# JiapengWu/TeMP

Hardware: AMD Instinct MI355X
Metric: edges/sec (fwd+bwd) RGCN+GRU seq_len=15 (higher is better)
Workload: dtype f32

## Files before the change

### include/temp_amd.h

```cpp
#ifndef TEMP_AMD_H
#define TEMP_AMD_H

#include <stddef.h>
#include <stdint.h>

#ifdef __cplusplus
extern "C" {
#endif

#define TEMP_ABI_VERSION 2

enum {
  TEMP_OK = 0,
  TEMP_E_BADARG = 1,
  TEMP_E_UNSUPPORTED = 2,
  TEMP_E_WORKSPACE = 3,
  TEMP_E_LAUNCH = 4
};

enum { TEMP_ACT_NONE = 0, TEMP_ACT_RELU = 1 };
enum { TEMP_GRU_TORCH = 0,
       TEMP_GRU_TYPE1 = 1 };

int temp_abi_version(void);
// ... 108 lines not shown
  TempEdgeView by_pair;
} TempPairView;
int temp_expand_chunk_segments(int n_chunks, const int32_t* chunk_seg, const int32_t* chunk_beg, const int32_t* chunk_end, int n_pos,
                               int32_t* seg_of, void* stream);
int temp_rgcn_pair_supported(int d_in, int d_out, int num_bases);
size_t temp_rgcn_pair_fwd_workspace(const TempGraph* g, const TempPairView* pv, int d_out);
int temp_rgcn_pair_fwd(const TempGraph* g, const TempPairView* pv, const float* table, const int32_t* ids, int n_table, int d_in, int d_out,
                       int num_bases, int n_rel_rows, const float* weight, const float* loop_w, const float* bias, int act, float* out,
                       void* workspace, size_t workspace_bytes, const TempDropout* drop, void* stream);
size_t temp_rgcn_pair_bwd_workspace(const TempGraph* g, const TempPairView* pv, int d_in, int d_out, int num_bases);
int temp_rgcn_pair_bwd(const TempGraph* g, const TempPairView* pv, const float* table, const int32_t* ids, const int32_t* inv_ptr,
                       const int32_t* inv_order, int n_table, const float* out, const float* d_out_grad, int d_in, int d_out, int num_bases,
                       int n_rel_rows, const float* weight, const float* loop_w, int has_bias, int act, float* d_table, float* d_weight,
                       float* d_loop_w, float* d_bias, void* workspace, size_t workspace_bytes, const TempDropout* drop, void* stream);

int temp_rgcn_isolated_fwd(int n, int d, const float* e, const float* loop_w, const float* bias ,
                           int act, float* out, const TempDropout* drop, void* stream);
size_t temp_rgcn_isolated_bwd_workspace(int n, int d);
int temp_rgcn_isolated_bwd(int n, int d, const float* e, const float* out, const float* d_out_grad,
                           const float* loop_w, int has_bias, int act,
                           float* d_e, float* d_loop_w, float* d_bias ,
                           void* workspace, size_t workspace_bytes, const TempDropout* drop, void* stream);

int temp_gru_fwd(int n, int d, int variant,
                 const float* x, const float* prev, const int32_t* prev_idx , const float* dt,
                 float lambda, const float* decay_wb ,
                 const float* w_ih, const float* w_hh, const float* b_ih, const float* b_hh,
                 float* h_out, float* saved, void* stream);

size_t temp_gru_bwd_workspace(int n, int d, int variant);
int temp_gru_bwd(int n, int d, int variant,
                 const float* x, const float* prev, const int32_t* prev_idx , const float* dt,
                 float lambda, const float* decay_wb ,
                 const float* w_ih, const float* w_hh,
                 const float* saved, const float* d_h_out,
                 float* d_x, float* d_prev, float* d_w_ih, float* d_w_hh, float* d_b_ih, float* d_b_hh,
                 float* d_decay_wb ,
                 void* workspace, size_t workspace_bytes, void* stream);

int temp_decay_rows(int n, int d, const float* x, const float* dt, float lambda, float* out, void* stream);

int temp_gru_input_gates(int n, int d, int variant, const float* x, const float* w_ih, const float* b_ih, float* gi, void* stream);
int temp_gru_input_gates_multi(int count, const int* ns, int d, int variant, const float* const* xs, const float* const* w_ihs,
                               const float* const* b_ihs, float* const* gis, void* stream);
int temp_gru_input_gates_gather_multi(int count, const int* ns, int d, int variant, const float* const* xs, const int32_t* const* x_idx,
                                      const float* const* w_ihs, const float* const* b_ihs, float* const* gis, void* stream);
int temp_gru_cell_fwd(int n, int d, int variant, const float* gi, const float* prev, const int32_t* prev_idx ,
                      const float* dt, float lambda, const float* w_hh, const float* b_hh,
                      float* h_out, float* saved, size_t saved_plane, void* stream);
int temp_gru_cell_bwd(int n, int d, int variant, const float* saved, size_t saved_plane,
                      const float* dh_up , const float* d_prev_next , const int32_t* next_idx ,
                      const float* dt, float lambda, const float* w_hh,
                      float* dgi, float* dgh, float* decv, float* d_prev, void* stream);
typedef struct TempGruCellFwd {
  int32_t n; const float* gi; const float* prev ;
  const int32_t* prev_idx ; const float* dt;
  const float* w_hh; const float* b_hh; float* h_out; float* saved ;
} TempGruCellFwd;
typedef struct TempGruCellBwd {
  int32_t n; const float* saved; const float* dh_up ; const float* d_prev_next ;
  const int32_t* next_idx ; const float* dt; const float* w_hh;
  float* dgi; float* dgh; float* decv; float* d_prev;
  int32_t no_prev;
} TempGruCellBwd;
int temp_gru_cell_fwd_multi(int count, const TempGruCellFwd* cells, int d, int variant, float lambda, size_t saved_plane, void* stream);
int temp_gru_cell_bwd_multi(int count, const TempGruCellBwd* cells, int d, int variant, float lambda, size_t saved_plane, void* stream);
size_t temp_gru_weight_grads_workspace(int n, int d, int variant);
int temp_gru_weight_grads(int n, int d, int variant, const float* x, const float* hdec, const float* dgi, const float* dgh,
                          const float* w_ih, float* d_x , float* d_w_ih, float* d_w_hh, float* d_b_ih, float* d_b_hh,
                          void* workspace, size_t workspace_bytes, void* stream);
size_t temp_gru_weight_grads_multi_workspace(int count, const int* ns, int d, int variant);
int temp_gru_weight_grads_multi(int count, const int* ns, int d, int variant, const float* const* xs, const float* const* hdecs,
                                const float* const* dgis, const float* const* dghs, const float* const* w_ihs, float* const* d_xs,
                                float* d_w, float* d_b, void* workspace, size_t workspace_bytes, void* stream);

size_t temp_gru_grads_g4_workspace(int count, const int* ns, int d);
int temp_gru_grads_g4(int count, const int* ns, int d, const float* const* xs, const float* const* hdecs, const float* const* g4s,
                      const float* const* w_ihs, float* const* d_xs, float* d_w, float* d_b, void* workspace, size_t workspace_bytes,
                      void* stream);
int temp_gru_grads_g4_keys(int count, const int* ns, int d, const float* const* xs, const float* const* hdecs, const float* const* g4s,
                           const float* const* w_ihs, float* const* d_xs, float* d_w, float* d_b, const uint32_t* const* g4_row_keys,
                           const uint32_t* const* g4_col_keys, const uint32_t* const* x_col_keys ,
                           void* workspace, size_t workspace_bytes, void* stream);

#define TEMP_CHAIN_HAS_PREV (1 << 30)
#define TEMP_CHAIN_TRACKS 32
#define TEMP_CHAIN_MAX_RNN 4
#define TEMP_CHAIN_MAX_UP 8
typedef struct TempGruChain {
  int32_t d, variant, n_panels, n_steps;
  int32_t max_steps;
  const int32_t* panel; const int32_t* rows; const int32_t* sinfo;
  const float* dt;
  float lambda;
  size_t saved_plane;
  int32_t n_rnn;
  const float* packed[TEMP_CHAIN_MAX_RNN];
  const float* b_hh[TEMP_CHAIN_MAX_RNN];
  const int32_t* gi_index;
  int32_t pack_layout;
} TempGruChain;
enum { TEMP_CHAIN_PACK_F32 = 1, TEMP_CHAIN_PACK_BX = 2, TEMP_CHAIN_PACK_HX = 3, TEMP_CHAIN_PACK_HX_X = 4 };
int temp_gru_chain_pack_layout(int d);
int temp_gru_chain_supported(int d);
size_t temp_gru_chain_pack_floats(int d);
int temp_gru_chain_pack(int d, const float* w_hh, float* packed, void* stream);
int temp_gru_chain_pack_multi(int count, int d, const float* const* w_hh, float* const* packed, void* stream);
int temp_gru_chain_fwd(const TempGruChain* c, const float* gi, float* h_out, float* saved, void* stream);
int temp_gru_chain_fwd_x_supported(int d, int variant, int max_steps);
size_t temp_gru_chain_pack_x_floats(int d);
int temp_gru_chain_pack_x_multi(int count, int d, const float* const* w_hh, const float* const* w_ih, float* const* packed, void* stream);
int temp_gru_chain_fwd_x(const TempGruChain* c, const float* x, const int32_t* x_index, const float* const* b_ih, float* h_out, float* saved,
                         void* stream);
long long temp_gru_chain_fwd_x_launches(void);
int temp_gru_chain_bwd(const TempGruChain* c, const float* saved, int n_up, const float* const* up ,
                       float* dgi, float* dgh, void* stream);
int temp_gru_chain_bwd_g4(const TempGruChain* c, const float* saved, int n_up, const float* const* up ,
                          float* g4, void* stream);
int temp_gru_chain_keys_supported(int d);
int temp_gru_chain_bwd_g4_keys(const TempGruChain* c, const float* saved, int n_up, const float* const* up, float* g4,
                               uint32_t* row_keys, uint32_t* col_keys, void* stream);

int temp_gather_rows(int n, int d, const float* table, const int32_t* idx, float* out, void* stream);
size_t temp_keys_cols_size(int d);
int temp_absmax_keys(int n, int d, const float* x, int ldx, uint32_t* row_keys, uint32_t* col_keys, void* stream);
int temp_gather_rows_keys(int n, int d, const float* table, const int32_t* idx, float* out, uint32_t* row_keys, uint32_t* col_keys, void* stream);
int temp_linear_keys(int M, int N, int K, const float* A, int lda, const uint32_t* a_keys, const float* B, int ldb, int trans_b, float* C, int ldc,
                     void* stream);
int temp_gru_input_gates_gather_multi_keys(int count, const int* ns, int d, int variant, const float* const* xs, const int32_t* const* x_idx,
                                           const uint32_t* const* x_keys, const float* const* w_ihs, const float* const* b_ihs, float* const* gis,
                                           void* stream);
int temp_scatter_add_rows(int n, int d, const float* src, const int32_t* idx, float* table, void* stream);
size_t temp_segment_sum_rows_workspace(int n_seg, int n_rows, int d);
int temp_segment_sum_rows(int n_seg, int n_rows, int d, const int32_t* seg_ptr, const int32_t* order, const float* src, float* out,
                          void* workspace, size_t workspace_bytes, void* stream);
int temp_segment_sum_rows_relu(int n_seg, int n_rows, int d, const int32_t* seg_ptr, const int32_t* order, const float* src, const float* relu_of,
                               float* out, void* workspace, size_t workspace_bytes, void* stream);

int temp_linear(int M, int N, int K, const float* A, int lda, const float* B, int ldb, int trans_b, float* C, int ldc, void* stream);
int temp_linear_t(int M, int N, int K, const float* A, int lda, const float* B, int ldb, int trans_b, float* Ct, int ldct, void* stream);
typedef struct TempLinearProblem { int M; const float* A; const float* B; float* C; } TempLinearProblem;
int temp_linear_multi(int count, const TempLinearProblem* probs, int N, int K, int lda, int ldb, int trans_b, int ldc, void* stream);
size_t temp_linear_tn_workspace(int M, int Ka, int Nb);
int temp_linear_tn(int M, int Ka, int Nb, const float* A, int lda, const float* B, int ldb, float* out, int ldo,
                   void* workspace, size_t workspace_bytes, void* stream);
size_t temp_linear_tn_multi_workspace(int count, int max_m, int Ka, int Nb);
int temp_linear_tn_multi(int count, const TempLinearProblem* probs, int Ka, int Nb, int lda, int ldb, int ldc, void* workspace,
                         size_t workspace_bytes, void* stream);

int temp_gather_ce_fwd(int P, int C, int N, const float* scores, const int32_t* cand, float* loss_rows, float* lse_rows, void* stream);
int temp_gather_ce_bwd(int P, int C, int N, const float* scores, const int32_t* cand, const float* lse_rows, const float* scale,
                       float inv_rows, const float* row_scale , float* d_scores, void* stream);

#define TEMP_SCORE_DISTMULT 0
#define TEMP_SCORE_COMPLEX 1
int temp_bilinear_query_fwd(int P, int d, int kind, const float* ent_rows, const int32_t* known_idx, const float* rel, const int32_t* rel_idx,
                            const int32_t* is_tail, float* q, void* stream);
int temp_bilinear_query_bwd(int P, int d, int kind, const float* ent_rows, const int32_t* known_idx, const float* rel, const int32_t* rel_idx,
                            const int32_t* is_tail, const float* d_q, float* d_known_rows, float* d_rel_rows, void* stream);

int temp_gated_query_fwd(int P, int d, int kind, const float* A, const int32_t* ia, const float* B, const int32_t* ib, const float* w,
                         const float* rel, const int32_t* rel_idx, const int32_t* is_tail, float* q, void* stream);
int temp_gated_query_bwd(int P, int d, int kind, const float* A, const int32_t* ia, const float* B, const int32_t* ib, const float* w,
                         const float* rel, const int32_t* rel_idx, const int32_t* is_tail, const float* d_q, float* d_a_rows, float* d_b_rows,
                         float* d_rel_rows, float* d_w, void* stream);
int temp_gather_ce_mix_fwd(int P, int C, int N, const float* s_a, const float* s_b, const float* w, const int32_t* cand, float* loss_rows,
                           float* lse_rows, void* stream);
int temp_gather_ce_mix_bwd(int P, int C, int N, const float* s_a, const float* s_b, const float* w, const int32_t* cand, const float* lse_rows,
                           const float* scale, float inv_rows, const float* row_scale , float* d_s_a, float* d_s_b,
                           float* d_w, void* stream);

#define TEMP_ASSEMBLE_PIECE 4096
typedef struct TempCopyDesc { const int32_t* src; const int32_t* aux; int32_t dst_off; int32_t len; int32_t add; int32_t mode; } TempCopyDesc;
int temp_assemble_views(int n_pieces, const int32_t* piece_desc, const int32_t* piece_start, const TempCopyDesc* descs, const int32_t* table,
                        int32_t* out, void* stream);

typedef struct TempSubsampleJob {
  int32_t n_nodes, n_edges, keep;
  uint64_t seed;
  const int32_t* parent; int32_t* child; const int32_t* eid;
  int32_t off_a[3], off_b[3], off_chunk_beg[3], off_chunk_end[3], off_chunk_seg[3], n_chunks[3];
  int32_t off_in_deg, off_out_deg, off_nnorm;
  uint8_t* keep_mask; void* scratch;
} TempSubsampleJob;
int temp_subsample_views(int n_jobs, const TempSubsampleJob* jobs, void* stream);

int temp_corrupt_sample(int R, int K, int N, uint64_t seed, const int32_t* truth, const int32_t* lo, const int32_t* hi, const int32_t* ids,
                        int32_t* cand, void* stream);

int temp_filtered_rank(int P, int N, int ld, const float* scores, const int32_t* target, const int32_t* filt_ptr,
                       const int32_t* filt_ids, int32_t* ranks, void* stream);

typedef struct TempAttn {
  int32_t n, D, heads, T;
// ... 22 lines not shown
```

### temp_amd/_lib.py

```python
import ctypes
import threading
import os

_HERE = os.path.dirname(os.path.abspath(__file__))
LIB_PATH = os.path.join(_HERE, "libtemp_amd.so")

c_i32p = ctypes.POINTER(ctypes.c_int32)
c_f32p = ctypes.POINTER(ctypes.c_float)
c_vp = ctypes.c_void_p

ACT_NONE, ACT_RELU = 0, 1
GRU_TORCH, GRU_TYPE1 = 0, 1
CHUNK = 64
CHUNK_REL = 128


class TempEdgeView(ctypes.Structure):
    _fields_ = [("n_seg", ctypes.c_int32), ("n_edges", ctypes.c_int32), ("a", c_vp), ("b", c_vp),
                ("n_chunks", ctypes.c_int32), ("chunk_seg", c_vp), ("chunk_beg", c_vp), ("chunk_end", c_vp),
                ("chunk_slot", c_vp), ("n_partial", ctypes.c_int32), ("n_fix", ctypes.c_int32),
                ("fix_seg", c_vp), ("fix_slot", c_vp), ("fix_cnt", c_vp)]


class TempMembers(ctypes.Structure):
    _fields_ = [("n_members", ctypes.c_int32), ("max_nodes", ctypes.c_int32), ("max_edges", ctypes.c_int32),
                ("max_chunks", ctypes.c_int32 * 3), ("node_off", c_vp), ("edge_off", c_vp), ("chunk_off", c_vp), ("fix_off", c_vp)]


class TempGraph(ctypes.Structure):
    _fields_ = [("n_nodes", ctypes.c_int32), ("n_edges", ctypes.c_int32), ("nnorm", c_vp), ("in_deg", c_vp),
                ("out_deg", c_vp), ("by_dst", TempEdgeView), ("by_src", TempEdgeView), ("by_rel", TempEdgeView),
                ("members", TempMembers)]


class TempPairView(ctypes.Structure):
    _fields_ = [("n_table", ctypes.c_int32), ("n_rel_rows", ctypes.c_int32), ("fwd_row", c_vp), ("by_pair", TempEdgeView)]


ABI_VERSION = 2
OPT_MFMA_BF16X3, OPT_TN_SPLIT, OPT_RGCN_SCALAR, OPT_GEMM_STREAM, OPT_GRU_STREAM, OPT_RGCN_TILE, OPT_DEBUG, OPT_OVERLAP, OPT_GEMM_RESIDENT, OPT_MFMA_F16X2, OPT_RGCN_PAIR = range(11)


class TempGruCellFwd(ctypes.Structure):
    _fields_ = [("n", ctypes.c_int32), ("gi", c_vp), ("prev", c_vp), ("prev_idx", c_vp), ("dt", c_vp), ("w_hh", c_vp),
                ("b_hh", c_vp), ("h_out", c_vp), ("saved", c_vp)]


class TempGruCellBwd(ctypes.Structure):
    _fields_ = [("n", ctypes.c_int32), ("saved", c_vp), ("dh_up", c_vp), ("d_prev_next", c_vp), ("next_idx", c_vp), ("dt", c_vp),
                ("w_hh", c_vp), ("dgi", c_vp), ("dgh", c_vp), ("decv", c_vp), ("d_prev", c_vp), ("no_prev", ctypes.c_int32)]


CHAIN_HAS_PREV = 1 << 30
CHAIN_TRACKS = 32
CHAIN_MAX_RNN = 4
CHAIN_MAX_UP = 8
CHAIN_MAX_STEPS = 64
CHAIN_PACK_F32, CHAIN_PACK_BX, CHAIN_PACK_HX, CHAIN_PACK_HX_X = 1, 2, 3, 4


class TempGruChain(ctypes.Structure):
    _fields_ = [("d", ctypes.c_int32), ("variant", ctypes.c_int32), ("n_panels", ctypes.c_int32), ("n_steps", ctypes.c_int32),
                ("max_steps", ctypes.c_int32), ("panel", c_vp), ("rows", c_vp), ("sinfo", c_vp), ("dt", c_vp), ("lambda_", ctypes.c_float),
                ("saved_plane", ctypes.c_size_t), ("n_rnn", ctypes.c_int32), ("packed", c_vp * CHAIN_MAX_RNN), ("b_hh", c_vp * CHAIN_MAX_RNN),
                ("gi_index", c_vp), ("pack_layout", ctypes.c_int32)]


class TempSubsampleJob(ctypes.Structure):
    _fields_ = [("n_nodes", ctypes.c_int32), ("n_edges", ctypes.c_int32), ("keep", ctypes.c_int32), ("seed", ctypes.c_uint64),
                ("parent", c_vp), ("child", c_vp), ("eid", c_vp),
                ("off_a", ctypes.c_int32 * 3), ("off_b", ctypes.c_int32 * 3), ("off_chunk_beg", ctypes.c_int32 * 3),
                ("off_chunk_end", ctypes.c_int32 * 3), ("off_chunk_seg", ctypes.c_int32 * 3), ("n_chunks", ctypes.c_int32 * 3),
                ("off_in_deg", ctypes.c_int32), ("off_out_deg", ctypes.c_int32), ("off_nnorm", ctypes.c_int32),
                ("keep_mask", c_vp), ("scratch", c_vp)]


class TempDropout(ctypes.Structure):
    _fields_ = [("p", ctypes.c_float), ("seed", ctypes.c_uint64)]


class TempAttn(ctypes.Structure):
    _fields_ = [("n", ctypes.c_int32), ("D", ctypes.c_int32), ("heads", ctypes.c_int32), ("T", ctypes.c_int32),
                ("q", c_vp), ("ldq", ctypes.c_int32), ("kh", c_vp), ("vh", c_vp), ("ldh", ctypes.c_int32),
                ("kc", c_vp), ("vc", c_vp), ("ldc", ctypes.c_int32), ("idx", c_vp), ("decay", c_vp)]


class TempLinearProblem(ctypes.Structure):
    _fields_ = [("M", ctypes.c_int32), ("A", c_vp), ("B", c_vp), ("C", c_vp)]


ASSEMBLE_PIECE = 4096
SCORE_KINDS = {"distmult": 0, "complex": 1}

_G = ctypes.POINTER(TempGraph)
_PV = ctypes.POINTER(TempPairView)
_I, _F, _SZ = ctypes.c_int, ctypes.c_float, ctypes.c_size_t
SYMBOLS = {
    "temp_abi_version": (_I, []),
    "temp_error_string": (ctypes.c_char_p, [_I]),
    "temp_set_option": (_I, [_I, _I]),
    "temp_get_option": (_I, [_I]),
    "temp_scratch_refused": (ctypes.c_longlong, []),
    "temp_f16_launches": (ctypes.c_longlong, []),
    "temp_tile_launches": (ctypes.c_longlong, []),
    "temp_set_debug_buffer": (None, [c_vp, _SZ]),
    "temp_rgcn_fwd_workspace": (_SZ, [_G, _I]),
    "temp_rgcn_fwd": (_I, [_G, c_vp, c_vp, _I, _I, _I, _I, c_vp, c_vp, c_vp, _I, c_vp, c_vp, _SZ, c_vp, c_vp]),
    "temp_rgcn_bwd_workspace": (_SZ, [_G, _I, _I, _I, _I]),
    "temp_rgcn_bwd": (_I, [_G, c_vp, c_vp, c_vp, _I, _I, _I, _I, c_vp, c_vp, _I, _I, c_vp, c_vp, c_vp, c_vp, c_vp, _SZ, c_vp, c_vp]),
    "temp_rgcn_bwd_dh": (_I, [_G, c_vp, c_vp, _I, _I, _I, _I, c_vp, c_vp, _I, c_vp, c_vp, c_vp, c_vp, _SZ, c_vp, c_vp]),
    "temp_rgcn_bwd_weights": (_I, [_G, c_vp, c_vp, c_vp, _I, _I, _I, _I, _I, c_vp, c_vp, c_vp, c_vp, _SZ, c_vp]),
    "temp_rgcn_table_fwd_workspace": (_SZ, [_G, _I, _I]),
    "temp_rgcn_table_fwd": (_I, [_G, c_vp, c_vp, _I, _I, _I, _I, _I, c_vp, c_vp, c_vp, _I, c_vp, c_vp, _SZ, c_vp, c_vp]),
    "temp_rgcn_table_bwd_workspace": (_SZ, [_G, _I, _I, _I, _I]),
    "temp_rgcn_table_bwd": (_I, [_G, c_vp, c_vp, c_vp, c_vp, _I, c_vp, c_vp, _I, _I, _I, _I, c_vp, c_vp, _I, _I, c_vp, c_vp, c_vp, c_vp,
                                 c_vp, _SZ, c_vp, c_vp]),
    "temp_pair_launches": (ctypes.c_longlong, []),
    "temp_expand_chunk_segments": (_I, [_I, c_vp, c_vp, c_vp, _I, c_vp, c_vp]),
    "temp_rgcn_pair_supported": (_I, [_I, _I, _I]),
    "temp_rgcn_pair_fwd_workspace": (_SZ, [_G, _PV, _I]),
    "temp_rgcn_pair_fwd": (_I, [_G, _PV, c_vp, c_vp, _I, _I, _I, _I, _I, c_vp, c_vp, c_vp, _I, c_vp, c_vp, _SZ, c_vp, c_vp]),
    "temp_rgcn_pair_bwd_workspace": (_SZ, [_G, _PV, _I, _I, _I]),
    "temp_rgcn_pair_bwd": (_I, [_G, _PV, c_vp, c_vp, c_vp, c_vp, _I, c_vp, c_vp, _I, _I, _I, _I, c_vp, c_vp, _I, _I, c_vp, c_vp, c_vp, c_vp,
                                c_vp, _SZ, c_vp, c_vp]),
    "temp_rgcn_isolated_fwd": (_I, [_I, _I, c_vp, c_vp, c_vp, _I, c_vp, c_vp, c_vp]),
    "temp_rgcn_isolated_bwd_workspace": (_SZ, [_I, _I]),
    "temp_rgcn_isolated_bwd": (_I, [_I, _I, c_vp, c_vp, c_vp, c_vp, _I, _I, c_vp, c_vp, c_vp, c_vp, _SZ, c_vp, c_vp]),
    "temp_gru_fwd": (_I, [_I, _I, _I, c_vp, c_vp, c_vp, c_vp, _F, c_vp, c_vp, c_vp, c_vp, c_vp, c_vp, c_vp, c_vp]),
    "temp_gru_bwd_workspace": (_SZ, [_I, _I, _I]),
    "temp_gru_bwd": (_I, [_I, _I, _I, c_vp, c_vp, c_vp, c_vp, _F, c_vp, c_vp, c_vp, c_vp, c_vp,
                          c_vp, c_vp, c_vp, c_vp, c_vp, c_vp, c_vp, c_vp, _SZ, c_vp]),
    "temp_decay_rows": (_I, [_I, _I, c_vp, c_vp, _F, c_vp, c_vp]),
    "temp_gru_input_gates": (_I, [_I, _I, _I, c_vp, c_vp, c_vp, c_vp, c_vp]),
    "temp_gru_input_gates_multi": (_I, [_I, c_vp, _I, _I, c_vp, c_vp, c_vp, c_vp, c_vp]),
    "temp_gru_input_gates_gather_multi": (_I, [_I, c_vp, _I, _I, c_vp, c_vp, c_vp, c_vp, c_vp, c_vp]),
    "temp_gru_cell_fwd": (_I, [_I, _I, _I, c_vp, c_vp, c_vp, c_vp, _F, c_vp, c_vp, c_vp, c_vp, _SZ, c_vp]),
    "temp_gru_cell_bwd": (_I, [_I, _I, _I, c_vp, _SZ, c_vp, c_vp, c_vp, c_vp, _F, c_vp, c_vp, c_vp, c_vp, c_vp, c_vp]),
    "temp_gru_cell_fwd_multi": (_I, [_I, ctypes.POINTER(TempGruCellFwd), _I, _I, _F, _SZ, c_vp]),
    "temp_gru_cell_bwd_multi": (_I, [_I, ctypes.POINTER(TempGruCellBwd), _I, _I, _F, _SZ, c_vp]),
    "temp_gru_weight_grads_workspace": (_SZ, [_I, _I, _I]),
    "temp_gru_weight_grads": (_I, [_I, _I, _I, c_vp, c_vp, c_vp, c_vp, c_vp, c_vp, c_vp, c_vp, c_vp, c_vp, c_vp, _SZ, c_vp]),
    "temp_gru_weight_grads_multi_workspace": (ctypes.c_size_t, [_I, c_vp, _I, _I]),
    "temp_gru_weight_grads_multi": (_I, [_I, c_vp, _I, _I, c_vp, c_vp, c_vp, c_vp, c_vp, c_vp, c_vp, c_vp, c_vp, ctypes.c_size_t, c_vp]),
    "temp_gru_chain_supported": (_I, [_I]),
    "temp_gru_chain_pack_floats": (_SZ, [_I]),
    "temp_gru_chain_pack": (_I, [_I, c_vp, c_vp, c_vp]),
    "temp_gru_chain_pack_multi": (_I, [_I, _I, ctypes.POINTER(c_vp), ctypes.POINTER(c_vp), c_vp]),
    "temp_gru_chain_fwd": (_I, [ctypes.POINTER(TempGruChain), c_vp, c_vp, c_vp, c_vp]),
    "temp_gru_chain_pack_layout": (_I, [_I]),
    "temp_gru_chain_fwd_x_supported": (_I, [_I, _I, _I]),
    "temp_gru_chain_pack_x_floats": (_SZ, [_I]),
    "temp_gru_chain_pack_x_multi": (_I, [_I, _I, ctypes.POINTER(c_vp), ctypes.POINTER(c_vp), ctypes.POINTER(c_vp), c_vp]),
    "temp_gru_chain_fwd_x": (_I, [ctypes.POINTER(TempGruChain), c_vp, c_vp, ctypes.POINTER(c_vp), c_vp, c_vp, c_vp]),
    "temp_gru_chain_fwd_x_launches": (ctypes.c_longlong, []),
    "temp_gru_chain_bwd": (_I, [ctypes.POINTER(TempGruChain), c_vp, _I, ctypes.POINTER(c_vp), c_vp, c_vp, c_vp]),
    "temp_gru_chain_bwd_g4": (_I, [ctypes.POINTER(TempGruChain), c_vp, _I, ctypes.POINTER(c_vp), c_vp, c_vp]),
    "temp_gru_chain_keys_supported": (_I, [_I]),
    "temp_gru_chain_bwd_g4_keys": (_I, [ctypes.POINTER(TempGruChain), c_vp, _I, ctypes.POINTER(c_vp), c_vp, c_vp, c_vp, c_vp]),
    "temp_gru_grads_g4_keys": (_I, [_I, c_vp, _I, c_vp, c_vp, c_vp, c_vp, c_vp, c_vp, c_vp, c_vp, c_vp, c_vp, c_vp, ctypes.c_size_t, c_vp]),
    "temp_gru_grads_g4_workspace": (ctypes.c_size_t, [_I, c_vp, _I]),
    "temp_gru_grads_g4": (_I, [_I, c_vp, _I, c_vp, c_vp, c_vp, c_vp, c_vp, c_vp, c_vp, c_vp, ctypes.c_size_t, c_vp]),
    "temp_gather_rows": (_I, [_I, _I, c_vp, c_vp, c_vp, c_vp]),
    "temp_keys_cols_size": (_SZ, [_I]),
    "temp_absmax_keys": (_I, [_I, _I, c_vp, _I, c_vp, c_vp, c_vp]),
    "temp_gather_rows_keys": (_I, [_I, _I, c_vp, c_vp, c_vp, c_vp, c_vp, c_vp]),
    "temp_linear_keys": (_I, [_I, _I, _I, c_vp, _I, c_vp, c_vp, _I, _I, c_vp, _I, c_vp]),
    "temp_gru_input_gates_gather_multi_keys": (_I, [_I, c_vp, _I, _I, c_vp, c_vp, c_vp, c_vp, c_vp, c_vp, c_vp]),
    "temp_scatter_add_rows": (_I, [_I, _I, c_vp, c_vp, c_vp, c_vp]),
    "temp_segment_sum_rows_workspace": (_SZ, [_I, _I, _I]),
    "temp_segment_sum_rows": (_I, [_I, _I, _I, c_vp, c_vp, c_vp, c_vp, c_vp, _SZ, c_vp]),
    "temp_segment_sum_rows_relu": (_I, [_I, _I, _I, c_vp, c_vp, c_vp, c_vp, c_vp, c_vp, _SZ, c_vp]),
    "temp_linear": (_I, [_I, _I, _I, c_vp, _I, c_vp, _I, _I, c_vp, _I, c_vp]),
    "temp_linear_t": (_I, [_I, _I, _I, c_vp, _I, c_vp, _I, _I, c_vp, _I, c_vp]),
    "temp_linear_multi": (_I, [_I, ctypes.POINTER(TempLinearProblem), _I, _I, _I, _I, _I, _I, c_vp]),
    "temp_linear_tn_workspace": (_SZ, [_I, _I, _I]),
    "temp_linear_tn_multi_workspace": (_SZ, [_I, _I, _I, _I]),
    "temp_linear_tn_multi": (_I, [_I, ctypes.POINTER(TempLinearProblem), _I, _I, _I, _I, _I, c_vp, _SZ, c_vp]),
    "temp_linear_tn": (_I, [_I, _I, _I, c_vp, _I, c_vp, _I, c_vp, _I, c_vp, _SZ, c_vp]),
    "temp_gather_ce_fwd": (_I, [_I, _I, _I, c_vp, c_vp, c_vp, c_vp, c_vp]),
    "temp_gather_ce_bwd": (_I, [_I, _I, _I, c_vp, c_vp, c_vp, c_vp, _F, c_vp, c_vp, c_vp]),
    "temp_bilinear_query_fwd": (_I, [_I, _I, _I, c_vp, c_vp, c_vp, c_vp, c_vp, c_vp, c_vp]),
    "temp_bilinear_query_bwd": (_I, [_I, _I, _I, c_vp, c_vp, c_vp, c_vp, c_vp, c_vp, c_vp, c_vp, c_vp]),
    "temp_gated_query_fwd": (_I, [_I, _I, _I, c_vp, c_vp, c_vp, c_vp, c_vp, c_vp, c_vp, c_vp, c_vp, c_vp]),
    "temp_gated_query_bwd": (_I, [_I, _I, _I, c_vp, c_vp, c_vp, c_vp, c_vp, c_vp, c_vp, c_vp, c_vp, c_vp, c_vp, c_vp, c_vp, c_vp]),
    "temp_gather_ce_mix_fwd": (_I, [_I, _I, _I, c_vp, c_vp, c_vp, c_vp, c_vp, c_vp, c_vp]),
    "temp_gather_ce_mix_bwd": (_I, [_I, _I, _I, c_vp, c_vp, c_vp, c_vp, c_vp, c_vp, _F, c_vp, c_vp, c_vp, c_vp, c_vp]),
    "temp_assemble_views": (_I, [_I, c_vp, c_vp, c_vp, c_vp, c_vp, c_vp]),
    "temp_subsample_views": (_I, [_I, ctypes.POINTER(TempSubsampleJob), c_vp]),
    "temp_corrupt_sample": (_I, [_I, _I, _I, ctypes.c_uint64, c_vp, c_vp, c_vp, c_vp, c_vp, c_vp]),
    "temp_filtered_rank": (_I, [_I, _I, _I, c_vp, c_vp, c_vp, c_vp, c_vp, c_vp]),
    "temp_sa_attn_fwd": (_I, [ctypes.POINTER(TempAttn), c_vp, c_vp, c_vp, c_vp]),
    "temp_sa_attn_bwd": (_I, [ctypes.POINTER(TempAttn), c_vp, c_vp, c_vp, c_vp, c_vp, _I, c_vp, c_vp, _I, c_vp, c_vp, _I, c_vp, _I, c_vp, c_vp, c_vp, c_vp]),
    "temp_copy_probe": (_I, [c_vp, c_vp, _SZ, c_vp]),
    "temp_trace_begin": (_I, [_I]),
    "temp_trace_end": (_I, [c_i32p, c_f32p, _I, c_i32p]),
    "temp_trace_kernel_name": (ctypes.c_char_p, [_I]),
}

_lib = None


class TempAmdError(RuntimeError):
    pass


def load():
    global _lib
    if _lib is not None:
        return _lib
    if not os.path.exists(LIB_PATH):
        raise TempAmdError("libtemp_amd.so not found at %s -- run `python -m temp_amd.build` "
                           "(hipcc --offload-arch=gfx950); there is no CPU fallback" % LIB_PATH)
    lib = ctypes.CDLL(LIB_PATH) if os.environ.get("TEMP_PYDLL", "1") == "0" else ctypes.PyDLL(LIB_PATH)
    for name, (res, args) in SYMBOLS.items():
        fn = getattr(lib, name)
        fn.restype = res
        fn.argtypes = args
    if lib.temp_abi_version() != ABI_VERSION:
        raise TempAmdError("libtemp_amd.so ABI version %d != %d (stale .so or stale Python package)" % (lib.temp_abi_version(), ABI_VERSION))
    _lib = lib
    return lib


def check(rc, what):
    if rc != 0:
        msg = load().temp_error_string(rc).decode()
        raise TempAmdError("%s failed: %s (code %d)" % (what, msg, rc))


class _CreateLock:

    def __init__(self):
        self._l = threading.RLock()

    def __enter__(self):
        if not self._l.acquire(blocking=False):
            held = getattr(_coop, "held", False)
            if held:
                _py_token.release()
            self._l.acquire()
            if held:
                _py_token.acquire()
# ... 100 lines not shown
```

### temp_amd/backend.py

```python
import ctypes

import torch

from . import _lib

_backend = None


def set_backend(b):
    global _backend
    _backend = b


def get_backend():
    global _backend
    if _backend is None:
        _backend = HipBackend()
    return _backend


def _ptr(t):
    return ctypes.c_void_p(t.data_ptr()) if t is not None else None


# ... 298 lines not shown
            a.dh_up, a.d_prev_next, a.next_idx = opt(c["dh_up"]), opt(c["d_prev_next"]), opt(nidx)
            a.dt, a.w_hh = dt.data_ptr(), w_hh.data_ptr()
            a.dgi, a.dgh, a.decv, a.d_prev = c["dgi"].data_ptr(), c["dgh"].data_ptr(), c["decv"].data_ptr(), c["d_prev"].data_ptr()
            a.no_prev = 1 if c.get("no_prev") else 0
        rc = self.lib.temp_gru_cell_bwd_multi(len(cells), arr, d, variant, float(lam), saved_all.shape[1] * d, _stream())
        _lib.check(rc, "temp_gru_cell_bwd_multi")

    def subsample_views(self, jobs):
        arr = (_lib.TempSubsampleJob * len(jobs))()
        for a, j in zip(arr, jobs):
            a.n_nodes, a.n_edges, a.keep, a.seed = j["n_nodes"], j["n_edges"], j["keep"], int(j["seed"]) & 0xFFFFFFFFFFFFFFFF
            a.parent, a.child = _i32(j["parent"], "parent").data_ptr(), _i32(j["child"], "child").data_ptr()
            a.eid = _i32(j["eid"], "eid").data_ptr() if j["n_edges"] else None
            for fld in ("off_a", "off_b", "off_chunk_beg", "off_chunk_end", "off_chunk_seg", "n_chunks"):
                for v in range(3):
                    getattr(a, fld)[v] = int(j[fld][v])
            a.off_in_deg, a.off_out_deg, a.off_nnorm = int(j["off_in_deg"]), int(j["off_out_deg"]), int(j["off_nnorm"])
            a.keep_mask = j["keep_mask"].data_ptr() if j.get("keep_mask") is not None else None
            a.scratch = j["scratch"].data_ptr()
        _lib.check(self.lib.temp_subsample_views(len(jobs), arr, _stream()), "temp_subsample_views")

    def decay_rows(self, x, dt, lam):
        x, dt = _f32(x, "x"), _f32(dt, "dt")
        out = torch.empty_like(x)
        _lib.check(self.lib.temp_decay_rows(x.shape[0], x.shape[1], _ptr(x), _ptr(dt), float(lam), _ptr(out), _stream()), "temp_decay_rows")
        return out

    def gru_chain_supported(self, d):
        return bool(self.lib.temp_gru_chain_supported(int(d)))

    def gru_chain_pack(self, w_hh):
        w_hh = _f32(w_hh, "w_hh")
        d = w_hh.shape[1]
        out = torch.empty(self.lib.temp_gru_chain_pack_floats(d), dtype=torch.float32, device=w_hh.device)
        layout = self.lib.temp_gru_chain_pack_layout(d)
        _lib.check(self.lib.temp_gru_chain_pack(d, _ptr(w_hh), _ptr(out), _stream()), "temp_gru_chain_pack")
        out.chain_pack_layout = layout
        return out

    def gru_chain_pack_multi(self, w_hhs):
        w_hhs = [_f32(w, "w_hh") for w in w_hhs]
        d = w_hhs[0].shape[1]
        n = self.lib.temp_gru_chain_pack_floats(d)
        buf = torch.empty(len(w_hhs), n, dtype=torch.float32, device=w_hhs[0].device)
        src = (ctypes.c_void_p * len(w_hhs))(*[w.data_ptr() for w in w_hhs])
        dst = (ctypes.c_void_p * len(w_hhs))(*[buf[i].data_ptr() for i in range(len(w_hhs))])
        layout = self.lib.temp_gru_chain_pack_layout(d)
        _lib.check(self.lib.temp_gru_chain_pack_multi(len(w_hhs), d, src, dst, _stream()), "temp_gru_chain_pack_multi")
        return self._tagged([buf[i] for i in range(len(w_hhs))], layout)

    @staticmethod
    def _tagged(packs, layout):
        for pk in packs:
            pk.chain_pack_layout = layout
        return packs

    def _chain_desc(self, tabs, d, variant, lam, plane, packs, b_hhs):
        c = _lib.TempGruChain()
        c.d, c.variant, c.n_panels, c.n_steps, c.max_steps = d, variant, tabs["n_panels"], tabs["n_steps"], tabs["max_steps"]
        c.panel, c.rows, c.sinfo, c.dt = (_i32(tabs[k], k).data_ptr() for k in ("panel", "rows", "sinfo", "dt_bits"))
        c.lambda_, c.saved_plane, c.n_rnn = float(lam), plane, len(packs)
        layouts = {getattr(pk, "chain_pack_layout", None) for pk in packs}
        assert len(layouts) == 1 and None not in layouts, "chain packs without one common layout tag (gru_chain_pack*)"
        c.pack_layout = layouts.pop()
        keep = []
        for i, (pk, b) in enumerate(zip(packs, b_hhs)):
            pk, b = _f32(pk, "packed"), _f32(b, "b_hh")
            keep += [pk, b]
            c.packed[i], c.b_hh[i] = pk.data_ptr(), b.data_ptr()
        return c, keep

    def gru_chain_fwd(self, tabs, gi, lam, variant, packs, b_hhs, h_out, saved_all, gi_index=None):
        d = saved_all.shape[2]
        c, keep = self._chain_desc(tabs, d, variant, lam, saved_all.shape[1] * d, packs, b_hhs)
        if gi_index is not None:
            assert gi_index.shape[0] == saved_all.shape[1]
            c.gi_index = _i32(gi_index, "gi_index").data_ptr()
        rc = self.lib.temp_gru_chain_fwd(ctypes.byref(c), _ptr(_f32(gi, "gi")), _ptr(h_out), _ptr(saved_all), _stream())
        _lib.check(rc, "temp_gru_chain_fwd")

    def gru_chain_fwd_x_supported(self, d, variant, max_steps):
        return bool(self.lib.temp_gru_chain_fwd_x_supported(int(d), int(variant), int(max_steps)))

    def gru_chain_pack_x_multi(self, w_hhs, w_ihs):
        w_hhs, w_ihs = [_f32(w, "w_hh") for w in w_hhs], [_f32(w, "w_ih") for w in w_ihs]
        d = w_hhs[0].shape[1]
        k = len(w_hhs)
        n = self.lib.temp_gru_chain_pack_x_floats(d)
        buf = torch.empty(k, n, dtype=torch.float32, device=w_hhs[0].device)
        arr = lambda ts: (ctypes.c_void_p * k)(*[t.data_ptr() for t in ts])
        _lib.check(self.lib.temp_gru_chain_pack_x_multi(k, d, arr(w_hhs), arr(w_ihs), arr([buf[i] for i in range(k)]), _stream()),
                   "temp_gru_chain_pack_x_multi")
        return self._tagged([buf[i] for i in range(k)], _lib.CHAIN_PACK_HX_X)

    def gru_chain_fwd_x(self, tabs, x, x_index, lam, variant, packs, b_hhs, b_ihs, h_out, saved_all):
        d = saved_all.shape[2]
        c, keep = self._chain_desc(tabs, d, variant, lam, saved_all.shape[1] * d, packs, b_hhs)
        x = _f32(x, "x")
        assert x.shape[1] == d and x_index.shape[0] == saved_all.shape[1]
        b_ihs = [_f32(b, "b_ih") for b in b_ihs]
        barr = (ctypes.c_void_p * len(b_ihs))(*[b.data_ptr() for b in b_ihs])
        rc = self.lib.temp_gru_chain_fwd_x(ctypes.byref(c), _ptr(x), _ptr(_i32(x_index, "x_index")), barr, _ptr(h_out), _ptr(saved_all), _stream())
        _lib.check(rc, "temp_gru_chain_fwd_x")

    def gru_chain_bwd(self, tabs, saved_all, ups, lam, variant, packs, b_hhs, dgi, dgh):
        d = saved_all.shape[2]
        c, keep = self._chain_desc(tabs, d, variant, lam, saved_all.shape[1] * d, packs, b_hhs)
        ups = [_f32(u, "upstream") if u is not None else None for u in ups]
        arr = (ctypes.c_void_p * max(len(ups), 1))(*[u.data_ptr() if u is not None else None for u in ups])
        rc = self.lib.temp_gru_chain_bwd(ctypes.byref(c), _ptr(saved_all), len(ups), arr, _ptr(dgi), _ptr(dgh), _stream())
        _lib.check(rc, "temp_gru_chain_bwd")

    def gru_chain_keys_supported(self, d):
        return bool(self.lib.temp_gru_chain_keys_supported(int(d)))

    def gru_chain_bwd_g4(self, tabs, saved_all, ups, lam, variant, packs, b_hhs, g4, keys=None):
        d = saved_all.shape[2]
        c, keep = self._chain_desc(tabs, d, variant, lam, saved_all.shape[1] * d, packs, b_hhs)
        ups = [_f32(u, "upstream") if u is not None else None for u in ups]
        arr = (ctypes.c_void_p * max(len(ups), 1))(*[u.data_ptr() if u is not None else None for u in ups])
        if keys is not None:
            row_keys, col_keys = keys
            assert row_keys.dtype == torch.int32 and col_keys.dtype == torch.int32 and col_keys.is_contiguous()
            assert row_keys.numel() == saved_all.shape[1] and col_keys.numel() == (len(packs) + tabs["n_panels"]) * 4 * d
            rc = self.lib.temp_gru_chain_bwd_g4_keys(ctypes.byref(c), _ptr(saved_all), len(ups), arr, _ptr(g4), _ptr(row_keys), _ptr(col_keys),
                                                     _stream())
            _lib.check(rc, "temp_gru_chain_bwd_g4_keys")
            return
        rc = self.lib.temp_gru_chain_bwd_g4(ctypes.byref(c), _ptr(saved_all), len(ups), arr, _ptr(g4), _stream())
        _lib.check(rc, "temp_gru_chain_bwd_g4")

    def gru_grads_g4_supported(self, ns, d, variant):
        k = len(ns)
        if k < 1 or k > 4 or variant != _lib.GRU_TORCH:
            return False
        return self.lib.temp_gru_grads_g4_workspace(k, (ctypes.c_int * k)(*[int(n) for n in ns]), int(d)) > 0

    def gru_grads_g4(self, xs, hdecs, g4s, w_ihs, d_xs, row_keys=None, col_keys=None, x_col_keys=None):
        k = len(xs)
        d = xs[0].shape[1]
        dev = xs[0].device
        ns = (ctypes.c_int * k)(*[x.shape[0] for x in xs])
        nb = self.lib.temp_gru_grads_g4_workspace(k, ns, d)
        if nb == 0:
            raise ValueError("temp_gru_grads_g4: unsupported shape (check gru_grads_g4_supported first)")
        keep = [[_f32(t, "operand") for t in ts] for ts in (xs, hdecs, w_ihs)]
        for g in g4s:
            assert g.dtype == torch.float32 and g.is_contiguous() and g.shape[1] == 4 * d
        arr = lambda ts: (ctypes.c_void_p * k)(*[t.data_ptr() for t in ts])
        dx = (ctypes.c_void_p * k)(*[None if t is None else t.data_ptr() for t in d_xs])
        d_w = torch.empty(2 * k, 3 * d, d, dtype=torch.float32, device=dev)
        d_b = torch.empty(2 * k, 3 * d, dtype=torch.float32, device=dev)
        ws = self._ws(nb, dev)
        if row_keys is not None and col_keys is not None:
            for rk, ck, x in zip(row_keys, col_keys, xs):
                assert rk.dtype == torch.int32 and ck.dtype == torch.int32 and rk.is_contiguous() and ck.is_contiguous()
                assert rk.numel() == x.shape[0] and ck.numel() == 4 * d
            xk = None
            if x_col_keys is not None:
                for t in x_col_keys:
                    assert t.dtype == torch.int32 and t.is_contiguous() and t.numel() == d
                xk = arr(x_col_keys)
            rc = self.lib.temp_gru_grads_g4_keys(k, ns, d, arr(keep[0]), arr(keep[1]), arr(g4s), arr(keep[2]), dx, _ptr(d_w), _ptr(d_b),
                                                 arr(row_keys), arr(col_keys), xk, _ptr(ws), ws.numel(), _stream())
            _lib.check(rc, "temp_gru_grads_g4_keys")
            return [(d_w[2 * i], d_w[2 * i + 1], d_b[2 * i], d_b[2 * i + 1]) for i in range(k)]
        rc = self.lib.temp_gru_grads_g4(k, ns, d, arr(keep[0]), arr(keep[1]), arr(g4s), arr(keep[2]), dx, _ptr(d_w), _ptr(d_b), _ptr(ws),
                                        ws.numel(), _stream())
        _lib.check(rc, "temp_gru_grads_g4")
        return [(d_w[2 * i], d_w[2 * i + 1], d_b[2 * i], d_b[2 * i + 1]) for i in range(k)]

    def gru_weight_grads(self, x, hdec, dgi, dgh, w_ih, variant, d_x):
        n, d = x.shape
        w_ih = _f32(w_ih, "w_ih")
        dev = x.device
        d_w_ih = torch.empty_like(w_ih)
        d_w_hh = torch.empty(3 * d, d, dtype=torch.float32, device=dev)
        d_b_ih = torch.empty(w_ih.shape[0], dtype=torch.float32, device=dev)
        d_b_hh = torch.empty(3 * d, dtype=torch.float32, device=dev)
        ws = self._ws(self.lib.temp_gru_weight_grads_workspace(n, d, variant), dev)
        rc = self.lib.temp_gru_weight_grads(n, d, variant, _ptr(x), _ptr(hdec), _ptr(dgi), _ptr(dgh), _ptr(w_ih), _ptr(d_x),
                                            _ptr(d_w_ih), _ptr(d_w_hh), _ptr(d_b_ih), _ptr(d_b_hh), _ptr(ws), ws.numel(), _stream())
        _lib.check(rc, "temp_gru_weight_grads")
        return d_w_ih, d_w_hh, d_b_ih, d_b_hh

    def gru_weight_grads_multi(self, xs, hdecs, dgis, dghs, w_ihs, variant, d_xs):
        k = len(xs)
        if k < 1 or k > 4 or variant != _lib.GRU_TORCH or any(h is None for h in hdecs):
            return None
        d = xs[0].shape[1]
        dev = xs[0].device
        ns = (ctypes.c_int * k)(*[x.shape[0] for x in xs])
        nb = self.lib.temp_gru_weight_grads_multi_workspace(k, ns, d, variant)
        if nb == 0:
            return None
        keep = [[_f32(t, "operand") for t in ts] for ts in (xs, hdecs, dgis, dghs, w_ihs)]
        arr = lambda ts: (ctypes.c_void_p * k)(*[t.data_ptr() for t in ts])
        dx = (ctypes.c_void_p * k)(*[None if t is None else t.data_ptr() for t in d_xs])
        d_w = torch.empty(2 * k, 3 * d, d, dtype=torch.float32, device=dev)
        d_b = torch.empty(2 * k, 3 * d, dtype=torch.float32, device=dev)
        ws = self._ws(nb, dev)
        rc = self.lib.temp_gru_weight_grads_multi(k, ns, d, variant, arr(keep[0]), arr(keep[1]), arr(keep[2]), arr(keep[3]), arr(keep[4]), dx,
                                                  _ptr(d_w), _ptr(d_b), _ptr(ws), ws.numel(), _stream())
        if rc == 2:
            return None
        _lib.check(rc, "temp_gru_weight_grads_multi")
        return [(d_w[2 * i], d_w[2 * i + 1], d_b[2 * i], d_b[2 * i + 1]) for i in range(k)]

    def linear(self, a, b, trans_b, out=None, a_keys=None):
        a, b = _f32(a, "a"), _f32(b, "b")
        M, K = a.shape
        N = b.shape[0] if trans_b else b.shape[1]
        c = out if out is not None else torch.empty(M, N, dtype=torch.float32, device=a.device)
        assert c.shape == (M, N) and c.is_contiguous() and c.dtype == torch.float32
        if a_keys is not None:
            assert a_keys.dtype == torch.int32 and a_keys.is_contiguous() and a_keys.numel() == M
            rc = self.lib.temp_linear_keys(M, N, K, _ptr(a), K, _ptr(a_keys), _ptr(b), b.shape[1], int(trans_b), _ptr(c), N, _stream())
            _lib.check(rc, "temp_linear_keys")
            return c
        rc = self.lib.temp_linear(M, N, K, _ptr(a), K, _ptr(b), b.shape[1], int(trans_b), _ptr(c), N, _stream())
        _lib.check(rc, "temp_linear")
        return c

    def absmax_keys(self, x, rows=True, cols=True):
        x = _f32(x, "x")
        n, d = x.shape
        rk = torch.empty(n, dtype=torch.int32, device=x.device) if rows else None
        ck = torch.empty(self.lib.temp_keys_cols_size(d), dtype=torch.int32, device=x.device) if cols else None
        _lib.check(self.lib.temp_absmax_keys(n, d, _ptr(x), d, _ptr(rk), _ptr(ck), _stream()), "temp_absmax_keys")
        return rk, (ck[:d] if cols else None)

    def linear_t(self, a, b, trans_b, out_t):
        a, b = _f32(a, "a"), _f32(b, "b")
        M, K = a.shape
        N = b.shape[0] if trans_b else b.shape[1]
        if out_t.shape != (N, M) or not out_t.is_contiguous() or out_t.dtype != torch.float32:
            raise ValueError("linear_t: out_t must be a contiguous float32 (N, M) matrix")
        rc = self.lib.temp_linear_t(M, N, K, _ptr(a), K, _ptr(b), b.shape[1], int(trans_b), _ptr(out_t), M, _stream())
        _lib.check(rc, "temp_linear_t")
        return out_t

    def linear_multi(self, a_list, b_list, trans_b, out):
        K = a_list[0].shape[1]
        N = out.shape[1]
        arr = (_lib.TempLinearProblem * len(a_list))()
# ... 254 lines not shown
```

### temp_amd/csrc/gemm_bx.hpp

```cpp
#pragma once
#include "gemm_panel.hpp"

namespace temp {

typedef __bf16 bx_bf16x8 __attribute__((ext_vector_type(8)));
typedef unsigned int bx_u32x4 __attribute__((ext_vector_type(4)));

__device__ __forceinline__ void bx_split(float x, unsigned& h, unsigned& m, unsigned& l) {
  h = __float_as_uint(x) & 0xffff0000u;
  const float r1 = x - __uint_as_float(h);
  m = __float_as_uint(r1) & 0xffff0000u;
  l = __float_as_uint(r1 - __uint_as_float(m));
}
__device__ __forceinline__ void bx_split2(float x0, float x1, unsigned& H, unsigned& M, unsigned& L) {
  unsigned h0, m0, l0, h1, m1, l1;
  bx_split(x0, h0, m0, l0);
  bx_split(x1, h1, m1, l1);
  H = __builtin_amdgcn_perm(h1, h0, 0x07060302u);
  M = __builtin_amdgcn_perm(m1, m0, 0x07060302u);
  L = __builtin_amdgcn_perm(l1, l0, 0x07060302u);
}
__device__ __forceinline__ void bx_split8(const float4 a, const float4 b, bx_u32x4& H, bx_u32x4& M, bx_u32x4& L) {
  unsigned h, m, l;
  bx_split2(a.x, a.y, h, m, l); H[0] = h; M[0] = m; L[0] = l;
// ... 496 lines not shown
  g->per_xcd = ceil_div(g->row_tiles, 8);
  int best = 1;
  float best_cost = 1e30f;
  const int gmax = g->n_tiles < 7 ? g->n_tiles : 7;
  for (int w = 1; w <= gmax; ++w) {
    const int ng = ceil_div(g->n_tiles, w);
    const long long all_tiles = total_rows > 0 ? (total_rows + 127) / 128 : g->row_tiles;
    const long long blocks = (all_tiles > g->row_tiles ? all_tiles : (long long)g->row_tiles) * ng;
    const float rounds = blocks <= 512 ? 1.f : (float)blocks / 512.f + 0.5f;
    const float cost = rounds * (w + 0.5f);
    if (cost < best_cost * 0.999f || (cost <= best_cost * 1.001f && w > best)) { best_cost = cost; best = w; }
  }
  *G = best;
  g->n_groups = ceil_div(g->n_tiles, best);
  g->tail_store = g->n_tiles - (g->n_groups - 1) * best;
  return true;
}

}
#include "gemm_bxr.hpp"
#include "gemm_hx.hpp"
namespace temp {

template <class Epi>
static inline bool bx_pack_batch(const PanelBatch<Epi>& batch, int count, const BxGeom& g, hipStream_t st, BxPacked* pk) {
  const size_t pbytes = bx_packed_bytes(g.N, g.K);
  int n_distinct = 0, which[PANEL_MAXP];
  for (int i = 0; i < count; ++i) {
    which[i] = -1;
    for (int j = 0; j < i; ++j)
      if (batch.p[j].B == batch.p[i].B) { which[i] = which[j]; break; }
    if (which[i] < 0) which[i] = n_distinct++;
  }
  bx_u32x4* slot = pbytes * n_distinct <= BX_PACK_MAX_BYTES ? bx_scratch(st, pbytes * n_distinct) : nullptr;
  if (!slot) return false;
  const int n_slabs = ceil_div(g.K, 16);
  int done = 0;
  BxPackJobs jobs = {};
  for (int i = 0; i < PANEL_MAXP; ++i) pk->b[i] = slot;
  for (int i = 0; i < count; ++i) {
    bx_u32x4* dst = slot + (size_t)which[i] * (pbytes / 16);
    pk->b[i] = dst;
    if (which[i] < done) continue;
    ++done;
    if (n_distinct > 1 && n_distinct <= BX_PACK_JOBS) { bx_pack_jobs_add(jobs, batch.p[i].B, dst, g.K, g.N, g.ldb, g.trans_b); continue; }
    const dim3 pgrid(ceil_div((long long)n_slabs * g.n_tiles, 4));
    if (g.trans_b) TEMP_LAUNCH(K_BX_PACK, (k_bx_pack<1>), pgrid, dim3(256), 0, st, g.K, g.N, g.n_tiles, n_slabs, batch.p[i].B, g.ldb, dst);
    else TEMP_LAUNCH(K_BX_PACK, (k_bx_pack<0>), pgrid, dim3(256), 0, st, g.K, g.N, g.n_tiles, n_slabs, batch.p[i].B, g.ldb, dst);
  }
  if (jobs.count) TEMP_LAUNCH(K_BX_PACK, k_bx_pack_multi, dim3(ceil_div(jobs.total_units, 4)), dim3(256), 0, st, jobs);
  return true;
}

template <int G, class Epi>
static inline void launch_bx_g(int kid, const PanelBatch<Epi>& batch, int count, const BxGeom& g, hipStream_t st, const BxPacked* pk) {
  dim3 grid(8 * g.per_xcd * g.n_groups, count);
  if (pk) {
    TEMP_LAUNCH(kid, (k_gemm_bxp<G, Epi>), grid, dim3(BX_THREADS), 0, st, batch, g, *pk);
    return;
  }
  if (g.trans_b) TEMP_LAUNCH(kid, (k_gemm_bx<G, 1, Epi>), grid, dim3(BX_THREADS), 0, st, batch, g);
  else TEMP_LAUNCH(kid, (k_gemm_bx<G, 0, Epi>), grid, dim3(BX_THREADS), 0, st, batch, g);
}

template <class Epi>
static inline bool launch_bxr(int kid, const PanelBatch<Epi>& batch, int count, const BxGeom& g, hipStream_t st, const BxPacked* pkp) {
  if (!option(TEMP_OPT_GEMM_RESIDENT) || g.K > BXR_MAX_SLABS * 16 || g.K < 72) return false;
  if (EpiRawPre<Epi>::value && !EpiAccInit<Epi>::value && !(option(TEMP_OPT_DEBUG) & 0x200000)) return false;
  int max_m = 0;
  for (int i = 0; i < count; ++i) max_m = batch.p[i].M > max_m ? batch.p[i].M : max_m;
  BxrGeom rg;
  if (!bxr_plan(g.N, g.K, g.lda, max_m, &rg)) return false;
  rg.ldb = g.ldb; rg.trans_b = g.trans_b;
  BxPacked pk;
  for (int i = 0; i < PANEL_MAXP; ++i) pk.b[i] = pkp ? pkp->b[i] : nullptr;
  static const bool granted = hipFuncSetAttribute(reinterpret_cast<const void*>(k_gemm_bxr<Epi>), hipFuncAttributeMaxDynamicSharedMemorySize, BXR_LDS_BYTES) == hipSuccess;
  if (!granted) { (void)hipGetLastError(); return false; }
  const size_t lds = (size_t)rg.n_slabs * BXR_G * 192 * 16 + BXR_BIAS_BYTES;
  TEMP_LAUNCH(kid, (k_gemm_bxr<Epi>), dim3(256, count), dim3(BXR_WAVES * 64), lds, st, batch, rg, pk);
  return true;
}

template <class Epi>
int launch_gemm_bx(int kid, const PanelBatch<Epi>& batch, int count, const BxGeom& g, int G, hipStream_t st) {
  if (launch_hxr(kid, batch, count, g, st)) return launch_status();
  if (launch_bxr(kid, batch, count, g, st, nullptr)) return launch_status();
  if (hx_supported(batch, count, g)) {
    const int rc = launch_gemm_hx(kid, batch, count, g, G, st);
    if (rc != TEMP_E_UNSUPPORTED) return rc;
  }
  BxPacked pk;
  const bool packed = bx_pack_batch(batch, count, g, st, &pk);
  const BxPacked* pp = packed ? &pk : nullptr;
  switch (G) {
    case 1: launch_bx_g<1, Epi>(kid, batch, count, g, st, pp); break;
    case 2: launch_bx_g<2, Epi>(kid, batch, count, g, st, pp); break;
    case 3: launch_bx_g<3, Epi>(kid, batch, count, g, st, pp); break;
    case 4: launch_bx_g<4, Epi>(kid, batch, count, g, st, pp); break;
    case 5: launch_bx_g<5, Epi>(kid, batch, count, g, st, pp); break;
    case 6: launch_bx_g<6, Epi>(kid, batch, count, g, st, pp); break;
    default: launch_bx_g<7, Epi>(kid, batch, count, g, st, pp); break;
  }
  return launch_status();
}

}
```

### temp_amd/csrc/gemm_hx.hpp

```cpp
#pragma once
#include "gemm_bx.hpp"
#include "hx_pack.hpp"

namespace temp {

struct HxPacked { const hx_u32x4* b[PANEL_MAXP]; const unsigned* keys[PANEL_MAXP]; };

template <int G, class Epi>
__global__ void __launch_bounds__(BX_THREADS, (G <= 4 ? 3 : 2)) k_gemm_hxp(PanelBatch<Epi> batch, BxGeom g, HxPacked packed, int keys_by_out) {
  constexpr int PIECES = G * 128;
  constexpr int NPC = (PIECES + BX_THREADS - 1) / BX_THREADS;
  __shared__ __attribute__((aligned(16))) hx_u32x4 Bs[2][PIECES];
  const PanelProblem<Epi>& pb = batch.p[blockIdx.y];
  const int M = pb.M;
  const int xcd = blockIdx.x & 7, local = blockIdx.x >> 3;
  const int grp = local % g.n_groups, rt_local = local / g.n_groups;
  const int rt = xcd * g.per_xcd + rt_local;
  if (rt_local >= g.per_xcd || rt * 128 >= M) return;
  const bool tail = grp == g.n_groups - 1;
  const int t0 = tail ? g.n_tiles - G : grp * G;
  const int t_store = tail ? G - g.tail_store : 0;
  const int n0 = t0 * 32;
  const int N = g.N, K = g.K;
  const float* __restrict__ A = pb.A;
// ... 182 lines not shown
struct AbsRowsBatch { int M[PANEL_MAXP]; const float* A[PANEL_MAXP]; const int32_t* idx[PANEL_MAXP]; unsigned* keys[PANEL_MAXP]; };
static __global__ void __launch_bounds__(256) k_absmax_rows_idx_multi(AbsRowsBatch b, int K, int lda) {
  const int pr = blockIdx.y;
  const int M = b.M[pr];
  const float* __restrict__ A = b.A[pr];
  const int32_t* __restrict__ a_idx = b.idx[pr];
  unsigned* __restrict__ keys = b.keys[pr];
  const int lane = threadIdx.x & 63, k4 = K >> 2;
  const int gw = blockIdx.x * 4 + (threadIdx.x >> 6), nw = gridDim.x * 4;
  for (int r0 = gw; r0 < M; r0 += 4 * nw) {
    float4 v[4];
    int src[4];
#pragma unroll
    for (int u = 0; u < 4; ++u) { const int r = r0 + u * nw; src[u] = r < M ? (a_idx ? a_idx[r] : r) : -1; }
#pragma unroll
    for (int u = 0; u < 4; ++u) v[u] = (src[u] >= 0 && lane < k4) ? ld4(A + (size_t)src[u] * lda + 4 * lane) : zero4();
#pragma unroll
    for (int u = 0; u < 4; ++u) {
      const int r = r0 + u * nw;
      unsigned k = hx_abs_bits4(v[u]);
      if (r < M) {
        for (int c = 256 + 4 * lane; c < K; c += 256) k = max(k, src[u] >= 0 ? hx_abs_bits4(ld4(A + (size_t)src[u] * lda + c)) : 0u);
        k = hx_wave_max(k);
        if (lane == 0) keys[r] = k;
      }
    }
  }
}

template <class Epi>
static inline bool hx_supported(const PanelBatch<Epi>& batch, int count, const BxGeom& g) {
  if (!hx_enabled() || g.K % 4 || g.lda % 4) return false;
  size_t need_keys = 0;
  for (int i = 0; i < count; ++i)
    if (!batch.p[i].a_keys) need_keys += align_up((size_t)(batch.p[i].M > 0 ? batch.p[i].M : 0) * 4, 256);
  if (need_keys > 0 && ceil_div(g.N, 32) < 16 && g.K < 400 && !(option(TEMP_OPT_DEBUG) & 0x800)) return false;
  return need_keys <= BX_SLOT_BYTES - HX_KEYS_OFFSET;
}

template <class Epi>
static inline bool hx_fill_keys(PanelBatch<Epi>& batch, int count, int K, int lda, unsigned char* slot, hipStream_t st, int* keys_by_out) {
  bool any_own = false, any_given_gather = false;
  for (int i = 0; i < count; ++i) {
    if (batch.p[i].M <= 0) continue;
    if (!batch.p[i].a_keys) any_own = true;
    else if (batch.p[i].a_idx) any_given_gather = true;
  }
  if (any_own && any_given_gather) return false;
  size_t koff = HX_KEYS_OFFSET;
  AbsRowsBatch ab = {};
  int n_own = 0, max_own = 0, last = -1;
  for (int i = 0; i < count; ++i) {
    if (batch.p[i].M <= 0) { batch.p[i].a_keys = reinterpret_cast<const unsigned*>(slot + HX_KEYS_OFFSET); continue; }
    if (batch.p[i].a_keys) continue;
    unsigned* keys = reinterpret_cast<unsigned*>(slot + koff);
    koff += align_up((size_t)batch.p[i].M * 4, 256);
    ab.M[n_own] = batch.p[i].M; ab.A[n_own] = batch.p[i].A; ab.idx[n_own] = batch.p[i].a_idx; ab.keys[n_own] = keys;
    max_own = batch.p[i].M > max_own ? batch.p[i].M : max_own;
    ++n_own;
    last = i;
    batch.p[i].a_keys = keys;
  }
  if (n_own == 1) {
    int blocks = ceil_div(batch.p[last].M, 16);
    if (blocks > 2048) blocks = 2048;
    TEMP_LAUNCH(K_KEYS, k_absmax_rows_idx, dim3(blocks), dim3(256), 0, st, ab.M[0], K, ab.A[0], lda, ab.idx[0], ab.keys[0]);
  } else if (n_own > 1) {
    int blocks = ceil_div(max_own, 16);
    if (blocks > 2048 / n_own) blocks = 2048 / n_own;
    TEMP_LAUNCH(K_KEYS, k_absmax_rows_idx_multi, dim3(blocks, n_own), dim3(256), 0, st, ab, K, lda);
  }
  for (int i = count; i < PANEL_MAXP; ++i) batch.p[i].a_keys = batch.p[0].a_keys;
  *keys_by_out = any_own ? 1 : 0;
  return true;
}

template <int G, class Epi>
static inline void launch_hxp_g(int kid, const PanelBatch<Epi>& batch, int count, const BxGeom& g, hipStream_t st, const HxPacked& pk, int keys_by_out) {
  dim3 grid(8 * g.per_xcd * g.n_groups, count);
  TEMP_LAUNCH(kid, (k_gemm_hxp<G, Epi>), grid, dim3(BX_THREADS), 0, st, batch, g, pk, keys_by_out);
}

template <class Epi>
int launch_gemm_hx(int kid, const PanelBatch<Epi>& batch_in, int count, const BxGeom& g, int G, hipStream_t st) {
  const size_t pbytes = align_up(hx_pack_bytes(g.N, g.K), 256);
  int n_distinct = 0, which[PANEL_MAXP];
  for (int i = 0; i < count; ++i) {
    which[i] = -1;
    for (int j = 0; j < i; ++j)
      if (batch_in.p[j].B == batch_in.p[i].B) { which[i] = which[j]; break; }
    if (which[i] < 0) which[i] = n_distinct++;
  }
  if (pbytes * n_distinct > BX_PACK_MAX_BYTES || n_distinct > HX_PACK_JOBS) return TEMP_E_UNSUPPORTED;
  unsigned char* slot = reinterpret_cast<unsigned char*>(bx_scratch(st, BX_SLOT_BYTES));
  if (!slot) return TEMP_E_UNSUPPORTED;
  PanelBatch<Epi> batch = batch_in;
  HxPacked pk;
  HxPackJobs jobs = {};
  const size_t items = hx_packed_items(g.N, g.K);
  int done = 0;
  for (int i = 0; i < PANEL_MAXP; ++i) { pk.b[i] = reinterpret_cast<const hx_u32x4*>(slot); pk.keys[i] = reinterpret_cast<const unsigned*>(slot + items * 16); }
  for (int i = 0; i < count; ++i) {
    unsigned char* dst = slot + (size_t)which[i] * pbytes;
    pk.b[i] = reinterpret_cast<const hx_u32x4*>(dst);
    pk.keys[i] = reinterpret_cast<const unsigned*>(dst + items * 16);
    if (which[i] < done) continue;
    ++done;
    hx_pack_jobs_add(jobs, batch.p[i].B, reinterpret_cast<hx_u32x4*>(dst), reinterpret_cast<unsigned*>(dst + items * 16), g.K, g.N, g.ldb, g.trans_b);
  }
  int kbo = 0;
  if (!hx_fill_keys(batch, count, g.K, g.lda, slot, st, &kbo)) return TEMP_E_UNSUPPORTED;
  hx_pack_launch(jobs, K_BX_PACK, st);
  hx_count();
  switch (G) {
    case 1: launch_hxp_g<1, Epi>(kid, batch, count, g, st, pk, kbo); break;
    case 2: launch_hxp_g<2, Epi>(kid, batch, count, g, st, pk, kbo); break;
    case 3: launch_hxp_g<3, Epi>(kid, batch, count, g, st, pk, kbo); break;
    case 4: launch_hxp_g<4, Epi>(kid, batch, count, g, st, pk, kbo); break;
    case 5: launch_hxp_g<5, Epi>(kid, batch, count, g, st, pk, kbo); break;
    case 6: launch_hxp_g<6, Epi>(kid, batch, count, g, st, pk, kbo); break;
    default: launch_hxp_g<7, Epi>(kid, batch, count, g, st, pk, kbo); break;
  }
  return launch_status();
}

}
#include "gemm_hxr.hpp"
namespace temp {

template <class Epi>
static inline bool launch_hxr(int kid, const PanelBatch<Epi>& batch_in, int count, const BxGeom& g, hipStream_t st) {
  if (!option(TEMP_OPT_GEMM_RESIDENT) || g.K > BXR_MAX_SLABS * 16 || g.K < 72 || g.K % 8 || !hx_supported(batch_in, count, g)) return false;
  int max_m = 0;
  for (int i = 0; i < count; ++i) max_m = batch_in.p[i].M > max_m ? batch_in.p[i].M : max_m;
  BxrGeom rg;
  if (!bxr_plan(g.N, g.K, g.lda, max_m, &rg)) return false;
  rg.ldb = g.ldb; rg.trans_b = g.trans_b;
  static const bool granted = hipFuncSetAttribute(reinterpret_cast<const void*>(k_gemm_hxr<Epi>), hipFuncAttributeMaxDynamicSharedMemorySize, HXR_LDS_BYTES) == hipSuccess;
  if (!granted) { (void)hipGetLastError(); return false; }
  PanelBatch<Epi> batch = batch_in;
  bool need = false;
  for (int i = 0; i < count; ++i) need = need || (batch.p[i].M > 0 && !batch.p[i].a_keys);
  int kbo = 0;
  if (need) {
    unsigned char* slot = reinterpret_cast<unsigned char*>(bx_scratch(st, BX_SLOT_BYTES));
    if (!slot || !hx_fill_keys(batch, count, g.K, g.lda, slot, st, &kbo)) return false;
  } else {
    for (int i = 0; i < PANEL_MAXP; ++i) if (!batch.p[i].a_keys) batch.p[i].a_keys = batch.p[0].a_keys;
    for (int i = 0; i < count; ++i) if (batch.p[i].M > 0) { for (int j = 0; j < PANEL_MAXP; ++j) if (!batch.p[j].a_keys) batch.p[j].a_keys = batch.p[i].a_keys; break; }
  }
  const size_t lds = (size_t)rg.n_slabs * BXR_G * 128 * 16 + 3 * BXR_BIAS_BYTES;
  TEMP_LAUNCH(kid, (k_gemm_hxr<Epi>), dim3(256, count), dim3(BXR_WAVES * 64), lds, st, batch, rg, kbo);
  hx_count();
  return true;
}

}
```

### temp_amd/csrc/gemm_wres.hpp

```cpp
#pragma once
#include <stdlib.h>
#include <type_traits>
#include "gemm_panel.hpp"
#include "gemm_bx.hpp"

namespace temp {

#define WRES_TPS 3
#define WRES_LDS_BYTES (80 * 1024)
#define WRES_LOCAL_BLOCKS 64

#define WRES_MIN_ROWS 4096
#define WRES_QC 5

struct WresGeom {
  int N, K, lda, ldb, trans_b;
  int ldk;
  int kpad;
  int n_tiles, tps;
  int n_slices;
  int tail_store;
  int gate_stride;
  int split;
};
// ... 182 lines not shown
        if constexpr (GROUP) {
          epi.fin_group(gpre, row, row_ok, n0, hh, acc);
        } else {
        const typename Epi::RowCtx rc = epi.row_ctx(row_ok ? row : 0);
#pragma unroll
        for (int t = 0; t < NTS; ++t) {
          if (t < t_store) continue;
          float4 pre[4];
          bool okc[4];
#pragma unroll
          for (int q = 0; q < 4; ++q) {
            const int col = n0 + t * 32 + 8 * q + 4 * hh;
            okc[q] = row_ok && col < g.N;
            pre[q] = epi.pre4(rc, okc[q] ? row : 0, okc[q] ? col : 0);
          }
#pragma unroll
          for (int q = 0; q < 4; ++q) {
            const int col = n0 + t * 32 + 8 * q + 4 * hh;
            if constexpr (VAR & 2) { if (acc[t][4 * q] == 12345.678f) epi.fin4(rc, row, col, zero4(), pre[q]); continue; }
            if (okc[q]) epi.fin4(rc, row, col, make_float4(acc[t][4 * q], acc[t][4 * q + 1], acc[t][4 * q + 2], acc[t][4 * q + 3]), pre[q]);
          }
        }
        }
        if constexpr (VAR & 8) epi.stamp(3, __builtin_amdgcn_s_memtime());
        zero_acc();
        chunk = 0;
        panel += stride;
      }
    };
    if (panel < p_end) {
      float4 bufA[QC], bufB[QC];
      bool okA = false, okB = false;
      int kcA = 0, kcB = 0;
      long srcA = -1, srcB = -1;
      setup_ld();
      zero_acc();
      issue(bufA, okA, kcA, srcA);
      while (true) {
        stage(bufA, okA, kcA, srcA, bufB, okB, kcB, srcB);
        if (panel >= p_end) break;
        stage(bufB, okB, kcB, srcB, bufA, okA, kcA, srcA);
        if (panel >= p_end) break;
      }
    }
    if constexpr (VAR & 8) epi.stamp(4, __builtin_amdgcn_s_memtime());
  }
}

template <int NTS, class Epi>
int launch_wres_one(int kid, const PanelBatch<Epi>& batch, int count, const WresGeom& g, hipStream_t st, int local_blocks = WRES_LOCAL_BLOCKS) {
  static bool attr_set = false;
  if (!attr_set) {
    if (hipFuncSetAttribute((const void*)k_gemm_wres<NTS, Epi>, hipFuncAttributeMaxDynamicSharedMemorySize, WRES_LDS_BYTES) != hipSuccess)
      return TEMP_E_LAUNCH;
    attr_set = true;
  }
  const int roles = g.n_slices * (g.split ? count : 1);
  const size_t lds = (size_t)NTS * 32 * g.ldk * 4;
  if (local_blocks == WRES_LOCAL_BLOCKS) {
    int per_cu = (int)((160 * 1024) / (lds + 1024));
    if (per_cu > 3) per_cu = 3;
    if (per_cu > 2) local_blocks = 32 * per_cu;
  }
  int bps = local_blocks / roles;
  if (bps < 1) bps = 1;
  int max_m = 0;
  for (int i = 0; i < count; ++i) max_m = batch.p[i].M > max_m ? batch.p[i].M : max_m;
  const int need = ceil_div(ceil_div(ceil_div(max_m, 32), 8), 4);
  if (bps > need) bps = need < 1 ? 1 : need;
  TEMP_LAUNCH(kid, (k_gemm_wres<NTS, Epi>), dim3(roles * bps * 8), dim3(256), lds, st, batch, count, g, bps);
  return launch_status();
}

template <class Epi>
int launch_gemm_wres(int kid, const PanelBatch<Epi>& batch, int count, const WresGeom& g, hipStream_t st) {
  if (g.tps == 3) return launch_wres_one<3, Epi>(kid, batch, count, g, st);
  if (g.tps == 2) return launch_wres_one<2, Epi>(kid, batch, count, g, st);
  return launch_wres_one<1, Epi>(kid, batch, count, g, st);
}

inline bool wres_disabled() { return option(TEMP_OPT_GEMM_STREAM) != 0; }

template <class Epi>
int launch_gemm_panel_multi(int kid, const PanelBatch<Epi>& batch, int count, int N, int K, int lda, int ldb, int trans_b, hipStream_t st) {
  if (count <= 0 || count > PANEL_MAXP) return TEMP_E_BADARG;
  long long rows = 0;
  for (int i = 0; i < count; ++i) rows += batch.p[i].M > 0 ? batch.p[i].M : 0;
  if (rows <= 0 || N <= 0) return TEMP_OK;
  if constexpr (!EpiIsGroup<Epi>::value) {
    if (bx_enabled()) {
      int max_m = 0;
      for (int i = 0; i < count; ++i) max_m = batch.p[i].M > max_m ? batch.p[i].M : max_m;
      BxGeom bg;
      int G;
      if (bx_plan(N, K, lda, ldb, trans_b, max_m, rows, &bg, &G)) return launch_gemm_bx(kid, batch, count, bg, G, st);
      if (K % 8 == 4 && bx_plan(N, K, lda, ldb, trans_b, max_m, rows, &bg, &G, true) && hx_supported(batch, count, bg)) {
        const int rc = launch_gemm_hx(kid, batch, count, bg, G, st);
        if (rc != TEMP_E_UNSUPPORTED) return rc;
      }
    }
  }
  WresGeom g;
  if (!wres_disabled() && wres_plan(N, K, lda, ldb, trans_b, rows, &g)) {
    bool distinct = count > 1;
    for (int i = 1; i < count; ++i) distinct = distinct && batch.p[i].B != batch.p[i - 1].B;
    if (distinct && g.n_slices * count <= WRES_LOCAL_BLOCKS) g.split = 1;
    return launch_gemm_wres(kid, batch, count, g, st);
  }
  return launch_gemm_stream_multi(kid, batch, count, N, K, lda, ldb, trans_b, st);
}

template <class Epi>
int launch_gemm_panel(int kid, int M, int N, int K, const float* A, int lda, const int32_t* a_idx, const float* B, int ldb, int trans_b,
                      const Epi& epi, hipStream_t st) {
  if (M <= 0 || N <= 0) return TEMP_OK;
  PanelBatch<Epi> batch;
  for (int i = 0; i < PANEL_MAXP; ++i) batch.p[i] = PanelProblem<Epi>{0, nullptr, nullptr, nullptr, epi};
  batch.p[0] = PanelProblem<Epi>{M, A, a_idx, B, epi};
  return launch_gemm_panel_multi(kid, batch, 1, N, K, lda, ldb, trans_b, st);
}

}
```

### temp_amd/csrc/gru_chain.hip

```cpp
#include <atomic>
#include "common.hpp"
#include "gru_math.hpp"
#include "gemm_bx.hpp"

namespace temp {

#define CH_SLOTS TEMP_CHAIN_TRACKS
#define CH_HAS_PREV TEMP_CHAIN_HAS_PREV
#define CH_ROW_MASK (TEMP_CHAIN_HAS_PREV - 1)
#define CH_LDS_LIMIT (160 * 1024)

struct ChainRnn { const float4* wf; const float4* wb; const float* b_hh; const unsigned* kf; const unsigned* kb; };
struct ChainArgs {
  int D, n_panels, max_steps, dbg;
  int layout;
  int n_rnn_keys;
  const int32_t* panel; const int32_t* rows; const int32_t* sinfo;
  const float* dt;
  const int32_t* gi_index;
  float lambda;
  size_t plane;
  ChainRnn rnn[TEMP_CHAIN_MAX_RNN];
};
struct ChainUps { const float* p[TEMP_CHAIN_MAX_UP]; };
// ... 493 lines not shown
          int en = -1;
          if (s + 1 < ns) en = tabb[(s + 1) * CH_SLOTS + slot];
          nxt[ps] = en >= 0 && (en & CH_HAS_PREV);
          const bool ok = e >= 0 && cact;
          const size_t row = ok ? (size_t)(e & CH_ROW_MASK) : 0;
          const float* src = saved + row * D + (ok ? col : 0);
          sr[ps] = ld4(src); sz[ps] = ld4(src + plane); sn[ps] = ld4(src + 2 * plane); shn[ps] = ld4(src + 3 * plane);
          shd[ps] = ld4(src + 4 * plane);
        }
      };
      prefetch(ns - 1);
      for (int s = ns - 1; s >= 0; --s) {
        const int cur = s & 1;
        const int up_sel = upb[2 * s], up_row0 = upb[2 * s + 1];
        const float* upp = up_sel >= 0 ? ups.p[up_sel] : nullptr;
#pragma unroll
        for (int ps = 0; ps < PASSES; ++ps) {
          const int slot = ps * MW + mw;
          const int e = erow[ps];
          if (!cact) continue;
          if (e < 0) continue;
          const size_t row = (size_t)(e & CH_ROW_MASK);
          float4 gd = upp ? ld4(upp + (row - (size_t)up_row0) * D + col) : zero4();
          if (nxt[ps]) gd = add4(gd, ld4(dpb + (size_t)slot * ldz + col));
          const float4 rg = sr[ps], zg = sz[ps], ng = sn[ps], hn = shn[ps], hd = shd[ps];
          float4 dr_pre, dz_pre, dn_pre, dhn, gz;
#define TEMP_GATE(c)                                          \
          {                                                   \
            const float dn = gd.c * (1.f - zg.c);             \
            const float dz = gd.c * (hd.c - ng.c);            \
            dn_pre.c = dn * (1.f - ng.c * ng.c);              \
            dr_pre.c = dn_pre.c * hn.c * rg.c * (1.f - rg.c); \
            dz_pre.c = dz * zg.c * (1.f - zg.c);              \
            dhn.c = dn_pre.c * rg.c;                          \
            gz.c = gd.c * zg.c;                               \
          }
          TEMP_GATE(x) TEMP_GATE(y) TEMP_GATE(z) TEMP_GATE(w)
#undef TEMP_GATE
          float* arow = ab + (size_t)slot * ldA + col;
          st4(arow, dr_pre); st4(arow + D, dz_pre); st4(arow + 2 * D, dhn);
          st4(gzb + (size_t)slot * ldz + col, gz);
          if constexpr (G4) {
            const size_t b4 = row * 4 * D + col;
            st4(dgi + b4, dr_pre); st4(dgi + b4 + D, dz_pre); st4(dgi + b4 + 2 * D, dn_pre); st4(dgi + b4 + 3 * D, dhn);
          } else {
          const size_t b3 = row * 3 * D + col;
          if (VARIANT == TEMP_GRU_TORCH) { st4(dgi + b3, dr_pre); st4(dgi + b3 + D, dz_pre); st4(dgi + b3 + 2 * D, dn_pre); }
          else st4(dgi + row * D + col, dn_pre);
          st4(dgh + b3, dr_pre); st4(dgh + b3 + D, dz_pre); st4(dgh + b3 + 2 * D, dhn);
          }
        }
        __syncthreads();
        if (s > 0) prefetch(s - 1);
        __syncthreads();
      }
    }
    __syncthreads();
  }
}

static bool chain_layout_ok(int layout, int d);
static int chain_check(const TempGruChain* c) {
  if (!c || c->d <= 0 || c->n_panels < 0 || c->n_steps < 0 || c->n_rnn <= 0 || c->n_rnn > TEMP_CHAIN_MAX_RNN) return TEMP_E_BADARG;
  if (c->variant != TEMP_GRU_TORCH && c->variant != TEMP_GRU_TYPE1) return TEMP_E_BADARG;
  if (c->n_panels > 0 && (!c->panel || !c->rows || !c->sinfo || !c->dt)) return TEMP_E_BADARG;
  for (int i = 0; i < c->n_rnn; ++i) if (!c->packed[i] || !c->b_hh[i]) return TEMP_E_BADARG;
  if (c->max_steps <= 0 || c->max_steps > CH_MAX_STEPS) return TEMP_E_BADARG;
  if (!temp_gru_chain_supported(c->d)) return TEMP_E_UNSUPPORTED;
  if (!chain_layout_ok(c->pack_layout, c->d)) return TEMP_E_BADARG;
  return TEMP_OK;
}

static bool chain_bx(int d) { return bx_enabled() && d % 8 == 0; }
static bool chain_hx_fits(int d) {
  if (d % 8) return false;
  const ChainGeomHx g = chain_geom_hx(d);
  return chain_lds_fwd_hx(d, CH_MAX_STEPS) <= CH_LDS_LIMIT && chain_lds_bwd_hx(d, CH_MAX_STEPS) <= CH_LDS_LIMIT && g.NT <= 20 && g.NTb <= 8;
}
static bool chain_hx(int d) { return chain_bx(d) && hx_enabled() && chain_hx_fits(d); }
static int chain_pack_layout(int d) { return chain_hx(d) ? TEMP_CHAIN_PACK_HX : chain_bx(d) ? TEMP_CHAIN_PACK_BX : TEMP_CHAIN_PACK_F32; }
static bool chain_layout_ok(int layout, int d) {
  if (layout == TEMP_CHAIN_PACK_F32) return true;
  if (layout == TEMP_CHAIN_PACK_BX) return d % 8 == 0;
  return (layout == TEMP_CHAIN_PACK_HX || layout == TEMP_CHAIN_PACK_HX_X) && chain_hx_fits(d);
}
static bool layout_hx(int layout) { return layout == TEMP_CHAIN_PACK_HX || layout == TEMP_CHAIN_PACK_HX_X; }

static ChainArgs chain_args(const TempGruChain* c) {
  ChainArgs a = {};
  const ChainGeom g = chain_geom(c->d);
  a.D = c->d; a.n_panels = c->n_panels; a.max_steps = c->max_steps; a.panel = c->panel; a.rows = c->rows; a.sinfo = c->sinfo; a.dt = c->dt;
  a.layout = c->pack_layout;
  a.n_rnn_keys = c->n_rnn; a.lambda = c->lambda; a.plane = c->saved_plane; a.gi_index = c->gi_index; a.dbg = option(TEMP_OPT_DEBUG) >> 8;
  for (int i = 0; i < c->n_rnn; ++i) {
    a.rnn[i].wf = (const float4*)c->packed[i];
    a.rnn[i].wb = (const float4*)c->packed[i] + (a.layout == TEMP_CHAIN_PACK_BX ? (size_t)(g.NQ >> 1) * g.NT * 192 : (size_t)g.NT * g.NQ * 64);
    a.rnn[i].b_hh = c->b_hh[i];
    a.rnn[i].kf = a.rnn[i].kb = nullptr;
    if (layout_hx(a.layout)) {
      const ChainGeomHx gx = chain_geom_hx(c->d);
      a.rnn[i].wb = (const float4*)c->packed[i] + chain_hx_fwd_items(c->d);
      a.rnn[i].kf = (const unsigned*)((const float4*)c->packed[i] + chain_hx_fwd_items(c->d) + chain_hx_bwd_items(c->d));
      a.rnn[i].kb = a.rnn[i].kf + gx.NT * 32;
    }
  }
  return a;
}

template <class K>
static int chain_lds_attr(K kernel, size_t bytes, bool* done) {
  if (*done) return TEMP_OK;
  if (hipFuncSetAttribute((const void*)kernel, hipFuncAttributeMaxDynamicSharedMemorySize, CH_LDS_LIMIT) != hipSuccess) return TEMP_E_LAUNCH;
  (void)bytes;
  *done = true;
  return TEMP_OK;
}

template <int VARIANT, int TPW>
static int launch_chain_fwd(const ChainArgs& a, const float* gi, float* h, float* saved, hipStream_t st) {
  static bool attr = false;
  static bool attr_bx = false;
  static bool attr_hx = false;
  if (layout_hx(a.layout)) {
    const size_t lds_hx = chain_lds_fwd_hx(a.D, a.max_steps);
    constexpr int TPW8 = (TPW * 4 + 7) / 8 < 1 ? 1 : (TPW * 4 + 7) / 8;
    const int cfg = (a.dbg >> 4) & 3;
    if (cfg == 1) {
      auto kernel = k_gru_chain_fwd_hx<VARIANT, TPW, 4, 4>;
      int rc = chain_lds_attr(kernel, lds_hx, &attr_hx);
      if (rc) return rc;
      TEMP_LAUNCH(K_GRU_CHAIN_FWD, kernel, dim3(a.n_panels), dim3(512), lds_hx, st, a, gi, h, saved);
    } else if (cfg == 2) {
      static bool attr_48 = false;
      auto kernel = k_gru_chain_fwd_hx<VARIANT, TPW, 8, 4>;
      int rc = chain_lds_attr(kernel, lds_hx, &attr_48);
      if (rc) return rc;
      TEMP_LAUNCH(K_GRU_CHAIN_FWD, kernel, dim3(a.n_panels), dim3(768), lds_hx, st, a, gi, h, saved);
    } else if (cfg == 3) {
      static bool attr_882 = false;
      auto kernel = k_gru_chain_fwd_hx<VARIANT, TPW8, 8, 8, 1>;
      int rc = chain_lds_attr(kernel, lds_hx, &attr_882);
      if (rc) return rc;
      TEMP_LAUNCH(K_GRU_CHAIN_FWD, kernel, dim3(a.n_panels), dim3(1024), lds_hx, st, a, gi, h, saved);
    } else {
      static bool attr_88 = false;
      auto kernel = k_gru_chain_fwd_hx<VARIANT, TPW8, 8, 8>;
      int rc = chain_lds_attr(kernel, lds_hx, &attr_88);
      if (rc) return rc;
      TEMP_LAUNCH(K_GRU_CHAIN_FWD, kernel, dim3(a.n_panels), dim3(1024), lds_hx, st, a, gi, h, saved);
    }
    hx_count();
    return launch_status();
  }
  const size_t lds = chain_lds_fwd(a.D, a.max_steps);
  if (a.layout == TEMP_CHAIN_PACK_BX) {
    auto kernel = k_gru_chain_fwd<VARIANT, TPW, 4, 1>;
    int rc = chain_lds_attr(kernel, lds, &attr_bx);
    if (rc) return rc;
    TEMP_LAUNCH(K_GRU_CHAIN_FWD, kernel, dim3(a.n_panels), dim3(512), lds, st, a, gi, h, saved);
    return launch_status();
  }
  auto kernel = k_gru_chain_fwd<VARIANT, TPW, 4, 0>;
  int rc = chain_lds_attr(kernel, lds, &attr);
  if (rc) return rc;
  TEMP_LAUNCH(K_GRU_CHAIN_FWD, kernel, dim3(a.n_panels), dim3(512), lds, st, a, gi, h, saved);
  return launch_status();
}

#define CH_FWD_X_OFF 0x400000
static std::atomic<long long> g_fwd_x_launches{0};
static size_t chain_x_ih_offset(int d) { return chain_hx_pack_floats(d); }
static bool chain_fwd_x_fits(int d, int max_steps) {
  return chain_hx_fits(d) && d / 4 <= 64 && max_steps > 0 && max_steps <= CH_MAX_STEPS && chain_lds_fwd_x(d, max_steps) <= CH_LDS_LIMIT &&
         (chain_geom_hx(d).NT + 7) / 8 <= 3;
}
static bool chain_fwd_x_ok(int d, int max_steps) { return chain_hx(d) && !(option(TEMP_OPT_DEBUG) & CH_FWD_X_OFF) && chain_fwd_x_fits(d, max_steps); }

template <int VARIANT, int TPWB, int G4 = 0>
static int launch_chain_bwd(const ChainArgs& a, const ChainUps& ups, const float* saved, float* dgi, float* dgh, hipStream_t st,
                            unsigned* row_keys = nullptr, unsigned* col_keys = nullptr) {
  static bool attr = false;
  static bool attr_bx = false;
  static bool attr_hx = false;
  if (layout_hx(a.layout)) {
    const size_t lds_hx = chain_lds_bwd_hx(a.D, a.max_steps);
    constexpr int TPWB8 = (TPWB * 4 + 7) / 8 < 1 ? 1 : (TPWB * 4 + 7) / 8;
    const int cfg = (a.dbg >> 4) & 3;
    if (cfg == 3) {
      static bool attr_5 = false;
      auto kernel = k_gru_chain_bwd_hx<VARIANT, TPWB, 8, G4, 4, 5>;
      int rc = chain_lds_attr(kernel, lds_hx, &attr_5);
      if (rc) return rc;
      TEMP_LAUNCH(K_GRU_CHAIN_BWD, kernel, dim3(a.n_panels), dim3(768), lds_hx, st, a, ups, saved, dgi, dgh, row_keys, col_keys);
    } else if (cfg != 2) {
      auto kernel = k_gru_chain_bwd_hx<VARIANT, TPWB, 8, G4, 4, 4>;
      int rc = chain_lds_attr(kernel, lds_hx, &attr_hx);
      if (rc) return rc;
      TEMP_LAUNCH(K_GRU_CHAIN_BWD, kernel, dim3(a.n_panels), dim3(768), lds_hx, st, a, ups, saved, dgi, dgh, row_keys, col_keys);
    } else {
      static bool attr_88 = false;
      auto kernel = k_gru_chain_bwd_hx<VARIANT, TPWB8, 8, G4, 8, 8>;
      int rc = chain_lds_attr(kernel, lds_hx, &attr_88);
      if (rc) return rc;
      TEMP_LAUNCH(K_GRU_CHAIN_BWD, kernel, dim3(a.n_panels), dim3(1024), lds_hx, st, a, ups, saved, dgi, dgh, row_keys, col_keys);
    }
    hx_count();
    if (col_keys) TEMP_LAUNCH(K_GRU_CHAIN_PACK, k_keys_reduce, dim3(ceil_div(4 * a.D, 32), a.n_rnn_keys), dim3(1024), 0, st, a.n_panels, 4 * a.D, col_keys + (size_t)a.n_rnn_keys * 4 * a.D, col_keys, a.panel, 4);
    return launch_status();
  }
  if (row_keys || col_keys) return TEMP_E_UNSUPPORTED;
  const size_t lds = chain_lds_bwd(a.D, a.max_steps);
  if (a.layout == TEMP_CHAIN_PACK_BX) {
    auto kernel = k_gru_chain_bwd<VARIANT, TPWB, 8, 1, G4>;
    int rc = chain_lds_attr(kernel, lds, &attr_bx);
    if (rc) return rc;
    TEMP_LAUNCH(K_GRU_CHAIN_BWD, kernel, dim3(a.n_panels), dim3(768), lds, st, a, ups, saved, dgi, dgh);
    return launch_status();
  }
  auto kernel = k_gru_chain_bwd<VARIANT, TPWB, 8, 0, G4>;
  int rc = chain_lds_attr(kernel, lds, &attr);
  if (rc) return rc;
  TEMP_LAUNCH(K_GRU_CHAIN_BWD, kernel, dim3(a.n_panels), dim3(768), lds, st, a, ups, saved, dgi, dgh);
  return launch_status();
}

}

using namespace temp;

extern "C" {

int temp_gru_chain_supported(int d) {
  if (d <= 0 || d % 4) return 0;
  return chain_lds_fwd(d, CH_MAX_STEPS) <= CH_LDS_LIMIT && chain_lds_bwd(d, CH_MAX_STEPS) <= CH_LDS_LIMIT && chain_geom(d).NT <= 24 && chain_geom(d).NTb <= 8;
}

size_t temp_gru_chain_pack_floats(int d) {
  if (d <= 0) return 0;
  const ChainGeom g = chain_geom(d);
  const size_t f32 = ((size_t)g.NT * g.NQ + (size_t)g.NTb * g.NQb) * 64 * 4;
  const size_t bx = ((size_t)(g.NQ >> 1) * g.NT + (size_t)(g.NQb >> 1) * g.NTb) * 192 * 4;
  const size_t hx = chain_hx_pack_floats(d);
  const size_t m = f32 > bx ? f32 : bx;
  return m > hx ? m : hx;
}

int temp_gru_chain_pack(int d, const float* w_hh, float* packed, void* stream) {
  if (d <= 0 || !w_hh || !packed) return TEMP_E_BADARG;
  if (d % 4) return TEMP_E_UNSUPPORTED;
  const ChainGeom g = chain_geom(d);
  if (chain_hx(d)) return temp_gru_chain_pack_multi(1, d, &w_hh, &packed, stream);
  if (chain_bx(d)) {
    const int nsf = g.NQ >> 1, nsb = g.NQb >> 1;
    bx_u32x4* pf = reinterpret_cast<bx_u32x4*>(packed);
    bx_u32x4* pb = pf + (size_t)nsf * g.NT * 192;
    TEMP_LAUNCH(K_GRU_CHAIN_PACK, (k_bx_pack<1>), dim3(ceil_div((long long)nsf * g.NT, 4)), dim3(256), 0, (hipStream_t)stream, d, 3 * d, g.NT, nsf,
                w_hh, d, pf);
    TEMP_LAUNCH(K_GRU_CHAIN_PACK, (k_bx_pack<0>), dim3(ceil_div((long long)nsb * g.NTb, 4)), dim3(256), 0, (hipStream_t)stream, 3 * d, d, g.NTb, nsb,
                w_hh, d, pb);
    return launch_status();
  }
  const size_t n4 = ((size_t)g.NT * g.NQ + (size_t)g.NTb * g.NQb) * 64;
  int gx = ceil_div((long long)n4, 256);
  if (gx > 1024) gx = 1024;
  TEMP_LAUNCH(K_GRU_CHAIN_PACK, k_gru_chain_pack, dim3(gx), dim3(256), 0, (hipStream_t)stream, d, w_hh, (float4*)packed);
  return launch_status();
}

int temp_gru_chain_pack_multi(int count, int d, const float* const* w_hh, float* const* packed, void* stream) {
  if (count <= 0 || count > TEMP_CHAIN_MAX_RNN || d <= 0 || !w_hh || !packed) return TEMP_E_BADARG;
  for (int i = 0; i < count; ++i) if (!w_hh[i] || !packed[i]) return TEMP_E_BADARG;
  if (d % 4) return TEMP_E_UNSUPPORTED;
  if (chain_hx(d)) {
    const ChainGeomHx gx = chain_geom_hx(d);
    HxPackJobs jobs = {};
    for (int i = 0; i < count; ++i) {
      hx_u32x4* pf = reinterpret_cast<hx_u32x4*>(packed[i]);
      hx_u32x4* pb = pf + chain_hx_fwd_items(d);
      unsigned* kf = reinterpret_cast<unsigned*>(pb + chain_hx_bwd_items(d));
      if (jobs.count + 2 > HX_PACK_JOBS) { hx_pack_launch(jobs, K_GRU_CHAIN_PACK, (hipStream_t)stream); jobs = HxPackJobs{}; }
      hx_pack_jobs_add(jobs, w_hh[i], pf, kf, d, 3 * d, d, 1);
      hx_pack_jobs_add(jobs, w_hh[i], pb, kf + gx.NT * 32, 3 * d, d, d, 0, gx.NSb);
    }
    hx_pack_launch(jobs, K_GRU_CHAIN_PACK, (hipStream_t)stream);
    return launch_status();
  }
  if (!chain_bx(d) || 2 * count > BX_PACK_JOBS) {
    for (int i = 0; i < count; ++i) { const int rc = temp_gru_chain_pack(d, w_hh[i], packed[i], stream); if (rc) return rc; }
    return TEMP_OK;
  }
  const ChainGeom g = chain_geom(d);
  BxPackJobs jobs = {};
  for (int i = 0; i < count; ++i) {
    bx_u32x4* pf = reinterpret_cast<bx_u32x4*>(packed[i]);
    bx_pack_jobs_add(jobs, w_hh[i], pf, d, 3 * d, d, 1);
    bx_pack_jobs_add(jobs, w_hh[i], pf + (size_t)(g.NQ >> 1) * g.NT * 192, 3 * d, d, d, 0);
  }
  TEMP_LAUNCH(K_GRU_CHAIN_PACK, k_bx_pack_multi, dim3(ceil_div(jobs.total_units, 4)), dim3(256), 0, (hipStream_t)stream, jobs);
  return launch_status();
}

int temp_gru_chain_fwd(const TempGruChain* c, const float* gi, float* h_out, float* saved, void* stream) {
  int rc = chain_check(c);
  if (rc) return rc;
  if (c->n_panels == 0) return TEMP_OK;
  if (!gi || !h_out || !saved) return TEMP_E_BADARG;
  const ChainArgs a = chain_args(c);
  hipStream_t st = (hipStream_t)stream;
  const int tpw = ceil_div(chain_geom(c->d).NT, 4);
#define TEMP_CHAIN_FWD(V)                                                            \
  switch (tpw) {                                                                     \
    case 1: return launch_chain_fwd<V, 1>(a, gi, h_out, saved, st);                  \
    case 2: return launch_chain_fwd<V, 2>(a, gi, h_out, saved, st);                  \
    case 3: return launch_chain_fwd<V, 3>(a, gi, h_out, saved, st);                  \
    case 4: return launch_chain_fwd<V, 4>(a, gi, h_out, saved, st);                  \
    case 5: return launch_chain_fwd<V, 5>(a, gi, h_out, saved, st);                  \
    case 6: return launch_chain_fwd<V, 6>(a, gi, h_out, saved, st);                  \
    default: return TEMP_E_UNSUPPORTED;                                              \
  }
  if (c->variant == TEMP_GRU_TORCH) { TEMP_CHAIN_FWD(TEMP_GRU_TORCH) }
  TEMP_CHAIN_FWD(TEMP_GRU_TYPE1)
#undef TEMP_CHAIN_FWD
}

int temp_gru_chain_fwd_x_supported(int d, int variant, int max_steps) {
  return d > 0 && d % 8 == 0 && variant == TEMP_GRU_TORCH && chain_fwd_x_ok(d, max_steps) ? 1 : 0;
}

size_t temp_gru_chain_pack_x_floats(int d) {
  if (d <= 0) return 0;
  return chain_x_ih_offset(d) + chain_hx_fwd_items(d) * 4;
}

int temp_gru_chain_pack_x_multi(int count, int d, const float* const* w_hh, const float* const* w_ih, float* const* packed, void* stream) {
  if (count <= 0 || count > TEMP_CHAIN_MAX_RNN || d <= 0 || !w_hh || !w_ih || !packed) return TEMP_E_BADARG;
  for (int i = 0; i < count; ++i) if (!w_hh[i] || !w_ih[i] || !packed[i]) return TEMP_E_BADARG;
  if (d % 8 || !chain_hx(d)) return TEMP_E_UNSUPPORTED;
  const ChainGeomHx gx = chain_geom_hx(d);
  HxPackJobs jobs = {};
  for (int i = 0; i < count; ++i) {
    hx_u32x4* pf = reinterpret_cast<hx_u32x4*>(packed[i]);
    hx_u32x4* pb = pf + chain_hx_fwd_items(d);
    unsigned* kf = reinterpret_cast<unsigned*>(pb + chain_hx_bwd_items(d));
    hx_u32x4* pi = reinterpret_cast<hx_u32x4*>(packed[i] + chain_x_ih_offset(d));
    if (jobs.count + 2 > HX_PACK_JOBS) { hx_pack_launch(jobs, K_GRU_CHAIN_PACK, (hipStream_t)stream); jobs = HxPackJobs{}; }
    hx_pack_jobs_add_joint(jobs, w_hh[i], pf, w_ih[i], pi, kf, d, 3 * d, d, 1);
    hx_pack_jobs_add(jobs, w_hh[i], pb, kf + gx.NT * 32, 3 * d, d, d, 0, gx.NSb);
  }
  hx_pack_launch(jobs, K_GRU_CHAIN_PACK, (hipStream_t)stream);
  return launch_status();
}

int temp_gru_chain_fwd_x(const TempGruChain* c, const float* x, const int32_t* x_index, const float* const* b_ih, float* h_out, float* saved, void* stream) {
  int rc = chain_check(c);
  if (rc) return rc;
  if (c->pack_layout != TEMP_CHAIN_PACK_HX_X) return TEMP_E_BADARG;
  if (c->variant != TEMP_GRU_TORCH || !chain_fwd_x_fits(c->d, c->max_steps)) return TEMP_E_UNSUPPORTED;
  if (c->n_panels == 0) return TEMP_OK;
  if (!x || !x_index || !b_ih || !h_out || !saved) return TEMP_E_BADARG;
  for (int i = 0; i < c->n_rnn; ++i) if (!b_ih[i]) return TEMP_E_BADARG;
  const ChainArgs a = chain_args(c);
  ChainX X = {};
  X.x = x; X.x_index = x_index;
  const ChainGeomHx gx = chain_geom_hx(c->d);
  for (int i = 0; i < c->n_rnn; ++i) {
    X.b_ih[i] = b_ih[i];
    X.wi[i] = reinterpret_cast<const hx_u32x4*>(c->packed[i] + chain_x_ih_offset(c->d));
  }
  static bool attr = false;
  const size_t lds = chain_lds_fwd_x(c->d, c->max_steps);
  hipStream_t st = (hipStream_t)stream;
  if ((gx.NT + 7) / 8 == 3) {
    auto kernel = k_gru_chain_fwd_x<3, 8, 8>;
    if ((rc = chain_lds_attr(kernel, lds, &attr))) return rc;
    TEMP_LAUNCH(K_GRU_CHAIN_FWD, kernel, dim3(a.n_panels), dim3(1024), lds, st, a, X, h_out, saved);
  } else if ((gx.NT + 7) / 8 == 2) {
    static bool attr2 = false;
    auto kernel = k_gru_chain_fwd_x<2, 8, 8>;
    if ((rc = chain_lds_attr(kernel, lds, &attr2))) return rc;
    TEMP_LAUNCH(K_GRU_CHAIN_FWD, kernel, dim3(a.n_panels), dim3(1024), lds, st, a, X, h_out, saved);
  } else {
    static bool attr1 = false;
    auto kernel = k_gru_chain_fwd_x<1, 8, 8>;
    if ((rc = chain_lds_attr(kernel, lds, &attr1))) return rc;
    TEMP_LAUNCH(K_GRU_CHAIN_FWD, kernel, dim3(a.n_panels), dim3(1024), lds, st, a, X, h_out, saved);
  }
  hx_count();
  g_fwd_x_launches.fetch_add(1, std::memory_order_relaxed);
  return launch_status();
}

long long temp_gru_chain_fwd_x_launches(void) { return g_fwd_x_launches.load(std::memory_order_relaxed); }

int temp_gru_chain_bwd_g4(const TempGruChain* c, const float* saved, int n_up, const float* const* up, float* g4, void* stream) {
  int rc = chain_check(c);
  if (rc) return rc;
  if (n_up < 0 || n_up > TEMP_CHAIN_MAX_UP || (n_up > 0 && !up)) return TEMP_E_BADARG;
  if (c->variant != TEMP_GRU_TORCH) return TEMP_E_UNSUPPORTED;
  if (c->n_panels == 0) return TEMP_OK;
  if (!saved || !g4) return TEMP_E_BADARG;
  const ChainArgs a = chain_args(c);
  ChainUps ups = {};
  for (int i = 0; i < n_up; ++i) ups.p[i] = up[i];
  hipStream_t st = (hipStream_t)stream;
  const int tpw = ceil_div(chain_geom(c->d).NTb, 4);
  if (tpw == 1) return launch_chain_bwd<TEMP_GRU_TORCH, 1, 1>(a, ups, saved, g4, nullptr, st);
  if (tpw == 2) return launch_chain_bwd<TEMP_GRU_TORCH, 2, 1>(a, ups, saved, g4, nullptr, st);
  return TEMP_E_UNSUPPORTED;
}

int temp_gru_chain_pack_layout(int d) { return d > 0 ? chain_pack_layout(d) : 0; }

int temp_gru_chain_keys_supported(int d) { return d > 0 && chain_hx(d) ? 1 : 0; }

int temp_gru_chain_bwd_g4_keys(const TempGruChain* c, const float* saved, int n_up, const float* const* up, float* g4, uint32_t* row_keys,
                               uint32_t* col_keys, void* stream) {
  int rc = chain_check(c);
  if (rc) return rc;
  if (n_up < 0 || n_up > TEMP_CHAIN_MAX_UP || (n_up > 0 && !up)) return TEMP_E_BADARG;
  if (c->variant != TEMP_GRU_TORCH || !layout_hx(c->pack_layout)) return TEMP_E_UNSUPPORTED;
  if (c->n_panels == 0) return TEMP_OK;
  if (!saved || !g4) return TEMP_E_BADARG;
  const ChainArgs a = chain_args(c);
  ChainUps ups = {};
  for (int i = 0; i < n_up; ++i) ups.p[i] = up[i];
  hipStream_t st = (hipStream_t)stream;
  const int tpw = ceil_div(chain_geom(c->d).NTb, 4);
  if (tpw == 1) return launch_chain_bwd<TEMP_GRU_TORCH, 1, 1>(a, ups, saved, g4, nullptr, st, row_keys, col_keys);
  if (tpw == 2) return launch_chain_bwd<TEMP_GRU_TORCH, 2, 1>(a, ups, saved, g4, nullptr, st, row_keys, col_keys);
  return TEMP_E_UNSUPPORTED;
}

int temp_gru_chain_bwd(const TempGruChain* c, const float* saved, int n_up, const float* const* up, float* dgi, float* dgh, void* stream) {
  int rc = chain_check(c);
  if (rc) return rc;
  if (n_up < 0 || n_up > TEMP_CHAIN_MAX_UP || (n_up > 0 && !up)) return TEMP_E_BADARG;
  if (c->n_panels == 0) return TEMP_OK;
  if (!saved || !dgi || !dgh) return TEMP_E_BADARG;
  const ChainArgs a = chain_args(c);
// ... 16 lines not shown
```

### temp_amd/csrc/gru_kernels.hip

```cpp
#include "common.hpp"
#include <stdlib.h>
#include "gemm_wres.hpp"
#include "gru_math.hpp"
#include "gru_wgrad_hx.hpp"
#include "side_stream.hpp"

namespace temp {

#define GRU_KC 40
#define GRU_LDB 33

#define GRU_NVB ((3 * GRU_KC * 32 / 4 + 255) / 256)
#define GRU_NQ (GRU_KC / 8)

struct GruPhase {
  const float* W; int row_base[3]; int D; int j0;
};

__device__ __forceinline__ bool gru_w_piece(int i, const GruPhase& ph, int k0, size_t* off) {
  const int p = threadIdx.x + i * 256;
  const int g = p / (32 * GRU_KC / 4), rem = p - g * (32 * GRU_KC / 4);
  const int j = rem / (GRU_KC / 4), k = (rem - j * (GRU_KC / 4)) * 4;
  const int rb = (g == 0) ? ph.row_base[0] : (g == 1 ? ph.row_base[1] : ph.row_base[2]);
  *off = (size_t)(rb + ph.j0 + j) * ph.D + k0 + k;
// ... 746 lines not shown
  if (d % 4) return TEMP_E_UNSUPPORTED;
  hipStream_t st = (hipStream_t)stream;
  GruGatesBatch gb = {};
  PanelBatch<EpiGruDprev> pb;
  for (int i = 0; i < PANEL_MAXP; ++i) pb.p[i] = PanelProblem<EpiGruDprev>{0, nullptr, nullptr, nullptr, EpiGruDprev{nullptr, nullptr, d}};
  for (int i = 0; i < count; ++i) {
    const TempGruCellBwd& c = cells[i];
    if (c.n < 0 || !c.w_hh) return TEMP_E_BADARG;
    if (c.n > 0 && (!c.saved || !c.dt || !c.dgi || !c.dgh || !c.decv || !c.d_prev)) return TEMP_E_BADARG;
    if (c.next_idx && !c.d_prev_next) return TEMP_E_BADARG;
    gb.c[i] = GruGatesCell{c.n, c.saved, c.dh_up, c.d_prev_next, c.next_idx, c.dt, c.dgi, c.dgh, c.decv, c.d_prev};
    pb.p[i] = PanelProblem<EpiGruDprev>{c.no_prev ? 0 : c.n, c.dgh, nullptr, c.w_hh, EpiGruDprev{c.decv, c.d_prev, d}};
  }
  int rc = launch_gru_gates_batch(gb, count, d, variant, saved_plane, lambda, nullptr, st);
  if (rc) return rc;
  return launch_gemm_panel_multi(K_GEMM_GRU_DPREV, pb, count, d, 3 * d, 3 * d, d, 0, st);
}

size_t temp_gru_weight_grads_workspace(int n, int d, int variant) {
  if (n < 0 || d <= 0) return 0;
  const int gi_w = (variant == TEMP_GRU_TORCH) ? 3 * d : d;
  size_t tn = gemm_tn_workspace(n, 3 * d, d);
  if (gemm_tn_workspace(n, gi_w, d) > tn) tn = gemm_tn_workspace(n, gi_w, d);
  return tn + colsum_workspace(n, 3 * d) + 512;
}

int temp_gru_weight_grads(int n, int d, int variant, const float* x, const float* hdec, const float* dgi, const float* dgh,
                          const float* w_ih, float* d_x, float* d_w_ih, float* d_w_hh, float* d_b_ih, float* d_b_hh, void* workspace,
                          size_t workspace_bytes, void* stream) {
  if (n < 0 || d <= 0 || !w_ih || !d_w_ih || !d_w_hh || !d_b_ih || !d_b_hh) return TEMP_E_BADARG;
  if (variant != TEMP_GRU_TORCH && variant != TEMP_GRU_TYPE1) return TEMP_E_BADARG;
  if (n > 0 && (!x || !dgi || !dgh)) return TEMP_E_BADARG;
  if (d % 4) return TEMP_E_UNSUPPORTED;
  if (!workspace || workspace_bytes < temp_gru_weight_grads_workspace(n, d, variant)) return TEMP_E_WORKSPACE;
  const int gi_w = (variant == TEMP_GRU_TORCH) ? 3 * d : d;
  size_t tn = gemm_tn_workspace(n, 3 * d, d);
  if (gemm_tn_workspace(n, gi_w, d) > tn) tn = gemm_tn_workspace(n, gi_w, d);
  char* base = (char*)workspace;
  return gru_weight_grads(n, d, variant, x, hdec, dgi, dgh, w_ih, d_x, d_w_ih, d_w_hh, d_b_ih, d_b_hh, base, tn, base + tn,
                          colsum_workspace(n, 3 * d), (hipStream_t)stream);
}

size_t temp_gru_weight_grads_multi_workspace(int count, const int* ns, int d, int variant) {
  if (count <= 0 || count > 4 || !ns || d <= 0 || variant != TEMP_GRU_TORCH) return 0;
  int max_n = 0;
  for (int i = 0; i < count; ++i) {
    if (ns[i] <= 0) return 0;
    max_n = ns[i] > max_n ? ns[i] : max_n;
  }
  if (d % 4 || !gemm_tn_multi_bias_supported(2 * count, max_n, 3 * d, d, 3 * d, d)) return 0;
  return gemm_tn_multi_bias_workspace(2 * count, max_n, 3 * d, d);
}

int temp_gru_weight_grads_multi(int count, const int* ns, int d, int variant, const float* const* xs, const float* const* hdecs,
                                const float* const* dgis, const float* const* dghs, const float* const* w_ihs, float* const* d_xs,
                                float* d_w, float* d_b, void* workspace, size_t workspace_bytes, void* stream) {
  if (count <= 0 || count > 4 || !ns || !xs || !hdecs || !dgis || !dghs || !w_ihs || !d_xs || !d_w || !d_b) return TEMP_E_BADARG;
  if (variant != TEMP_GRU_TORCH || d % 4) return TEMP_E_UNSUPPORTED;
  int max_n = 0;
  for (int i = 0; i < count; ++i) {
    if (ns[i] <= 0 || !xs[i] || !hdecs[i] || !dgis[i] || !dghs[i] || !w_ihs[i]) return TEMP_E_UNSUPPORTED;
    max_n = ns[i] > max_n ? ns[i] : max_n;
  }
  hipStream_t st = (hipStream_t)stream;
  int Ms[8];
  const float* As[8];
  const float* Bs[8];
  for (int i = 0; i < count; ++i) {
    Ms[2 * i] = Ms[2 * i + 1] = ns[i];
    As[2 * i] = dgis[i]; Bs[2 * i] = xs[i];
    As[2 * i + 1] = dghs[i]; Bs[2 * i + 1] = hdecs[i];
  }
  int rc = gemm_tn_multi_bias(2 * count, Ms, 3 * d, d, As, 3 * d, Bs, d, d_w, d_b, workspace, workspace_bytes, st);
  if (rc) return rc;
  PanelBatch<EpiStore> batch;
  int nx = 0;
  for (int i = 0; i < count; ++i)
    if (d_xs[i]) batch.p[nx++] = PanelProblem<EpiStore>{ns[i], dgis[i], nullptr, w_ihs[i], EpiStore{d_xs[i], d}};
  for (int i = nx; i < PANEL_MAXP && nx > 0; ++i) { batch.p[i] = batch.p[0]; batch.p[i].M = 0; }
  if (nx > 0) rc = launch_gemm_panel_multi(K_GEMM_GRU_DX, batch, nx, d, 3 * d, 3 * d, d, 0, st);
  return rc ? rc : launch_status();
}

size_t temp_gru_grads_g4_workspace(int count, const int* ns, int d) {
  WgArgs a = {};
  if (!grads_g4_plan(count, ns, d, &a)) return 0;
  return wg_workspace(a).total;
}

int temp_gru_grads_g4(int count, const int* ns, int d, const float* const* xs, const float* const* hdecs, const float* const* g4s,
                      const float* const* w_ihs, float* const* d_xs, float* d_w, float* d_b, void* workspace, size_t workspace_bytes,
                      void* stream) {
  return temp_gru_grads_g4_keys(count, ns, d, xs, hdecs, g4s, w_ihs, d_xs, d_w, d_b, nullptr, nullptr, nullptr, workspace, workspace_bytes, stream);
}

int temp_gru_grads_g4_keys(int count, const int* ns, int d, const float* const* xs, const float* const* hdecs, const float* const* g4s,
                           const float* const* w_ihs, float* const* d_xs, float* d_w, float* d_b, const uint32_t* const* g4_row_keys,
                           const uint32_t* const* g4_col_keys, const uint32_t* const* x_col_keys, void* workspace, size_t workspace_bytes,
                           void* stream) {
  if (count <= 0 || count > WG_MAXG || !ns || !xs || !hdecs || !g4s || !w_ihs || !d_xs || !d_w || !d_b) return TEMP_E_BADARG;
  WgArgs a = {};
  if (!grads_g4_plan(count, ns, d, &a)) return TEMP_E_UNSUPPORTED;
  for (int i = 0; i < count; ++i) {
    if (!xs[i] || !hdecs[i] || !g4s[i] || !w_ihs[i]) return TEMP_E_UNSUPPORTED;
    a.g[i] = WgGroup{ns[i], g4s[i], xs[i], hdecs[i]};
  }
  const WgWs ws = wg_workspace(a);
  if (!workspace || workspace_bytes < ws.total) return TEMP_E_WORKSPACE;
  char* base = (char*)workspace;
  a.part = (float*)(base + ws.part); a.bpart = (float*)(base + ws.bpart);
  a.part2 = (float*)(base + ws.part2); a.bpart2 = (float*)(base + ws.bpart2);
  hipStream_t st = (hipStream_t)stream;
  int rc;
  bool hx = hx_enabled() && g4_col_keys != nullptr;
  for (int i = 0; i < count && hx; ++i) hx = g4_col_keys[i] != nullptr;
  PanelBatch<EpiStore> batch;
  int nx = 0;
  for (int i = 0; i < count; ++i)
    if (d_xs[i]) batch.p[nx++] = PanelProblem<EpiStore>{ns[i], g4s[i], nullptr, w_ihs[i], EpiStore{d_xs[i], d}, (hx && g4_row_keys) ? g4_row_keys[i] : nullptr};
  for (int i = nx; i < PANEL_MAXP && nx > 0; ++i) { batch.p[i] = batch.p[0]; batch.p[i].M = 0; }
  SideScope side(st);
  const bool beside = nx > 0 && (option(TEMP_OPT_DEBUG) & 0x10000) && side_fork(side);
  if (beside) {
    rc = launch_gemm_panel_multi(K_GEMM_GRU_DX, batch, nx, d, 3 * d, 4 * d, d, 0, side.ss->s);
    if (!side_done(side) || rc) return rc ? rc : TEMP_E_LAUNCH;
  }
  if (hx) {
    WgxKeys keys = {};
    unsigned* xk = (unsigned*)(base + ws.xkeys);
    for (int i = 0; i < count; ++i) {
      keys.g[i] = g4_col_keys[i];
      if (x_col_keys && x_col_keys[i]) { keys.x[i] = x_col_keys[i]; continue; }
      keys.x[i] = xk + (size_t)i * d;
      launch_absmax_keys(ns[i], d, xs[i], d, nullptr, xk + (size_t)i * d, xk + (size_t)count * d + (size_t)i * ABSMAX_BLOCKS * d, st);
    }
    switch (wg_col_tiles(d)) {
      case 1: rc = launch_gru_wgrad_hx<1>(a, keys, st); break;
      case 2: rc = launch_gru_wgrad_hx<2>(a, keys, st); break;
      case 3: rc = launch_gru_wgrad_hx<3>(a, keys, st); break;
      case 4: rc = launch_gru_wgrad_hx<4>(a, keys, st); break;
      case 5: rc = launch_gru_wgrad_hx<5>(a, keys, st); break;
      case 6: rc = launch_gru_wgrad_hx<6>(a, keys, st); break;
      case 7: rc = launch_gru_wgrad_hx<7>(a, keys, st); break;
      default: rc = launch_gru_wgrad_hx<8>(a, keys, st); break;
    }
  } else
  switch (wg_col_tiles(d)) {
    case 1: rc = launch_gru_wgrad<1>(a, st); break;
    case 2: rc = launch_gru_wgrad<2>(a, st); break;
    case 3: rc = launch_gru_wgrad<3>(a, st); break;
    case 4: rc = launch_gru_wgrad<4>(a, st); break;
    case 5: rc = launch_gru_wgrad<5>(a, st); break;
    case 6: rc = launch_gru_wgrad<6>(a, st); break;
    case 7: rc = launch_gru_wgrad<7>(a, st); break;
    default: rc = launch_gru_wgrad<8>(a, st); break;
  }
  if (rc) return rc;
  const int Ka = 3 * d, R0 = a.tail ? 256 * a.fb : Ka, S2 = a.tail ? a.S * a.P : 0;
  const long long quads = (long long)2 * count * Ka * (d / 4);
  int gx = ceil_div(quads, 256);
  if (gx > 2048) gx = 2048;
  TEMP_LAUNCH(K_REDUCE_SLICES, k_gru_wgrad_reduce, dim3(gx), dim3(256), 0, st, 2 * count, Ka, d, a.S, a.part, a.bpart, R0, S2, a.part2, a.bpart2, d_w, d_b);
  if (beside) {
    const int jr = side.join();
    return jr ? jr : launch_status();
  }
  if (nx > 0) rc = launch_gemm_panel_multi(K_GEMM_GRU_DX, batch, nx, d, 3 * d, 4 * d, d, 0, st);
  return rc ? rc : launch_status();
}

}
```

### temp_amd/csrc/rgcn_kernels.hip

```cpp
#include <stdlib.h>
#include <atomic>
#include <mutex>
#include "common.hpp"
#include "side_stream.hpp"

namespace temp {

enum { MODE_FWD = 0, MODE_DX = 1 };

template <int S, int MODE>
__device__ __forceinline__ void block_mac(float4& acc, const float4 x, const float4* w, const float c) {
  if (S == 1) {
    acc.x = fmaf(c * x.x, w[0].x, acc.x);
    acc.y = fmaf(c * x.y, w[0].y, acc.y);
    acc.z = fmaf(c * x.z, w[0].z, acc.z);
    acc.w = fmaf(c * x.w, w[0].w, acc.w);
  } else if (S == 2) {
    const float x0 = c * x.x, x1 = c * x.y, x2 = c * x.z, x3 = c * x.w;
    if (MODE == MODE_FWD) {
      acc.x = fmaf(x0, w[0].x, fmaf(x1, w[0].z, acc.x));
      acc.y = fmaf(x0, w[0].y, fmaf(x1, w[0].w, acc.y));
      acc.z = fmaf(x2, w[1].x, fmaf(x3, w[1].z, acc.z));
      acc.w = fmaf(x2, w[1].y, fmaf(x3, w[1].w, acc.w));
    } else {
// ... 833 lines not shown
        else acc = add4(acc, x);
      };
      int e = 0;
      for (; e + 8 <= cnt; e += 8) {
        float4 x[8];
#pragma unroll
        for (int u = 0; u < 8; ++u) x[u] = row(e + u);
#pragma unroll
        for (int u = 0; u < 8; ++u) add(e + u, x[u]);
      }
      for (; e + 2 <= cnt; e += 2) {
        const float4 x0 = row(e), x1 = row(e + 1);
        add(e, x0);
        add(e + 1, x1);
      }
      if (e < cnt) add(e, row(e));
    }
  }
  return acc;
}

__device__ __forceinline__ float4 pair_epilogue(float4 v, int node, int f, int D, const int32_t* __restrict__ ids, const float* __restrict__ t_loop,
                                                const float* __restrict__ bias, int act, const DropSpec& drop) {
  float4 lm = ld4(t_loop + (size_t)ids[node] * D + f);
  if (drop.p > 0.f) lm = drop4(drop, (unsigned)node, (unsigned)f, lm);
  v = add4(v, lm);
  if (bias) v = add4(v, ld4(bias + f));
  if (act == TEMP_ACT_RELU) v = make_float4(fmaxf(v.x, 0.f), fmaxf(v.y, 0.f), fmaxf(v.z, 0.f), fmaxf(v.w, 0.f));
  return v;
}

__global__ void __launch_bounds__(256) k_pair_gather_fwd(TempEdgeView v, const int32_t* __restrict__ fwd_row, const float* __restrict__ M,
                                                         const float* __restrict__ nnorm, int D, const int32_t* __restrict__ ids,
                                                         const float* __restrict__ t_loop, const float* __restrict__ bias, int act, DropSpec drop,
                                                         float* __restrict__ out, float* __restrict__ partial) {
  const int lane = threadIdx.x & 63;
  const int wave = __builtin_amdgcn_readfirstlane(threadIdx.x >> 6), wpb = blockDim.x >> 6;
  const int f = lane << 2;
  const bool active = lane < (D >> 2);
  ItemRange it = xcd_chunks(v.n_chunks, v.n_edges, v.chunk_beg, wpb);
  for (int c = it.beg + wave; c < it.end; c += it.stride) {
    const int seg = __builtin_amdgcn_readfirstlane(v.chunk_seg[c]), beg = __builtin_amdgcn_readfirstlane(v.chunk_beg[c]);
    const int end = __builtin_amdgcn_readfirstlane(v.chunk_end[c]), slot = __builtin_amdgcn_readfirstlane(v.chunk_slot[c]);
    float4 acc = pair_rows_sum<false>(fwd_row, beg, end, M, D, nullptr, lane, active);
    if (!active) continue;
    const float nn = nnorm[seg];
    acc = scale4(acc, nn * nn);
    if (slot < 0) st4(out + (size_t)seg * D + f, pair_epilogue(acc, seg, f, D, ids, t_loop, bias, act, drop));
    else st4(partial + (size_t)slot * D + f, acc);
  }
}

__global__ void __launch_bounds__(256) k_pair_fix_epi(int n_fix, const int32_t* __restrict__ fix_seg, const int32_t* __restrict__ fix_slot,
                                                      const int32_t* __restrict__ fix_cnt, const float* __restrict__ partial, int n_nodes,
                                                      const int32_t* __restrict__ in_deg, int D, const int32_t* __restrict__ ids,
                                                      const float* __restrict__ t_loop, const float* __restrict__ bias, int act, DropSpec drop,
                                                      float* __restrict__ out) {
  const int lane = threadIdx.x & 63, wpb = blockDim.x >> 6;
  const int gw = blockIdx.x * wpb + (threadIdx.x >> 6), waves = gridDim.x * wpb;
  const int f = lane << 2;
  if (f >= D) return;
  for (int i = gw; i < n_fix; i += waves) {
    const int seg = fix_seg[i];
    st4(out + (size_t)seg * D + f, pair_epilogue(fixup_walk(partial + (size_t)fix_slot[i] * D + f, 0, fix_cnt[i], D), seg, f, D, ids, t_loop, bias, act, drop));
  }
  for (int node = gw; node < n_nodes; node += waves)
    if (in_deg[node] <= 0) st4(out + (size_t)node * D + f, pair_epilogue(zero4(), node, f, D, ids, t_loop, bias, act, drop));
}

__global__ void __launch_bounds__(256) k_pair_gather_bwd(TempEdgeView v, const float* __restrict__ dz, const float* __restrict__ nnorm, int D,
                                                         float* __restrict__ G, float* __restrict__ partial) {
  const int lane = threadIdx.x & 63;
  const int wave = __builtin_amdgcn_readfirstlane(threadIdx.x >> 6), wpb = blockDim.x >> 6;
  const int f = lane << 2;
  const bool active = lane < (D >> 2);
  for (int c = blockIdx.x * wpb + wave; c < v.n_chunks; c += gridDim.x * wpb) {
    const int seg = __builtin_amdgcn_readfirstlane(v.chunk_seg[c]), beg = __builtin_amdgcn_readfirstlane(v.chunk_beg[c]);
    const int end = __builtin_amdgcn_readfirstlane(v.chunk_end[c]), slot = __builtin_amdgcn_readfirstlane(v.chunk_slot[c]);
    const float4 acc = pair_rows_sum<true>(v.a, beg, end, dz, D, nnorm, lane, active);
    if (active) st4((slot < 0 ? G + (size_t)seg * D : partial + (size_t)slot * D) + f, acc);
  }
}

template <int S>
__global__ void __launch_bounds__(64) k_pair_dtable(int n_table, int n_rel_rows, int D, const float* __restrict__ G, const float* __restrict__ W,
                                                    float* __restrict__ d_table) {
  const int D4 = D >> 2;
  const int i = blockIdx.x * blockDim.x + threadIdx.x;
  if (i >= n_table * D4) return;
  const int e = i / D4, f = (i - e * D4) << 2;
  float4 acc = zero4();
#pragma unroll 4
  for (int r = 0; r < n_rel_rows; ++r) {
    const float* wr = W + (size_t)r * (D * S) + f * S;
    float4 w[S];
#pragma unroll
    for (int j = 0; j < S; ++j) w[j] = ld4(wr + 4 * j);
    block_mac<S, MODE_DX>(acc, ld4(G + ((size_t)r * n_table + e) * D + f), w, 1.f);
  }
  st4(d_table + (size_t)e * D + f, acc);
}

template <int S>
__global__ void __launch_bounds__(1024) k_pair_dw(int n_table, int D, const float* __restrict__ table, const float* __restrict__ G,
                                                  float* __restrict__ dW) {
  __shared__ float4 share[16][64];
  const int lane = threadIdx.x & 63, wave = __builtin_amdgcn_readfirstlane(threadIdx.x >> 6);
  const int r = blockIdx.x, f = lane << 2;
  const bool active = f < D;
  const int per = (n_table + 15) >> 4;
  const int e0 = min(n_table, wave * per), e1 = min(n_table, e0 + per);
  float4 acc[S];
#pragma unroll
  for (int j = 0; j < S; ++j) acc[j] = zero4();
  if (active) {
    const float* g = G + (size_t)r * n_table * D + f;
#pragma unroll 4
    for (int e = e0; e < e1; ++e) {
      const float4 xx = ld4(table + (size_t)e * D + f), gg = ld4(g + (size_t)e * D);
      if (S == 1) {
        acc[0].x = fmaf(xx.x, gg.x, acc[0].x);
        acc[0].y = fmaf(xx.y, gg.y, acc[0].y);
        acc[0].z = fmaf(xx.z, gg.z, acc[0].z);
        acc[0].w = fmaf(xx.w, gg.w, acc[0].w);
      } else if (S == 2) {
        acc[0].x = fmaf(xx.x, gg.x, acc[0].x);
        acc[0].y = fmaf(xx.x, gg.y, acc[0].y);
        acc[0].z = fmaf(xx.y, gg.x, acc[0].z);
        acc[0].w = fmaf(xx.y, gg.y, acc[0].w);
        acc[1].x = fmaf(xx.z, gg.z, acc[1].x);
        acc[1].y = fmaf(xx.z, gg.w, acc[1].y);
        acc[1].z = fmaf(xx.w, gg.z, acc[1].z);
        acc[1].w = fmaf(xx.w, gg.w, acc[1].w);
      } else {
        acc[0] = fma4(xx.x, gg, acc[0]);
        acc[1] = fma4(xx.y, gg, acc[1]);
        acc[2] = fma4(xx.z, gg, acc[2]);
        acc[3] = fma4(xx.w, gg, acc[3]);
      }
    }
  }
#pragma unroll
  for (int j = 0; j < S; ++j) {
    share[wave][lane] = acc[j];
    __syncthreads();
    if (wave == 0 && active) {
      float4 t = share[0][lane];
#pragma unroll
      for (int u = 1; u < 16; ++u) t = add4(t, share[u][lane]);
      st4(dW + (size_t)r * (D * S) + f * S + 4 * j, t);
    }
    __syncthreads();
  }
}

__global__ void __launch_bounds__(256) k_expand_chunk_seg(int n_chunks, const int32_t* __restrict__ chunk_seg, const int32_t* __restrict__ chunk_beg,
                                                          const int32_t* __restrict__ chunk_end, int n_pos, int32_t* __restrict__ seg_of) {
  const int lane = threadIdx.x & 63, wpb = blockDim.x >> 6;
  for (int c = blockIdx.x * wpb + (threadIdx.x >> 6); c < n_chunks; c += gridDim.x * wpb) {
    const int seg = chunk_seg[c], beg = max(0, chunk_beg[c]), end = min(n_pos, chunk_end[c]);
    for (int p = beg + lane; p < end; p += 64) seg_of[p] = seg;
  }
}

static bool pair_view_ok(const TempGraph* g, const TempPairView* pv, int n_table, int n_rel_rows) {
  if (!g || !pv || pv->n_table != n_table || pv->n_rel_rows != n_rel_rows) return false;
  const TempEdgeView& v = pv->by_pair;
  if (v.n_seg != n_rel_rows * n_table + 1 || v.n_chunks < 0 || v.n_partial < 0 || v.n_fix < 0) return false;
  if ((v.n_edges > 0 && !v.a) || !v.chunk_seg || !v.chunk_beg || !v.chunk_end || !v.chunk_slot) return false;
  if (v.n_fix > 0 && (!v.fix_seg || !v.fix_slot || !v.fix_cnt)) return false;
  return g->by_dst.n_edges == 0 || pv->fwd_row != nullptr;
}

struct PairFwdWs { float *partial, *t_loop, *M; size_t total; };
static PairFwdWs carve_pair_fwd(const TempGraph* g, const TempPairView* pv, int d_out, char* base) {
  PairFwdWs w;
  size_t off = 0;
  auto take = [&](size_t bytes) { char* p = base ? base + off : nullptr; off += align_up(bytes, 256); return p; };
  w.partial = (float*)take((size_t)g->by_dst.n_partial * d_out * sizeof(float));
  w.t_loop = (float*)take((size_t)pv->n_table * d_out * sizeof(float));
  w.M = (float*)take((size_t)pv->n_rel_rows * pv->n_table * d_out * sizeof(float));
  w.total = off + 256;
  return w;
}

struct PairBwdWs {
  float *dz, *dzm, *G, *part, *seg_dz;
  void *ss, *tn, *cs;
  size_t ss_bytes, tn_bytes, cs_bytes, total;
};
static PairBwdWs carve_pair_bwd(const TempGraph* g, const TempPairView* pv, int d_in, int d_out, char* base) {
  PairBwdWs w;
  size_t off = 0;
  auto take = [&](size_t bytes) { char* p = base ? base + off : nullptr; off += align_up(bytes, 256); return p; };
  w.dz = (float*)take((size_t)g->n_nodes * d_out * sizeof(float));
  w.dzm = (float*)take((size_t)g->n_nodes * d_out * sizeof(float));
  w.G = (float*)take((size_t)pv->by_pair.n_seg * d_out * sizeof(float));
  w.part = (float*)take(partial_bytes(pv->by_pair.n_partial, d_out));
  w.seg_dz = (float*)take((size_t)pv->n_table * d_out * sizeof(float));
  w.ss_bytes = segment_sum_rows_workspace(pv->n_table, g->n_nodes, d_out);
  w.ss = take(w.ss_bytes);
  w.tn_bytes = gemm_tn_workspace(pv->n_table, d_in, d_out);
  w.tn = take(w.tn_bytes);
  w.cs_bytes = colsum_workspace(g->n_nodes, d_out);
  w.cs = take(w.cs_bytes);
  w.total = off + 256;
  return w;
}

struct TableBwdWs {
  float *dz, *dzm, *d_h, *part_dx, *part_dw, *seg_dz;
  void *tn, *cs;
  size_t tn_bytes, cs_bytes, total;
};
static TableBwdWs carve_table_bwd(const TempGraph* g, int n_table, int d_in, int d_out, int num_bases, char* base) {
  TableBwdWs w;
  size_t off = 0;
  auto take = [&](size_t bytes) { char* p = base ? base + off : nullptr; off += align_up(bytes, 256); return p; };
  const size_t wrow = (size_t)num_bases * (d_in / num_bases) * (d_out / num_bases);
  w.dz = (float*)take((size_t)g->n_nodes * d_out * sizeof(float));
  w.dzm = (float*)take((size_t)g->n_nodes * d_out * sizeof(float));
  w.d_h = (float*)take((size_t)g->n_nodes * d_in * sizeof(float));
  w.part_dx = (float*)take(partial_bytes(g->by_src.n_partial, d_in));
  w.part_dw = (float*)take(partial_bytes(g->by_rel.n_partial, wrow));
  w.seg_dz = (float*)take((size_t)n_table * d_out * sizeof(float));
  w.tn_bytes = gemm_tn_workspace(n_table, d_in, d_out);
  w.tn = take(w.tn_bytes);
  w.cs_bytes = colsum_workspace(g->n_nodes, d_out);
  w.cs = take(w.cs_bytes);
  w.total = off + 256;
  return w;
}

}

// ... 126 lines not shown
}

int temp_rgcn_pair_fwd(const TempGraph* g, const TempPairView* pv, const float* table, const int32_t* ids, int n_table, int d_in, int d_out,
                       int num_bases, int n_rel_rows, const float* weight, const float* loop_w, const float* bias, int act, float* out,
                       void* workspace, size_t workspace_bytes, const TempDropout* drop, void* stream) {
  if (!g || !pv || !table || !weight || !loop_w || !out || n_table <= 0 || d_in <= 0 || d_out <= 0 || num_bases <= 0 || n_rel_rows <= 0) return TEMP_E_BADARG;
  int S = 0;
  if (!fast_shape(d_in, d_out, num_bases, &S)) return TEMP_E_UNSUPPORTED;
  if ((long long)n_rel_rows * n_table >= (1LL << 31) / d_out) return TEMP_E_UNSUPPORTED;
  if (g->n_nodes < 0 || !view_ok(g->by_dst) || !pair_view_ok(g, pv, n_table, n_rel_rows) || (g->n_nodes > 0 && (!g->nnorm || !g->in_deg || !ids))) return TEMP_E_BADARG;
  if (act != TEMP_ACT_NONE && act != TEMP_ACT_RELU) return TEMP_E_BADARG;
  if (!workspace || workspace_bytes < temp_rgcn_pair_fwd_workspace(g, pv, d_out)) return TEMP_E_WORKSPACE;
  if (g->n_nodes == 0) return TEMP_OK;
  hipStream_t st = (hipStream_t)stream;
  const PairFwdWs w = carve_pair_fwd(g, pv, d_out, (char*)workspace);
  const int D = d_in, P = n_rel_rows * n_table;
  int grid = ceil_div((long long)P * (D / 4), 256);
  if (grid > 8192) grid = 8192;
  if (S == 1) TEMP_LAUNCH(K_PAIR_MSG, k_pair_msg<1>, dim3(grid), dim3(256), 0, st, P, n_table, D, table, weight, w.M);
  else if (S == 2) TEMP_LAUNCH(K_PAIR_MSG, k_pair_msg<2>, dim3(grid), dim3(256), 0, st, P, n_table, D, table, weight, w.M);
  else TEMP_LAUNCH(K_PAIR_MSG, k_pair_msg<4>, dim3(grid), dim3(256), 0, st, P, n_table, D, table, weight, w.M);
  int rc = gemm_add_bias_act(K_GEMM_ISO, n_table, d_out, d_in, table, d_in, nullptr, loop_w, d_out, 0, nullptr, 0, nullptr, nullptr, TEMP_ACT_NONE,
                             w.t_loop, d_out, st);
  if (rc) return rc;
  const DropSpec ds = drop_spec(drop);
  const TempEdgeView& v = g->by_dst;
  if (v.n_chunks > 0) {
    grid = (v.n_chunks + 3) / 4;
    grid = grid < 8 ? 8 : (grid > 4096 ? 4096 : (grid + 7) / 8 * 8);
    TEMP_LAUNCH(K_PAIR_GATHER_FWD, k_pair_gather_fwd, dim3(grid), dim3(256), 0, st, v, pv->fwd_row, w.M, g->nnorm, D, ids, w.t_loop, bias, act, ds, out,
                w.partial);
  }
  const int items = v.n_fix > (g->n_nodes + 7) / 8 ? v.n_fix : (g->n_nodes + 7) / 8;
  grid = (items + 3) / 4;
  if (grid > 4096) grid = 4096;
  TEMP_LAUNCH(K_PAIR_FIX_EPI, k_pair_fix_epi, dim3(grid), dim3(256), 0, st, v.n_fix, v.fix_seg, v.fix_slot, v.fix_cnt, w.partial, g->n_nodes, g->in_deg, D,
              ids, w.t_loop, bias, act, ds, out);
  g_pair_launches.fetch_add(1, std::memory_order_relaxed);
  return launch_status();
}

size_t temp_rgcn_pair_bwd_workspace(const TempGraph* g, const TempPairView* pv, int d_in, int d_out, int num_bases) {
  if (!g || !pv || num_bases <= 0 || d_in <= 0 || d_out <= 0 || pv->n_table < 0 || pv->by_pair.n_seg < 0) return 0;
  return carve_pair_bwd(g, pv, d_in, d_out, nullptr).total;
}

int temp_rgcn_pair_bwd(const TempGraph* g, const TempPairView* pv, const float* table, const int32_t* ids, const int32_t* inv_ptr,
                       const int32_t* inv_order, int n_table, const float* out, const float* d_out_grad, int d_in, int d_out, int num_bases,
                       int n_rel_rows, const float* weight, const float* loop_w, int has_bias, int act, float* d_table, float* d_weight,
                       float* d_loop_w, float* d_bias, void* workspace, size_t workspace_bytes, const TempDropout* drop, void* stream) {
  if (!g || !pv || !table || !d_out_grad || !weight || !loop_w || !d_table || !d_weight || !d_loop_w || !inv_ptr) return TEMP_E_BADARG;
  if (n_table <= 0 || d_in <= 0 || d_out <= 0 || num_bases <= 0 || n_rel_rows <= 0) return TEMP_E_BADARG;
  int S = 0;
  if (!fast_shape(d_in, d_out, num_bases, &S)) return TEMP_E_UNSUPPORTED;
  if ((long long)n_rel_rows * n_table >= (1LL << 31) / d_out) return TEMP_E_UNSUPPORTED;
  if (act == TEMP_ACT_RELU && !out) return TEMP_E_BADARG;
  if (act != TEMP_ACT_NONE && act != TEMP_ACT_RELU) return TEMP_E_BADARG;
  if (has_bias && !d_bias) return TEMP_E_BADARG;
  if (g->n_nodes < 0 || !pair_view_ok(g, pv, n_table, n_rel_rows) || (g->n_nodes > 0 && (!g->nnorm || !ids || !inv_order))) return TEMP_E_BADARG;
  if (!workspace || workspace_bytes < temp_rgcn_pair_bwd_workspace(g, pv, d_in, d_out, num_bases)) return TEMP_E_WORKSPACE;
  hipStream_t st = (hipStream_t)stream;
  const size_t wrow = (size_t)d_in * S;
  if (g->n_nodes == 0) {
    if (hipMemsetAsync(d_table, 0, (size_t)n_table * d_in * sizeof(float), st) != hipSuccess) return TEMP_E_LAUNCH;
    if (hipMemsetAsync(d_weight, 0, (size_t)n_rel_rows * wrow * sizeof(float), st) != hipSuccess) return TEMP_E_LAUNCH;
    if (hipMemsetAsync(d_loop_w, 0, (size_t)d_in * d_out * sizeof(float), st) != hipSuccess) return TEMP_E_LAUNCH;
    if (has_bias && hipMemsetAsync(d_bias, 0, (size_t)d_out * sizeof(float), st) != hipSuccess) return TEMP_E_LAUNCH;
    return TEMP_OK;
  }
  const PairBwdWs w = carve_pair_bwd(g, pv, d_in, d_out, (char*)workspace);
  const int D = d_in;
  const float* dz = d_out_grad;
  int rc;
  if (act == TEMP_ACT_RELU) {
    rc = relu_bwd((size_t)g->n_nodes * d_out, out, d_out_grad, w.dz, st);
    if (rc) return rc;
    dz = w.dz;
  }
  const TempEdgeView& v = pv->by_pair;
  int grid = (v.n_chunks + 3) / 4;
  grid = grid < 1 ? 1 : (grid > 4096 ? 4096 : grid);
  TEMP_LAUNCH(K_PAIR_GATHER_BWD, k_pair_gather_bwd, dim3(grid), dim3(256), 0, st, v, dz, g->nnorm, D, w.G, w.part);
  launch_fixup(v, w.part, D, w.G, st);
  grid = ceil_div((long long)n_table * (D / 4), 64);
  if (S == 1) TEMP_LAUNCH(K_PAIR_DTABLE, k_pair_dtable<1>, dim3(grid), dim3(64), 0, st, n_table, n_rel_rows, D, w.G, weight, d_table);
  else if (S == 2) TEMP_LAUNCH(K_PAIR_DTABLE, k_pair_dtable<2>, dim3(grid), dim3(64), 0, st, n_table, n_rel_rows, D, w.G, weight, d_table);
  else TEMP_LAUNCH(K_PAIR_DTABLE, k_pair_dtable<4>, dim3(grid), dim3(64), 0, st, n_table, n_rel_rows, D, w.G, weight, d_table);
  if (S == 1) TEMP_LAUNCH(K_PAIR_DW, k_pair_dw<1>, dim3(n_rel_rows), dim3(1024), 0, st, n_table, D, table, w.G, d_weight);
  else if (S == 2) TEMP_LAUNCH(K_PAIR_DW, k_pair_dw<2>, dim3(n_rel_rows), dim3(1024), 0, st, n_table, D, table, w.G, d_weight);
  else TEMP_LAUNCH(K_PAIR_DW, k_pair_dw<4>, dim3(n_rel_rows), dim3(1024), 0, st, n_table, D, table, w.G, d_weight);
  const DropSpec ds = drop_spec(drop);
  const float* dzm = dz;
  if (ds.p > 0.f) {
    rc = mask_rows(g->n_nodes, d_out, dz, w.dzm, ds, st);
    if (rc) return rc;
    dzm = w.dzm;
  }
  rc = segment_sum_rows(n_table, d_out, inv_ptr, inv_order, dzm, nullptr, w.seg_dz, st, g->n_nodes, w.ss, w.ss_bytes);
  if (rc) return rc;
  rc = gemm_add_bias_act(K_GEMM_LOOP_DX, n_table, d_in, d_out, w.seg_dz, d_out, nullptr, loop_w, d_out, 1, d_table, d_in, nullptr, nullptr,
                         TEMP_ACT_NONE, d_table, d_in, st);
  if (rc) return rc;
  rc = gemm_tn(n_table, d_in, d_out, table, d_in, w.seg_dz, d_out, d_loop_w, d_out, w.tn, w.tn_bytes, st);
  if (rc) return rc;
  if (has_bias) {
    rc = colsum(g->n_nodes, d_out, dz, d_out, d_bias, w.cs, w.cs_bytes, st);
    if (rc) return rc;
  }
  g_pair_launches.fetch_add(1, std::memory_order_relaxed);
  return launch_status();
}

size_t temp_rgcn_fwd_workspace(const TempGraph* g, int d_out) {
  if (!g) return 0;
  return partial_bytes(g->by_dst.n_partial, d_out) + 256;
}

int temp_rgcn_fwd(const TempGraph* g, const float* h, const int32_t* h_ids, int d_in, int d_out, int num_bases, int n_rel_rows,
                  const float* weight, const float* loop_w, const float* bias, int act, float* out, void* workspace,
                  size_t workspace_bytes, const TempDropout* drop, void* stream) {
  if (!g || !h || !weight || !loop_w || !out || d_in <= 0 || d_out <= 0 || num_bases <= 0 || n_rel_rows <= 0) return TEMP_E_BADARG;
  if (d_in % num_bases || d_out % num_bases || d_in % 4 || d_out % 4) return TEMP_E_UNSUPPORTED;
  if (g->n_nodes < 0 || !view_ok(g->by_dst) || (g->n_nodes > 0 && (!g->nnorm || !g->in_deg))) return TEMP_E_BADARG;
  if (act != TEMP_ACT_NONE && act != TEMP_ACT_RELU) return TEMP_E_BADARG;
  if (workspace_bytes < temp_rgcn_fwd_workspace(g, d_out) || (!workspace && g->by_dst.n_partial > 0)) return TEMP_E_WORKSPACE;
  if (g->n_nodes == 0) return TEMP_OK;
  hipStream_t st = (hipStream_t)stream;
  float* partial = (float*)workspace;
  int rc = run_agg(MODE_FWD, g->by_dst, members_of(g), h, d_in, h_ids, weight, n_rel_rows, g->nnorm, d_in, d_out, num_bases, out, partial, st);
  if (rc) return rc;
  const DropSpec ds = drop_spec(drop);
  return gemm_add_bias_act(K_GEMM_LOOP_FWD, g->n_nodes, d_out, d_in, h, d_in, h_ids, loop_w, d_out, 0, out, d_out, g->in_deg, bias, act, out, d_out, st, &ds);
}

struct BwdWs {
  float* dz;
  float* dzm;
  float* part_dx;
  float* part_dw;
  void* tn;
  size_t tn_bytes;
  void* cs;
  size_t cs_bytes;
  size_t total;
};
static BwdWs carve_bwd(const TempGraph* g, int d_in, int d_out, int num_bases, char* base) {
  BwdWs w;
  size_t off = 0;
  auto take = [&](size_t bytes) { char* p = base ? base + off : nullptr; off += align_up(bytes, 256); return p; };
  const size_t wrow = (size_t)num_bases * (d_in / num_bases) * (d_out / num_bases);
  w.dz = (float*)take((size_t)g->n_nodes * d_out * sizeof(float));
  w.dzm = (float*)take((size_t)g->n_nodes * d_out * sizeof(float));
  w.part_dx = (float*)take(partial_bytes(g->by_src.n_partial, d_in));
  w.part_dw = (float*)take(partial_bytes(g->by_rel.n_partial, wrow));
  w.tn_bytes = gemm_tn_workspace(g->n_nodes, d_in, d_out);
  w.tn = take(w.tn_bytes);
  w.cs_bytes = colsum_workspace(g->n_nodes, d_out);
  w.cs = take(w.cs_bytes);
  w.total = off + 256;
  return w;
}

size_t temp_rgcn_bwd_workspace(const TempGraph* g, int d_in, int d_out, int num_bases, int n_rel_rows) {
  (void)n_rel_rows;
  if (!g || num_bases <= 0 || d_in <= 0 || d_out <= 0) return 0;
  return carve_bwd(g, d_in, d_out, num_bases, nullptr).total;
}

int temp_rgcn_bwd(const TempGraph* g, const float* h, const float* out, const float* d_out_grad, int d_in, int d_out, int num_bases,
                  int n_rel_rows, const float* weight, const float* loop_w, int has_bias, int act, float* d_h, float* d_weight,
                  float* d_loop_w, float* d_bias, void* workspace, size_t workspace_bytes, const TempDropout* drop, void* stream) {
  if (!g || !h || !d_out_grad || !weight || !loop_w || !d_h || !d_weight || !d_loop_w) return TEMP_E_BADARG;
  if (d_in <= 0 || d_out <= 0 || num_bases <= 0 || n_rel_rows <= 0) return TEMP_E_BADARG;
  if (d_in % num_bases || d_out % num_bases || d_in % 4 || d_out % 4) return TEMP_E_UNSUPPORTED;
  if (act == TEMP_ACT_RELU && !out) return TEMP_E_BADARG;
  if (has_bias && !d_bias) return TEMP_E_BADARG;
  if (!view_ok(g->by_src) || !view_ok(g->by_rel) || (g->n_nodes > 0 && (!g->nnorm || !g->out_deg))) return TEMP_E_BADARG;
  if (g->by_rel.n_seg != n_rel_rows) return TEMP_E_BADARG;
  if (!workspace || workspace_bytes < temp_rgcn_bwd_workspace(g, d_in, d_out, num_bases, n_rel_rows)) return TEMP_E_WORKSPACE;
  hipStream_t st = (hipStream_t)stream;
  const size_t wrow = (size_t)num_bases * (d_in / num_bases) * (d_out / num_bases);
  if (g->n_nodes == 0) {
    if (hipMemsetAsync(d_weight, 0, (size_t)n_rel_rows * wrow * sizeof(float), st) != hipSuccess) return TEMP_E_LAUNCH;
    if (hipMemsetAsync(d_loop_w, 0, (size_t)d_in * d_out * sizeof(float), st) != hipSuccess) return TEMP_E_LAUNCH;
    if (has_bias && hipMemsetAsync(d_bias, 0, (size_t)d_out * sizeof(float), st) != hipSuccess) return TEMP_E_LAUNCH;
    return TEMP_OK;
  }
// ... 110 lines not shown
```

### temp_amd/gru_chain.py

```python
import numpy as np
import torch

from . import _hostlib, _lib
from .backend import get_backend


CHAIN_KERNELS = True
WEIGHT_GRADS_MULTI = True
KEYED_GRADS = True
GATE_GRADS_ONCE = True
FUSED_INPUT_GATES = True


class GruInstance:
    __slots__ = ("n", "x0", "h0", "rnn", "prev", "next", "prev_idx", "next_idx", "dt", "group")

    def __init__(self, n, x0, rnn, prev, prev_idx_np, dt_np, next_idx_np=None):
        self.n, self.x0, self.rnn, self.prev = int(n), int(x0), rnn, prev
        self.h0 = 0
        self.next = -1
        self.prev_idx = prev_idx_np
        self.next_idx = next_idx_np
        self.dt = dt_np
        self.group = -1
# ... 149 lines not shown
                sel[list(want)] = np.arange(len(want), dtype=np.int32)
                h0 = np.array([it.h0 for it in self.inst], dtype=np.int32)
                sinfo[:, 0] = plan["any_prev"].astype(np.int32) | np.where(sel[si] >= 0, 2, 0)
                sinfo[:, 1] = sel[si]
                sinfo[:, 2] = np.where(sel[si] >= 0, h0[si], 0)
            dt = np.zeros(self.n_total, dtype=np.float32)
            for it in self.inst:
                if it.n:
                    dt[it.h0:it.h0 + it.n] = np.asarray(it.dt, dtype=np.float32).reshape(-1)
            _lib.pause_point()
            parts = [plan["panel"].reshape(-1), plan["rows"].reshape(-1), sinfo.reshape(-1), dt.view(np.int32)]
            buf = _lib.to_device(np.concatenate(parts), device)
            cuts = np.cumsum([0] + [p.size for p in parts])
            tabs = cache[key] = dict(n_panels=int(plan["panel"].shape[0]), n_steps=int(S), max_steps=int(plan["panel"][:, 2].max()), panel=buf[cuts[0]:cuts[1]], rows=buf[cuts[1]:cuts[2]],
                                     sinfo=buf[cuts[2]:cuts[3]], dt_bits=buf[cuts[3]:cuts[4]])
        return tabs

    def gi_shared(self, device):
        src = getattr(self, "x_src", None)
        if src is None:
            return None
        c = getattr(self, "_gi_shared", None)
        if c is not None and c[0] == str(device):
            return c[1]
        src = np.asarray(src)
        reps, g0, index, total = [], [], np.zeros(self.n_total, dtype=np.int32), 0
        n_labels = int(src.max()) + 1 if src.size else 0
        for g in self.groups:
            assert g["x1"] - g["x0"] == g["h1"] - g["h0"]
            first, inv = _hostlib.unique_labels(src[g["x0"]:g["x1"]], n_labels)
            reps.append(first)
            g0.append(total)
            index[g["h0"]:g["h1"]] = total + inv.reshape(-1)
            total += first.size
        res = None
        if total * 8 <= self.n_total * 7:
            buf = _lib.to_device(np.concatenate(reps + [index]), device)
            cuts = np.cumsum([0] + [r.size for r in reps])
            res = dict(rep=[buf[cuts[i]:cuts[i + 1]] for i in range(len(reps))], g0=g0, rows=int(total), gi_index=buf[cuts[-1]:])
        self._gi_shared = (str(device), res)
        return res

    def x_index(self, device):
        c = getattr(self, "_x_index", None)
        if c is None or c[0] != str(device):
            idx = np.zeros(self.n_total, dtype=np.int32)
            for it in self.inst:
                idx[it.h0:it.h0 + it.n] = it.x0 + np.arange(it.n, dtype=np.int32)
            c = self._x_index = (str(device), _lib.to_device(idx, device))
        return c[1]

    def constants(self, device, d):
        key = (str(device), int(d))
        c = getattr(self, "_const", None)
        if c is None or c[0] != key:
            n0 = max([it.n for it in self.inst if it.prev < 0] + [1])
            c = self._const = (key, torch.zeros(1, d, dtype=torch.float32, device=device), torch.full((n0,), -1, dtype=torch.int32, device=device))
        return c[1], c[2]

    def upload(self, device):
        if self.dev is not None and self.dev[0] == str(device):
            return self.dev[1]
        parts, spans, off = [], [], 0
        for it in self.inst:
            span = []
            for arr in (it.prev_idx.astype(np.int32) if it.prev >= 0 else None, it.next_idx,
                        np.ascontiguousarray(it.dt, dtype=np.float32).view(np.int32)):
                if arr is None:
                    span.append(None)
                    continue
                parts.append(arr.reshape(-1))
                span.append((off, off + arr.size))
                off += arr.size
            spans.append(span)
        buf = _lib.to_device(np.concatenate(parts) if parts else np.zeros(0, np.int32), device)
        cut = lambda sp: buf[sp[0]:sp[1]] if sp is not None else None
        t = [(cut(a), cut(b), cut(c).view(torch.float32)) for a, b, c in spans]
        self.dev = (str(device), t)
        return t


class _GruChainFn(torch.autograd.Function):
    @staticmethod
    def forward(ctx, x_all, prog, lam, variant, n_rnn, want, x_keys, *weights):
        be = get_backend()
        dev = x_all.device
        d = x_all.shape[1]
        G = weights[0].shape[0]
        N = prog.n_total
        x_all = x_all.detach().contiguous()
        W = [tuple(w.detach().contiguous() for w in weights[4 * r:4 * r + 4]) for r in range(n_rnn)]
        tabs = None
        if CHAIN_KERNELS and hasattr(be, "gru_chain_fwd") and n_rnn <= _lib.CHAIN_MAX_RNN and be.gru_chain_supported(d):
            tabs = prog.chain_tables(dev, want)
        fused = bool(tabs is not None and FUSED_INPUT_GATES and variant == _lib.GRU_TORCH and hasattr(be, "gru_chain_fwd_x")
                     and be.gru_chain_fwd_x_supported(d, variant, tabs["max_steps"]))
        share = prog.gi_shared(dev) if (tabs is not None and not fused) else None
        ctx.x_keys = x_keys if (x_keys is not None and tabs is not None) else None
        gk = (lambda: dict(x_keys=[ctx.x_keys[0][g["x0"]:g["x1"]] for g in prog.groups])) if ctx.x_keys is not None else dict
        gi_index = None
        if fused:
            gi = None
        elif share is not None:
            gi_index = share["gi_index"]
            gi = torch.empty(share["rows"], G, dtype=torch.float32, device=dev)
            cut = share["g0"] + [share["rows"]]
            be.gru_input_gates_multi([x_all[g["x0"]:g["x1"]] for g in prog.groups], [W[g["rnn"]][0] for g in prog.groups],
                                     [W[g["rnn"]][2] for g in prog.groups], variant, [gi[cut[i]:cut[i + 1]] for i in range(len(prog.groups))],
                                     x_idx=share["rep"], **gk())
        else:
            gi = torch.empty(N, G, dtype=torch.float32, device=dev)
        if share is not None or fused:
            pass
        elif len(prog.groups) > 1 and hasattr(be, "gru_input_gates_multi"):
            be.gru_input_gates_multi([x_all[g["x0"]:g["x1"]] for g in prog.groups], [W[g["rnn"]][0] for g in prog.groups],
                                     [W[g["rnn"]][2] for g in prog.groups], variant, [gi[g["h0"]:g["h1"]] for g in prog.groups], **gk())
        else:
            for g in prog.groups:
                w_ih, _, b_ih, _ = W[g["rnn"]]
                be.gru_input_gates(x_all[g["x0"]:g["x1"]], w_ih, b_ih, variant, gi[g["h0"]:g["h1"]])
        H = torch.empty(N, d, dtype=torch.float32, device=dev)
        saved = torch.empty(5, N, d, dtype=torch.float32, device=dev)
        packs = None
        if fused:
            packs = be.gru_chain_pack_x_multi([W[r][1] for r in range(n_rnn)], [W[r][0] for r in range(n_rnn)])
            be.gru_chain_fwd_x(tabs, x_all, prog.x_index(dev), lam, variant, packs, [W[r][3] for r in range(n_rnn)], [W[r][2] for r in range(n_rnn)],
                               H, saved)
        elif tabs is not None:
            packs = be.gru_chain_pack_multi([W[r][1] for r in range(n_rnn)]) if hasattr(be, "gru_chain_pack_multi") else \
                [be.gru_chain_pack(W[r][1]) for r in range(n_rnn)]
            be.gru_chain_fwd(tabs, gi, lam, variant, packs, [W[r][3] for r in range(n_rnn)], H, saved, gi_index=gi_index)
        else:
            tens = prog.upload(dev)
            zero, none_idx = prog.constants(dev, d)
        for level in (prog.levels if tabs is None else ()):
            cells = []
            for i in level:
                it = prog.inst[i]
                pi, _, dt = tens[i]
                _, w_hh, _, b_hh = W[it.rnn]
                if it.prev >= 0:
                    p = prog.inst[it.prev]
                    prev, pidx = H[p.h0:p.h0 + p.n], pi
                else:
                    prev, pidx = None, none_idx[:it.n]
                cells.append(dict(gi=gi[it.h0:it.h0 + it.n], prev=prev, prev_idx=pidx, dt=dt, w_hh=w_hh, b_hh=b_hh,
                                  h_out=H[it.h0:it.h0 + it.n], row0=it.h0))
            be.gru_cell_fwd_multi(cells, lam, variant, saved)
        ctx.set_materialize_grads(False)
        ctx.save_for_backward(x_all, saved, *[w for ws in W for w in ws])
        ctx.prog, ctx.lam, ctx.variant, ctx.n_rnn, ctx.G, ctx.want = prog, lam, variant, n_rnn, G, want
        ctx.tabs, ctx.packs = tabs, packs
        if want is None:
            return H
        return tuple(H[prog.inst[i].h0:prog.inst[i].h0 + prog.inst[i].n] for i in want)

    @staticmethod
    def backward(ctx, *d_outs):
        be = get_backend()
        x_all, saved = ctx.saved_tensors[:2]
        flat = ctx.saved_tensors[2:]
        W = [flat[4 * r:4 * r + 4] for r in range(ctx.n_rnn)]
        prog, lam, variant, G = ctx.prog, ctx.lam, ctx.variant, ctx.G
        dev, d, N = x_all.device, x_all.shape[1], prog.n_total
        if ctx.want is None:
            dH = d_outs[0].contiguous() if d_outs[0] is not None else torch.zeros(N, d, dtype=torch.float32, device=dev)
            up = lambda i, it: dH[it.h0:it.h0 + it.n]
        else:
            given = {i: g.contiguous() for i, g in zip(ctx.want, d_outs) if g is not None}
            up = lambda i, it: given.get(i)
        groups = list(prog.groups)
        zero_state = [all(it.prev < 0 for it in prog.inst if it.group == gi) for gi in range(len(groups))]
        disjoint = all(groups[a]["x1"] <= groups[b]["x0"] or groups[b]["x1"] <= groups[a]["x0"] for a in range(len(groups)) for b in range(a))
        one_launch = bool(groups and disjoint and not any(zero_state) and len({g["rnn"] for g in groups}) == len(groups) and WEIGHT_GRADS_MULTI)
        once = bool(one_launch and GATE_GRADS_ONCE and ctx.tabs is not None and hasattr(be, "gru_grads_g4")
                    and be.gru_grads_g4_supported([g["h1"] - g["h0"] for g in groups], d, variant))
        if once:
            g4 = torch.empty(N, 4 * d, dtype=torch.float32, device=dev)
            ups = [dH] if ctx.want is None else [given.get(i) for i in ctx.want]
            keyed = bool(KEYED_GRADS and hasattr(be, "gru_chain_keys_supported") and be.gru_chain_keys_supported(d))
            keys = (torch.empty(N, dtype=torch.int32, device=dev), torch.empty(ctx.n_rnn + ctx.tabs["n_panels"], 4 * d, dtype=torch.int32, device=dev)) if keyed else None
            be.gru_chain_bwd_g4(ctx.tabs, saved, ups, lam, variant, ctx.packs, [W[r][3] for r in range(ctx.n_rnn)], g4, **({"keys": keys} if keyed else {}))
            d_x_all = torch.empty_like(x_all)
            xsl = [slice(g["x0"], g["x1"]) for g in groups]
            hsl = [slice(g["h0"], g["h1"]) for g in groups]
            kw = dict(row_keys=[keys[0][b] for b in hsl], col_keys=[keys[1][g["rnn"]] for g in groups]) if keyed else {}
            if keyed and ctx.x_keys is not None:
                kw["x_col_keys"] = [ctx.x_keys[1]] * len(groups)
            multi = be.gru_grads_g4([x_all[a] for a in xsl], [saved[4, b] for b in hsl], [g4[b] for b in hsl], [W[g["rnn"]][0] for g in groups],
                                    [d_x_all[a] for a in xsl], **kw)
            grads = [None] * (4 * ctx.n_rnn)
            covered = np.zeros(x_all.shape[0], dtype=bool)
            for g, gw in zip(groups, multi):
                covered[g["x0"]:g["x1"]] = True
                for k in range(4):
                    grads[4 * g["rnn"] + k] = gw[k]
            if not covered.all():
                d_x_all[torch.from_numpy(~covered).to(dev)] = 0
            return (d_x_all, None, None, None, None, None, None) + tuple(grads)
        dgi = torch.empty(N, G, dtype=torch.float32, device=dev)
        dgh = torch.empty(N, 3 * d, dtype=torch.float32, device=dev)
        if ctx.tabs is not None:
            ups = [dH] if ctx.want is None else [given.get(i) for i in ctx.want]
            be.gru_chain_bwd(ctx.tabs, saved, ups, lam, variant, ctx.packs, [W[r][3] for r in range(ctx.n_rnn)], dgi, dgh)
        else:
            tens = prog.upload(dev)
            decv = torch.empty(N, dtype=torch.float32, device=dev)
            d_prev = torch.empty(N, d, dtype=torch.float32, device=dev)
        for level in (reversed(prog.levels) if ctx.tabs is None else ()):
            cells = []
            for i in level:
                it = prog.inst[i]
                _, ni, dt = tens[i]
                nxt = prog.inst[it.next] if (it.next >= 0 and prog.inst[it.next].n > 0) else None
                sl = slice(it.h0, it.h0 + it.n)
                cells.append(dict(row0=it.h0, n=it.n, dh_up=up(i, it), d_prev_next=d_prev[nxt.h0:nxt.h0 + nxt.n] if nxt is not None else None,
                                  next_idx=ni if nxt is not None else None, dt=dt, w_hh=W[it.rnn][1], dgi=dgi[sl], dgh=dgh[sl],
                                  decv=decv[sl], d_prev=d_prev[sl], no_prev=it.prev < 0))
            be.gru_cell_bwd_multi(cells, lam, variant, saved)
        d_x_all = torch.empty_like(x_all)
        written = np.zeros(x_all.shape[0], dtype=bool)
        grads = [None] * (4 * ctx.n_rnn)
        multi = None
        if one_launch and hasattr(be, "gru_weight_grads_multi"):
            xsl = [slice(g["x0"], g["x1"]) for g in groups]
            hsl = [slice(g["h0"], g["h1"]) for g in groups]
            multi = be.gru_weight_grads_multi([x_all[a] for a in xsl], [saved[4, b] for b in hsl], [dgi[b] for b in hsl], [dgh[b] for b in hsl],
                                              [W[g["rnn"]][0] for g in groups], variant, [d_x_all[a] for a in xsl])
        if multi is not None:
            for g, gw in zip(groups, multi):
                written[g["x0"]:g["x1"]] = True
                for k in range(4):
                    grads[4 * g["rnn"] + k] = gw[k]
            groups = []
        for g in groups:
            gi_ = prog.groups.index(g)
            xs, hs = slice(g["x0"], g["x1"]), slice(g["h0"], g["h1"])
            first = not written[xs].any()
            assert first or written[xs].all()
            tgt = d_x_all[xs] if first else torch.empty(g["x1"] - g["x0"], d, dtype=torch.float32, device=dev)
            gw = be.gru_weight_grads(x_all[xs], None if zero_state[gi_] else saved[4, hs], dgi[hs], dgh[hs], W[g["rnn"]][0], variant, tgt)
            if not first:
                d_x_all[xs] += tgt
            written[xs] = True
            for k in range(4):
                j = 4 * g["rnn"] + k
                grads[j] = gw[k] if grads[j] is None else grads[j] + gw[k]
        if not written.all():
            d_x_all[torch.from_numpy(~written).to(dev)] = 0
        return (d_x_all, None, None, None, None, None, None) + tuple(grads)


def chain_kernels_usable(d, n_rnn=1):
    be = get_backend()
    return bool(CHAIN_KERNELS and hasattr(be, "gru_chain_fwd") and n_rnn <= _lib.CHAIN_MAX_RNN and be.gru_chain_supported(d))


def prepare_program(prog, device, d, n_rnn, want):
    if chain_kernels_usable(d, n_rnn) and prog.chain_tables(device, tuple(want) if want is not None else None) is not None:
        _lib.pause_point()
        prog.gi_shared(device)
        prog.x_index(device)
        return
    prog.upload(device)


def zero_state_program(n):
    return GruProgram([GruInstance(n, 0, 0, -1, np.full(n, -1, dtype=np.int32), np.zeros(n, dtype=np.float32))])


def gru_chain(x_all, prog, rnns, lam, type1=False, want=None, x_keys=None):
    ws = []
    for r in rnns:
        if type1:
            ws += [r.weight_ih, r.weight_hh, r.bias_ih, r.bias_hh]
        else:
            ws += [r.weight_ih_l0, r.weight_hh_l0, r.bias_ih_l0, r.bias_hh_l0]
    return _GruChainFn.apply(x_all, prog, float(lam), _lib.GRU_TYPE1 if type1 else _lib.GRU_TORCH, len(rnns),
                             tuple(want) if want is not None else None, x_keys, *ws)
```

Before: 922.6 million.

## Pre-pack GRU input weights for backward dx and fuse RGCN pair-backward tail kernels

When gradients are needed, the forward GRU chain pack now also packs W_ih into the hx layout used by the backward dx GEMM. The backward g4 gradient path can then pass these precomputed packs in and skip repacking the weights on every call. Separately, the RGCN pair backward replaces the separate dtable, dweight, loop-dx GEMM and loop-weight TN GEMM launches with one fused k_pair_tail kernel, which cuts launches and passes over memory. The cost is a larger pack buffer, extra pack work in the forward pass, and a hand-written fused kernel that may be slower per item than the tuned GEMMs.

```diff
diff --git a/include/temp_amd.h b/include/temp_amd.h
--- a/include/temp_amd.h
+++ b/include/temp_amd.h
@@ -214,6 +214,10 @@
                            const float* const* w_ihs, float* const* d_xs, float* d_w, float* d_b, const uint32_t* const* g4_row_keys,
                            const uint32_t* const* g4_col_keys, const uint32_t* const* x_col_keys ,
                            void* workspace, size_t workspace_bytes, void* stream);
+int temp_gru_grads_g4_keys_packed(int count, const int* ns, int d, const float* const* xs, const float* const* hdecs, const float* const* g4s,
+                                  const float* const* w_ihs, float* const* d_xs, float* d_w, float* d_b, const uint32_t* const* g4_row_keys,
+                                  const uint32_t* const* g4_col_keys, const uint32_t* const* x_col_keys, const float* const* w_ih_packs,
+                                  void* workspace, size_t workspace_bytes, void* stream);
 
 #define TEMP_CHAIN_HAS_PREV (1 << 30)
 #define TEMP_CHAIN_TRACKS 32
@@ -232,7 +236,8 @@
   const int32_t* gi_index;
   int32_t pack_layout;
 } TempGruChain;
-enum { TEMP_CHAIN_PACK_F32 = 1, TEMP_CHAIN_PACK_BX = 2, TEMP_CHAIN_PACK_HX = 3, TEMP_CHAIN_PACK_HX_X = 4 };
+enum { TEMP_CHAIN_PACK_F32 = 1, TEMP_CHAIN_PACK_BX = 2, TEMP_CHAIN_PACK_HX = 3, TEMP_CHAIN_PACK_HX_X = 4,
+       TEMP_CHAIN_PACK_HX_X_DX = 5  };
 int temp_gru_chain_pack_layout(int d);
 int temp_gru_chain_supported(int d);
 size_t temp_gru_chain_pack_floats(int d);
@@ -242,6 +247,8 @@
 int temp_gru_chain_fwd_x_supported(int d, int variant, int max_steps);
 size_t temp_gru_chain_pack_x_floats(int d);
 int temp_gru_chain_pack_x_multi(int count, int d, const float* const* w_hh, const float* const* w_ih, float* const* packed, void* stream);
+size_t temp_gru_chain_pack_dx_offset(int d);
+int temp_gru_chain_pack_x_dx_multi(int count, int d, const float* const* w_hh, const float* const* w_ih, float* const* packed, void* stream);
 int temp_gru_chain_fwd_x(const TempGruChain* c, const float* x, const int32_t* x_index, const float* const* b_ih, float* h_out, float* saved,
                          void* stream);
 long long temp_gru_chain_fwd_x_launches(void);
diff --git a/temp_amd/_lib.py b/temp_amd/_lib.py
--- a/temp_amd/_lib.py
+++ b/temp_amd/_lib.py
@@ -56,7 +56,8 @@
 CHAIN_MAX_RNN = 4
 CHAIN_MAX_UP = 8
 CHAIN_MAX_STEPS = 64
-CHAIN_PACK_F32, CHAIN_PACK_BX, CHAIN_PACK_HX, CHAIN_PACK_HX_X = 1, 2, 3, 4
+CHAIN_PACK_F32, CHAIN_PACK_BX, CHAIN_PACK_HX, CHAIN_PACK_HX_X, CHAIN_PACK_HX_X_DX = 1, 2, 3, 4, 5
+DEBUG_DX_PACK_HERE = 1 << 23
 
 
 class TempGruChain(ctypes.Structure):
@@ -151,6 +152,8 @@
     "temp_gru_chain_fwd_x_supported": (_I, [_I, _I, _I]),
     "temp_gru_chain_pack_x_floats": (_SZ, [_I]),
     "temp_gru_chain_pack_x_multi": (_I, [_I, _I, ctypes.POINTER(c_vp), ctypes.POINTER(c_vp), ctypes.POINTER(c_vp), c_vp]),
+    "temp_gru_chain_pack_dx_offset": (_SZ, [_I]),
+    "temp_gru_chain_pack_x_dx_multi": (_I, [_I, _I, ctypes.POINTER(c_vp), ctypes.POINTER(c_vp), ctypes.POINTER(c_vp), c_vp]),
     "temp_gru_chain_fwd_x": (_I, [ctypes.POINTER(TempGruChain), c_vp, c_vp, ctypes.POINTER(c_vp), c_vp, c_vp, c_vp]),
     "temp_gru_chain_fwd_x_launches": (ctypes.c_longlong, []),
     "temp_gru_chain_bwd": (_I, [ctypes.POINTER(TempGruChain), c_vp, _I, ctypes.POINTER(c_vp), c_vp, c_vp, c_vp]),
@@ -158,6 +161,7 @@
     "temp_gru_chain_keys_supported": (_I, [_I]),
     "temp_gru_chain_bwd_g4_keys": (_I, [ctypes.POINTER(TempGruChain), c_vp, _I, ctypes.POINTER(c_vp), c_vp, c_vp, c_vp, c_vp]),
     "temp_gru_grads_g4_keys": (_I, [_I, c_vp, _I, c_vp, c_vp, c_vp, c_vp, c_vp, c_vp, c_vp, c_vp, c_vp, c_vp, c_vp, ctypes.c_size_t, c_vp]),
+    "temp_gru_grads_g4_keys_packed": (_I, [_I, c_vp, _I, c_vp, c_vp, c_vp, c_vp, c_vp, c_vp, c_vp, c_vp, c_vp, c_vp, c_vp, c_vp, ctypes.c_size_t, c_vp]),
     "temp_gru_grads_g4_workspace": (ctypes.c_size_t, [_I, c_vp, _I]),
     "temp_gru_grads_g4": (_I, [_I, c_vp, _I, c_vp, c_vp, c_vp, c_vp, c_vp, c_vp, c_vp, c_vp, ctypes.c_size_t, c_vp]),
     "temp_gather_rows": (_I, [_I, _I, c_vp, c_vp, c_vp, c_vp]),
diff --git a/temp_amd/backend.py b/temp_amd/backend.py
--- a/temp_amd/backend.py
+++ b/temp_amd/backend.py
@@ -404,13 +404,18 @@
     def gru_chain_fwd_x_supported(self, d, variant, max_steps):
         return bool(self.lib.temp_gru_chain_fwd_x_supported(int(d), int(variant), int(max_steps)))
 
-    def gru_chain_pack_x_multi(self, w_hhs, w_ihs):
+    def gru_chain_pack_x_multi(self, w_hhs, w_ihs, dx=False):
         w_hhs, w_ihs = [_f32(w, "w_hh") for w in w_hhs], [_f32(w, "w_ih") for w in w_ihs]
         d = w_hhs[0].shape[1]
         k = len(w_hhs)
         n = self.lib.temp_gru_chain_pack_x_floats(d)
         buf = torch.empty(k, n, dtype=torch.float32, device=w_hhs[0].device)
         arr = lambda ts: (ctypes.c_void_p * k)(*[t.data_ptr() for t in ts])
+        dx = bool(dx) and not (self.lib.temp_get_option(_lib.OPT_DEBUG) & _lib.DEBUG_DX_PACK_HERE)
+        if dx:
+            _lib.check(self.lib.temp_gru_chain_pack_x_dx_multi(k, d, arr(w_hhs), arr(w_ihs), arr([buf[i] for i in range(k)]), _stream()),
+                       "temp_gru_chain_pack_x_dx_multi")
+            return self._tagged([buf[i] for i in range(k)], _lib.CHAIN_PACK_HX_X_DX)
         _lib.check(self.lib.temp_gru_chain_pack_x_multi(k, d, arr(w_hhs), arr(w_ihs), arr([buf[i] for i in range(k)]), _stream()),
                    "temp_gru_chain_pack_x_multi")
         return self._tagged([buf[i] for i in range(k)], _lib.CHAIN_PACK_HX_X)
@@ -458,7 +463,7 @@
             return False
         return self.lib.temp_gru_grads_g4_workspace(k, (ctypes.c_int * k)(*[int(n) for n in ns]), int(d)) > 0
 
-    def gru_grads_g4(self, xs, hdecs, g4s, w_ihs, d_xs, row_keys=None, col_keys=None, x_col_keys=None):
+    def gru_grads_g4(self, xs, hdecs, g4s, w_ihs, d_xs, row_keys=None, col_keys=None, x_col_keys=None, dx_packs=None):
         k = len(xs)
         d = xs[0].shape[1]
         dev = xs[0].device
@@ -483,6 +488,13 @@
                 for t in x_col_keys:
                     assert t.dtype == torch.int32 and t.is_contiguous() and t.numel() == d
                 xk = arr(x_col_keys)
+            if dx_packs is not None and all(getattr(pk, "chain_pack_layout", None) == _lib.CHAIN_PACK_HX_X_DX for pk in dx_packs):
+                off = 4 * self.lib.temp_gru_chain_pack_dx_offset(d)
+                wp = (ctypes.c_void_p * k)(*[pk.data_ptr() + off for pk in dx_packs])
+                rc = self.lib.temp_gru_grads_g4_keys_packed(k, ns, d, arr(keep[0]), arr(keep[1]), arr(g4s), arr(keep[2]), dx, _ptr(d_w), _ptr(d_b),
+                                                            arr(row_keys), arr(col_keys), xk, wp, _ptr(ws), ws.numel(), _stream())
+                _lib.check(rc, "temp_gru_grads_g4_keys_packed")
+                return [(d_w[2 * i], d_w[2 * i + 1], d_b[2 * i], d_b[2 * i + 1]) for i in range(k)]
             rc = self.lib.temp_gru_grads_g4_keys(k, ns, d, arr(keep[0]), arr(keep[1]), arr(g4s), arr(keep[2]), dx, _ptr(d_w), _ptr(d_b),
                                                  arr(row_keys), arr(col_keys), xk, _ptr(ws), ws.numel(), _stream())
             _lib.check(rc, "temp_gru_grads_g4_keys")
diff --git a/temp_amd/csrc/gemm_bx.hpp b/temp_amd/csrc/gemm_bx.hpp
--- a/temp_amd/csrc/gemm_bx.hpp
+++ b/temp_amd/csrc/gemm_bx.hpp
@@ -602,11 +602,11 @@
 }
 
 template <class Epi>
-int launch_gemm_bx(int kid, const PanelBatch<Epi>& batch, int count, const BxGeom& g, int G, hipStream_t st) {
+int launch_gemm_bx(int kid, const PanelBatch<Epi>& batch, int count, const BxGeom& g, int G, hipStream_t st, const HxPacked* hx_pre = nullptr) {
   if (launch_hxr(kid, batch, count, g, st)) return launch_status();
   if (launch_bxr(kid, batch, count, g, st, nullptr)) return launch_status();
   if (hx_supported(batch, count, g)) {
-    const int rc = launch_gemm_hx(kid, batch, count, g, G, st);
+    const int rc = launch_gemm_hx(kid, batch, count, g, G, st, hx_pre);
     if (rc != TEMP_E_UNSUPPORTED) return rc;
   }
   BxPacked pk;
diff --git a/temp_amd/csrc/gemm_hx.hpp b/temp_amd/csrc/gemm_hx.hpp
--- a/temp_amd/csrc/gemm_hx.hpp
+++ b/temp_amd/csrc/gemm_hx.hpp
@@ -288,7 +288,7 @@
 }
 
 template <class Epi>
-int launch_gemm_hx(int kid, const PanelBatch<Epi>& batch_in, int count, const BxGeom& g, int G, hipStream_t st) {
+int launch_gemm_hx(int kid, const PanelBatch<Epi>& batch_in, int count, const BxGeom& g, int G, hipStream_t st, const HxPacked* pre = nullptr) {
   const size_t pbytes = align_up(hx_pack_bytes(g.N, g.K), 256);
   int n_distinct = 0, which[PANEL_MAXP];
   for (int i = 0; i < count; ++i) {
@@ -297,7 +297,7 @@
       if (batch_in.p[j].B == batch_in.p[i].B) { which[i] = which[j]; break; }
     if (which[i] < 0) which[i] = n_distinct++;
   }
-  if (pbytes * n_distinct > BX_PACK_MAX_BYTES || n_distinct > HX_PACK_JOBS) return TEMP_E_UNSUPPORTED;
+  if (!pre && (pbytes * n_distinct > BX_PACK_MAX_BYTES || n_distinct > HX_PACK_JOBS)) return TEMP_E_UNSUPPORTED;
   unsigned char* slot = reinterpret_cast<unsigned char*>(bx_scratch(st, BX_SLOT_BYTES));
   if (!slot) return TEMP_E_UNSUPPORTED;
   PanelBatch<Epi> batch = batch_in;
@@ -306,7 +306,8 @@
   const size_t items = hx_packed_items(g.N, g.K);
   int done = 0;
   for (int i = 0; i < PANEL_MAXP; ++i) { pk.b[i] = reinterpret_cast<const hx_u32x4*>(slot); pk.keys[i] = reinterpret_cast<const unsigned*>(slot + items * 16); }
-  for (int i = 0; i < count; ++i) {
+  if (pre) pk = *pre;
+  for (int i = 0; i < count && !pre; ++i) {
     unsigned char* dst = slot + (size_t)which[i] * pbytes;
     pk.b[i] = reinterpret_cast<const hx_u32x4*>(dst);
     pk.keys[i] = reinterpret_cast<const unsigned*>(dst + items * 16);
diff --git a/temp_amd/csrc/gemm_wres.hpp b/temp_amd/csrc/gemm_wres.hpp
--- a/temp_amd/csrc/gemm_wres.hpp
+++ b/temp_amd/csrc/gemm_wres.hpp
@@ -288,7 +288,8 @@
 inline bool wres_disabled() { return option(TEMP_OPT_GEMM_STREAM) != 0; }
 
 template <class Epi>
-int launch_gemm_panel_multi(int kid, const PanelBatch<Epi>& batch, int count, int N, int K, int lda, int ldb, int trans_b, hipStream_t st) {
+int launch_gemm_panel_multi(int kid, const PanelBatch<Epi>& batch, int count, int N, int K, int lda, int ldb, int trans_b, hipStream_t st,
+                            const HxPacked* hx_pre = nullptr) {
   if (count <= 0 || count > PANEL_MAXP) return TEMP_E_BADARG;
   long long rows = 0;
   for (int i = 0; i < count; ++i) rows += batch.p[i].M > 0 ? batch.p[i].M : 0;
@@ -299,7 +300,7 @@
       for (int i = 0; i < count; ++i) max_m = batch.p[i].M > max_m ? batch.p[i].M : max_m;
       BxGeom bg;
       int G;
-      if (bx_plan(N, K, lda, ldb, trans_b, max_m, rows, &bg, &G)) return launch_gemm_bx(kid, batch, count, bg, G, st);
+      if (bx_plan(N, K, lda, ldb, trans_b, max_m, rows, &bg, &G)) return launch_gemm_bx(kid, batch, count, bg, G, st, hx_pre);
       if (K % 8 == 4 && bx_plan(N, K, lda, ldb, trans_b, max_m, rows, &bg, &G, true) && hx_supported(batch, count, bg)) {
         const int rc = launch_gemm_hx(kid, batch, count, bg, G, st);
         if (rc != TEMP_E_UNSUPPORTED) return rc;
diff --git a/temp_amd/csrc/gru_chain.hip b/temp_amd/csrc/gru_chain.hip
--- a/temp_amd/csrc/gru_chain.hip
+++ b/temp_amd/csrc/gru_chain.hip
@@ -599,9 +599,9 @@
 static bool chain_layout_ok(int layout, int d) {
   if (layout == TEMP_CHAIN_PACK_F32) return true;
   if (layout == TEMP_CHAIN_PACK_BX) return d % 8 == 0;
-  return (layout == TEMP_CHAIN_PACK_HX || layout == TEMP_CHAIN_PACK_HX_X) && chain_hx_fits(d);
-}
-static bool layout_hx(int layout) { return layout == TEMP_CHAIN_PACK_HX || layout == TEMP_CHAIN_PACK_HX_X; }
+  return (layout == TEMP_CHAIN_PACK_HX || layout == TEMP_CHAIN_PACK_HX_X || layout == TEMP_CHAIN_PACK_HX_X_DX) && chain_hx_fits(d);
+}
+static bool layout_hx(int layout) { return layout == TEMP_CHAIN_PACK_HX || layout == TEMP_CHAIN_PACK_HX_X || layout == TEMP_CHAIN_PACK_HX_X_DX; }
 
 static ChainArgs chain_args(const TempGruChain* c) {
   ChainArgs a = {};
@@ -687,6 +687,7 @@
 #define CH_FWD_X_OFF 0x400000
 static std::atomic<long long> g_fwd_x_launches{0};
 static size_t chain_x_ih_offset(int d) { return chain_hx_pack_floats(d); }
+static size_t chain_x_dx_offset(int d) { return align_up((chain_x_ih_offset(d) + chain_hx_fwd_items(d) * 4) * sizeof(float), 256) / sizeof(float); }
 static bool chain_fwd_x_fits(int d, int max_steps) {
   return chain_hx_fits(d) && d / 4 <= 64 && max_steps > 0 && max_steps <= CH_MAX_STEPS && chain_lds_fwd_x(d, max_steps) <= CH_LDS_LIMIT &&
          (chain_geom_hx(d).NT + 7) / 8 <= 3;
@@ -846,32 +847,47 @@
 
 size_t temp_gru_chain_pack_x_floats(int d) {
   if (d <= 0) return 0;
-  return chain_x_ih_offset(d) + chain_hx_fwd_items(d) * 4;
-}
-
-int temp_gru_chain_pack_x_multi(int count, int d, const float* const* w_hh, const float* const* w_ih, float* const* packed, void* stream) {
+  return chain_x_dx_offset(d) + align_up(hx_pack_bytes(d, 3 * d), 256) / sizeof(float);
+}
+
+size_t temp_gru_chain_pack_dx_offset(int d) { return d > 0 ? chain_x_dx_offset(d) : 0; }
+
+static int chain_pack_x(int count, int d, const float* const* w_hh, const float* const* w_ih, float* const* packed, bool dx, void* stream) {
   if (count <= 0 || count > TEMP_CHAIN_MAX_RNN || d <= 0 || !w_hh || !w_ih || !packed) return TEMP_E_BADARG;
   for (int i = 0; i < count; ++i) if (!w_hh[i] || !w_ih[i] || !packed[i]) return TEMP_E_BADARG;
   if (d % 8 || !chain_hx(d)) return TEMP_E_UNSUPPORTED;
   const ChainGeomHx gx = chain_geom_hx(d);
+  const int per = dx ? 3 : 2;
   HxPackJobs jobs = {};
   for (int i = 0; i < count; ++i) {
     hx_u32x4* pf = reinterpret_cast<hx_u32x4*>(packed[i]);
     hx_u32x4* pb = pf + chain_hx_fwd_items(d);
     unsigned* kf = reinterpret_cast<unsigned*>(pb + chain_hx_bwd_items(d));
     hx_u32x4* pi = reinterpret_cast<hx_u32x4*>(packed[i] + chain_x_ih_offset(d));
-    if (jobs.count + 2 > HX_PACK_JOBS) { hx_pack_launch(jobs, K_GRU_CHAIN_PACK, (hipStream_t)stream); jobs = HxPackJobs{}; }
+    if (jobs.count + per > HX_PACK_JOBS) { hx_pack_launch(jobs, K_GRU_CHAIN_PACK, (hipStream_t)stream); jobs = HxPackJobs{}; }
     hx_pack_jobs_add_joint(jobs, w_hh[i], pf, w_ih[i], pi, kf, d, 3 * d, d, 1);
     hx_pack_jobs_add(jobs, w_hh[i], pb, kf + gx.NT * 32, 3 * d, d, d, 0, gx.NSb);
+    if (dx) {
+      hx_u32x4* px = reinterpret_cast<hx_u32x4*>(packed[i] + chain_x_dx_offset(d));
+      hx_pack_jobs_add(jobs, w_ih[i], px, reinterpret_cast<unsigned*>(px + hx_packed_items(d, 3 * d)), 3 * d, d, d, 0);
+    }
   }
   hx_pack_launch(jobs, K_GRU_CHAIN_PACK, (hipStream_t)stream);
   return launch_status();
+}
+
+int temp_gru_chain_pack_x_multi(int count, int d, const float* const* w_hh, const float* const* w_ih, float* const* packed, void* stream) {
+  return chain_pack_x(count, d, w_hh, w_ih, packed, false, stream);
+}
+
+int temp_gru_chain_pack_x_dx_multi(int count, int d, const float* const* w_hh, const float* const* w_ih, float* const* packed, void* stream) {
+  return chain_pack_x(count, d, w_hh, w_ih, packed, true, stream);
 }
 
 int temp_gru_chain_fwd_x(const TempGruChain* c, const float* x, const int32_t* x_index, const float* const* b_ih, float* h_out, float* saved, void* stream) {
   int rc = chain_check(c);
   if (rc) return rc;
-  if (c->pack_layout != TEMP_CHAIN_PACK_HX_X) return TEMP_E_BADARG;
+  if (c->pack_layout != TEMP_CHAIN_PACK_HX_X && c->pack_layout != TEMP_CHAIN_PACK_HX_X_DX) return TEMP_E_BADARG;
   if (c->variant != TEMP_GRU_TORCH || !chain_fwd_x_fits(c->d, c->max_steps)) return TEMP_E_UNSUPPORTED;
   if (c->n_panels == 0) return TEMP_OK;
   if (!x || !x_index || !b_ih || !h_out || !saved) return TEMP_E_BADARG;
diff --git a/temp_amd/csrc/gru_kernels.hip b/temp_amd/csrc/gru_kernels.hip
--- a/temp_amd/csrc/gru_kernels.hip
+++ b/temp_amd/csrc/gru_kernels.hip
@@ -852,6 +852,8 @@
   return rc ? rc : launch_status();
 }
 
+#define GRU_DX_PACK_HERE 0x800000
+
 size_t temp_gru_grads_g4_workspace(int count, const int* ns, int d) {
   WgArgs a = {};
   if (!grads_g4_plan(count, ns, d, &a)) return 0;
@@ -868,6 +870,14 @@
                            const float* const* w_ihs, float* const* d_xs, float* d_w, float* d_b, const uint32_t* const* g4_row_keys,
                            const uint32_t* const* g4_col_keys, const uint32_t* const* x_col_keys, void* workspace, size_t workspace_bytes,
                            void* stream) {
+  return temp_gru_grads_g4_keys_packed(count, ns, d, xs, hdecs, g4s, w_ihs, d_xs, d_w, d_b, g4_row_keys, g4_col_keys, x_col_keys, nullptr, workspace,
+                                       workspace_bytes, stream);
+}
+
+int temp_gru_grads_g4_keys_packed(int count, const int* ns, int d, const float* const* xs, const float* const* hdecs, const float* const* g4s,
+                                  const float* const* w_ihs, float* const* d_xs, float* d_w, float* d_b, const uint32_t* const* g4_row_keys,
+                                  const uint32_t* const* g4_col_keys, const uint32_t* const* x_col_keys, const float* const* w_ih_packs,
+                                  void* workspace, size_t workspace_bytes, void* stream) {
   if (count <= 0 || count > WG_MAXG || !ns || !xs || !hdecs || !g4s || !w_ihs || !d_xs || !d_w || !d_b) return TEMP_E_BADARG;
   WgArgs a = {};
   if (!grads_g4_plan(count, ns, d, &a)) return TEMP_E_UNSUPPORTED;
@@ -889,10 +899,24 @@
   for (int i = 0; i < count; ++i)
     if (d_xs[i]) batch.p[nx++] = PanelProblem<EpiStore>{ns[i], g4s[i], nullptr, w_ihs[i], EpiStore{d_xs[i], d}, (hx && g4_row_keys) ? g4_row_keys[i] : nullptr};
   for (int i = nx; i < PANEL_MAXP && nx > 0; ++i) { batch.p[i] = batch.p[0]; batch.p[i].M = 0; }
+  HxPacked dx_pre;
+  bool pre = hx && nx > 0 && w_ih_packs != nullptr && !(option(TEMP_OPT_DEBUG) & GRU_DX_PACK_HERE);
+  for (int i = 0; i < count && pre; ++i) pre = !d_xs[i] || w_ih_packs[i] != nullptr;
+  if (pre) {
+    const size_t items = hx_packed_items(d, 3 * d);
+    int j = 0;
+    for (int i = 0; i < count; ++i) {
+      if (!d_xs[i]) continue;
+      dx_pre.b[j] = reinterpret_cast<const hx_u32x4*>(w_ih_packs[i]);
+      dx_pre.keys[j++] = reinterpret_cast<const unsigned*>(reinterpret_cast<const unsigned char*>(w_ih_packs[i]) + items * 16);
+    }
+    for (; j < PANEL_MAXP; ++j) { dx_pre.b[j] = dx_pre.b[0]; dx_pre.keys[j] = dx_pre.keys[0]; }
+  }
+  const HxPacked* dx_pk = pre ? &dx_pre : nullptr;
   SideScope side(st);
   const bool beside = nx > 0 && (option(TEMP_OPT_DEBUG) & 0x10000) && side_fork(side);
   if (beside) {
-    rc = launch_gemm_panel_multi(K_GEMM_GRU_DX, batch, nx, d, 3 * d, 4 * d, d, 0, side.ss->s);
+    rc = launch_gemm_panel_multi(K_GEMM_GRU_DX, batch, nx, d, 3 * d, 4 * d, d, 0, side.ss->s, dx_pk);
     if (!side_done(side) || rc) return rc ? rc : TEMP_E_LAUNCH;
   }
   if (hx) {
@@ -935,7 +959,7 @@
     const int jr = side.join();
     return jr ? jr : launch_status();
   }
-  if (nx > 0) rc = launch_gemm_panel_multi(K_GEMM_GRU_DX, batch, nx, d, 3 * d, 4 * d, d, 0, st);
+  if (nx > 0) rc = launch_gemm_panel_multi(K_GEMM_GRU_DX, batch, nx, d, 3 * d, 4 * d, d, 0, st, dx_pk);
   return rc ? rc : launch_status();
 }
 
diff --git a/temp_amd/csrc/rgcn_kernels.hip b/temp_amd/csrc/rgcn_kernels.hip
--- a/temp_amd/csrc/rgcn_kernels.hip
+++ b/temp_amd/csrc/rgcn_kernels.hip
@@ -939,6 +939,21 @@
   }
 }
 
+template <int S, int U>
+__device__ __forceinline__ float4 pair_dtable_rel(int n_table, int n_rel_rows, int D, const float* __restrict__ G, const float* __restrict__ W,
+                                                  int e, int f) {
+  float4 acc = zero4();
+#pragma unroll U
+  for (int r = 0; r < n_rel_rows; ++r) {
+    const float* wr = W + (size_t)r * (D * S) + f * S;
+    float4 w[S];
+#pragma unroll
+    for (int j = 0; j < S; ++j) w[j] = ld4(wr + 4 * j);
+    block_mac<S, MODE_DX>(acc, ld4(G + ((size_t)r * n_table + e) * D + f), w, 1.f);
+  }
+  return acc;
+}
+
 template <int S>
 __global__ void __launch_bounds__(64) k_pair_dtable(int n_table, int n_rel_rows, int D, const float* __restrict__ G, const float* __restrict__ W,
                                                     float* __restrict__ d_table) {
@@ -946,35 +961,23 @@
   const int i = blockIdx.x * blockDim.x + threadIdx.x;
   if (i >= n_table * D4) return;
   const int e = i / D4, f = (i - e * D4) << 2;
-  float4 acc = zero4();
-#pragma unroll 4
-  for (int r = 0; r < n_rel_rows; ++r) {
-    const float* wr = W + (size_t)r * (D * S) + f * S;
-    float4 w[S];
-#pragma unroll
-    for (int j = 0; j < S; ++j) w[j] = ld4(wr + 4 * j);
-    block_mac<S, MODE_DX>(acc, ld4(G + ((size_t)r * n_table + e) * D + f), w, 1.f);
-  }
-  st4(d_table + (size_t)e * D + f, acc);
+  st4(d_table + (size_t)e * D + f, pair_dtable_rel<S, 4>(n_table, n_rel_rows, D, G, W, e, f));
 }
 
 template <int S>
-__global__ void __launch_bounds__(1024) k_pair_dw(int n_table, int D, const float* __restrict__ table, const float* __restrict__ G,
-                                                  float* __restrict__ dW) {
-  __shared__ float4 share[16][64];
+__device__ __forceinline__ void pair_dw_block(float4 (*share)[64], int n_table, int D, const float* __restrict__ xp, const float* __restrict__ gp,
+                                              float* __restrict__ out, int ostep) {
   const int lane = threadIdx.x & 63, wave = __builtin_amdgcn_readfirstlane(threadIdx.x >> 6);
-  const int r = blockIdx.x, f = lane << 2;
-  const bool active = f < D;
+  const bool active = (lane << 2) < D;
   const int per = (n_table + 15) >> 4;
   const int e0 = min(n_table, wave * per), e1 = min(n_table, e0 + per);
   float4 acc[S];
 #pragma unroll
   for (int j = 0; j < S; ++j) acc[j] = zero4();
   if (active) {
-    const float* g = G + (size_t)r * n_table * D + f;
 #pragma unroll 4
     for (int e = e0; e < e1; ++e) {
-      const float4 xx = ld4(table + (size_t)e * D + f), gg = ld4(g + (size_t)e * D);
+      const float4 xx = ld4(xp + (size_t)e * D), gg = ld4(gp + (size_t)e * D);
       if (S == 1) {
         acc[0].x = fmaf(xx.x, gg.x, acc[0].x);
         acc[0].y = fmaf(xx.y, gg.y, acc[0].y);
@@ -1005,9 +1008,95 @@
       float4 t = share[0][lane];
 #pragma unroll
       for (int u = 1; u < 16; ++u) t = add4(t, share[u][lane]);
-      st4(dW + (size_t)r * (D * S) + f * S + 4 * j, t);
+      st4(out + (size_t)j * ostep, t);
     }
     __syncthreads();
+  }
+}
+
+template <int S>
+__global__ void __launch_bounds__(1024) k_pair_dw(int n_table, int D, const float* __restrict__ table, const float* __restrict__ G,
+                                                  float* __restrict__ dW) {
+  __shared__ float4 share[16][64];
+  const int r = blockIdx.x, f = (threadIdx.x & 63) << 2;
+  pair_dw_block<S>(share, n_table, D, table + f, G + (size_t)r * n_table * D + f, dW + (size_t)r * (D * S) + f * S, 4);
+}
+
+constexpr int PT_ROWS = 8, PT_KT = 40, PT_LD = PT_KT + 1;
+static_assert(PT_KT % 4 == 0 && 3 * 1024 * 4 >= 256 * PT_KT, "three float4 per thread hold a [256][PT_KT] tile of loop_w");
+static_assert(PT_ROWS == 2 * (1024 / 256) && PT_ROWS * (256 / 4) <= 1024, "a quarter of the block owns two rows; one thread per float4 of the 8 rows");
+static_assert(PT_ROWS * 256 * sizeof(float) <= 16 * 64 * sizeof(float4), "the loop term [PT_ROWS][256] fits the wave shares");
+template <int S>
+__global__ void __launch_bounds__(1024) k_pair_tail(int n_table, int n_rel_rows, int D, int nb_dt, const float* __restrict__ G,
+                                                    const float* __restrict__ W, const float* __restrict__ table,
+                                                    const float* __restrict__ seg_dz, const float* __restrict__ loop_w,
+                                                    float* __restrict__ d_table, float* __restrict__ dW, float* __restrict__ d_loop_w) {
+  __shared__ float4 share[16][64];
+  __shared__ float lt[256 * PT_LD];
+  const int t = threadIdx.x;
+  int b = blockIdx.x;
+  if (b >= nb_dt) {
+    b -= nb_dt;
+    const int f = (t & 63) << 2;
+    if (b < n_rel_rows) pair_dw_block<S>(share, n_table, D, table + f, G + (size_t)b * n_table * D + f, dW + (size_t)b * (D * S) + f * S, 4);
+    else pair_dw_block<4>(share, n_table, D, table + 4 * (b - n_rel_rows), seg_dz + f, d_loop_w + (size_t)4 * (b - n_rel_rows) * D + f, D);
+    return;
+  }
+  const int e0 = b * PT_ROWS;
+  const int q = __builtin_amdgcn_readfirstlane(t >> 8), i = t & 255;
+  const float* sa = seg_dz + (size_t)min(e0 + 2 * q, n_table - 1) * D;
+  const float* sb = seg_dz + (size_t)min(e0 + 2 * q + 1, n_table - 1) * D;
+  float acc_a = 0.f, acc_b = 0.f;
+  float4 pre[3];
+  auto fetch = [&](int k0) {
+    const int kn4 = min(PT_KT, D - k0) >> 2;
+#pragma unroll
+    for (int u = 0; u < 3; ++u) {
+      const int idx = t + u * 1024;
+      if (idx < D * kn4) {
+        const int row = idx / kn4, c = idx - row * kn4;
+        pre[u] = ld4(loop_w + (size_t)row * D + k0 + 4 * c);
+      }
+    }
+  };
+  fetch(0);
+  for (int k0 = 0; k0 < D; k0 += PT_KT) {
+    const int kn = min(PT_KT, D - k0), kn4 = kn >> 2;
+    __syncthreads();
+#pragma unroll
+    for (int u = 0; u < 3; ++u) {
+      const int idx = t + u * 1024;
+      if (idx < D * kn4) {
+        const int row = idx / kn4, c = idx - row * kn4;
+        float* p = lt + row * PT_LD + 4 * c;
+        p[0] = pre[u].x; p[1] = pre[u].y; p[2] = pre[u].z; p[3] = pre[u].w;
+      }
+    }
+    __syncthreads();
+    if (k0 + PT_KT < D) fetch(k0 + PT_KT);
+    if (i < D) {
+      const float* l = lt + i * PT_LD;
+#pragma unroll 2
+      for (int kk = 0; kk < kn; kk += 4) {
+        const float4 a = ld4(sa + k0 + kk), c = ld4(sb + k0 + kk);
+        acc_a = fmaf(a.x, l[kk], acc_a); acc_b = fmaf(c.x, l[kk], acc_b);
+        acc_a = fmaf(a.y, l[kk + 1], acc_a); acc_b = fmaf(c.y, l[kk + 1], acc_b);
+        acc_a = fmaf(a.z, l[kk + 2], acc_a); acc_b = fmaf(c.z, l[kk + 2], acc_b);
+        acc_a = fmaf(a.w, l[kk + 3], acc_a); acc_b = fmaf(c.w, l[kk + 3], acc_b);
+      }
+    }
+  }
+  float* lr = (float*)&share[0][0];
+  lr[(2 * q) * 256 + i] = acc_a;
+  lr[(2 * q + 1) * 256 + i] = acc_b;
+  __syncthreads();
+  const int D4 = D >> 2;
+  if (t < PT_ROWS * D4) {
+    const int er = t / D4, f = (t - er * D4) << 2, e = e0 + er;
+    if (e < n_table) {
+      const float4 rel = pair_dtable_rel<S, 8>(n_table, n_rel_rows, D, G, W, e, f);
+      st4(d_table + (size_t)e * D + f, add4(rel, ld4(lr + er * 256 + f)));
+    }
   }
 }
 
@@ -1300,13 +1389,6 @@
   grid = grid < 1 ? 1 : (grid > 4096 ? 4096 : grid);
   TEMP_LAUNCH(K_PAIR_GATHER_BWD, k_pair_gather_bwd, dim3(grid), dim3(256), 0, st, v, dz, g->nnorm, D, w.G, w.part);
   launch_fixup(v, w.part, D, w.G, st);
-  grid = ceil_div((long long)n_table * (D / 4), 64);
-  if (S == 1) TEMP_LAUNCH(K_PAIR_DTABLE, k_pair_dtable<1>, dim3(grid), dim3(64), 0, st, n_table, n_rel_rows, D, w.G, weight, d_table);
-  else if (S == 2) TEMP_LAUNCH(K_PAIR_DTABLE, k_pair_dtable<2>, dim3(grid), dim3(64), 0, st, n_table, n_rel_rows, D, w.G, weight, d_table);
-  else TEMP_LAUNCH(K_PAIR_DTABLE, k_pair_dtable<4>, dim3(grid), dim3(64), 0, st, n_table, n_rel_rows, D, w.G, weight, d_table);
-  if (S == 1) TEMP_LAUNCH(K_PAIR_DW, k_pair_dw<1>, dim3(n_rel_rows), dim3(1024), 0, st, n_table, D, table, w.G, d_weight);
-  else if (S == 2) TEMP_LAUNCH(K_PAIR_DW, k_pair_dw<2>, dim3(n_rel_rows), dim3(1024), 0, st, n_table, D, table, w.G, d_weight);
-  else TEMP_LAUNCH(K_PAIR_DW, k_pair_dw<4>, dim3(n_rel_rows), dim3(1024), 0, st, n_table, D, table, w.G, d_weight);
   const DropSpec ds = drop_spec(drop);
   const float* dzm = dz;
   if (ds.p > 0.f) {
@@ -1316,11 +1398,26 @@
   }
   rc = segment_sum_rows(n_table, d_out, inv_ptr, inv_order, dzm, nullptr, w.seg_dz, st, g->n_nodes, w.ss, w.ss_bytes);
   if (rc) return rc;
-  rc = gemm_add_bias_act(K_GEMM_LOOP_DX, n_table, d_in, d_out, w.seg_dz, d_out, nullptr, loop_w, d_out, 1, d_table, d_in, nullptr, nullptr,
-                         TEMP_ACT_NONE, d_table, d_in, st);
-  if (rc) return rc;
-  rc = gemm_tn(n_table, d_in, d_out, table, d_in, w.seg_dz, d_out, d_loop_w, d_out, w.tn, w.tn_bytes, st);
-  if (rc) return rc;
+  if (!(option(TEMP_OPT_RGCN_PAIR) & 16)) {
+    const int nb_dt = ceil_div(n_table, PT_ROWS);
+    grid = nb_dt + n_rel_rows + D / 4;
+    if (S == 1) TEMP_LAUNCH(K_PAIR_DTABLE, k_pair_tail<1>, dim3(grid), dim3(1024), 0, st, n_table, n_rel_rows, D, nb_dt, w.G, weight, table, w.seg_dz, loop_w, d_table, d_weight, d_loop_w);
+    else if (S == 2) TEMP_LAUNCH(K_PAIR_DTABLE, k_pair_tail<2>, dim3(grid), dim3(1024), 0, st, n_table, n_rel_rows, D, nb_dt, w.G, weight, table, w.seg_dz, loop_w, d_table, d_weight, d_loop_w);
+    else TEMP_LAUNCH(K_PAIR_DTABLE, k_pair_tail<4>, dim3(grid), dim3(1024), 0, st, n_table, n_rel_rows, D, nb_dt, w.G, weight, table, w.seg_dz, loop_w, d_table, d_weight, d_loop_w);
+  } else {
+    grid = ceil_div((long long)n_table * (D / 4), 64);
+    if (S == 1) TEMP_LAUNCH(K_PAIR_DTABLE, k_pair_dtable<1>, dim3(grid), dim3(64), 0, st, n_table, n_rel_rows, D, w.G, weight, d_table);
+    else if (S == 2) TEMP_LAUNCH(K_PAIR_DTABLE, k_pair_dtable<2>, dim3(grid), dim3(64), 0, st, n_table, n_rel_rows, D, w.G, weight, d_table);
+    else TEMP_LAUNCH(K_PAIR_DTABLE, k_pair_dtable<4>, dim3(grid), dim3(64), 0, st, n_table, n_rel_rows, D, w.G, weight, d_table);
+    if (S == 1) TEMP_LAUNCH(K_PAIR_DW, k_pair_dw<1>, dim3(n_rel_rows), dim3(1024), 0, st, n_table, D, table, w.G, d_weight);
+    else if (S == 2) TEMP_LAUNCH(K_PAIR_DW, k_pair_dw<2>, dim3(n_rel_rows), dim3(1024), 0, st, n_table, D, table, w.G, d_weight);
+    else TEMP_LAUNCH(K_PAIR_DW, k_pair_dw<4>, dim3(n_rel_rows), dim3(1024), 0, st, n_table, D, table, w.G, d_weight);
+    rc = gemm_add_bias_act(K_GEMM_LOOP_DX, n_table, d_in, d_out, w.seg_dz, d_out, nullptr, loop_w, d_out, 1, d_table, d_in, nullptr, nullptr,
+                           TEMP_ACT_NONE, d_table, d_in, st);
+    if (rc) return rc;
+    rc = gemm_tn(n_table, d_in, d_out, table, d_in, w.seg_dz, d_out, d_loop_w, d_out, w.tn, w.tn_bytes, st);
+    if (rc) return rc;
+  }
   if (has_bias) {
     rc = colsum(g->n_nodes, d_out, dz, d_out, d_bias, w.cs, w.cs_bytes, st);
     if (rc) return rc;
diff --git a/temp_amd/gru_chain.py b/temp_amd/gru_chain.py
--- a/temp_amd/gru_chain.py
+++ b/temp_amd/gru_chain.py
@@ -255,7 +255,7 @@
 
 class _GruChainFn(torch.autograd.Function):
     @staticmethod
-    def forward(ctx, x_all, prog, lam, variant, n_rnn, want, x_keys, *weights):
+    def forward(ctx, x_all, prog, lam, variant, n_rnn, want, x_keys, bwd, *weights):
         be = get_backend()
         dev = x_all.device
         d = x_all.shape[1]
@@ -296,7 +296,8 @@
         saved = torch.empty(5, N, d, dtype=torch.float32, device=dev)
         packs = None
         if fused:
-            packs = be.gru_chain_pack_x_multi([W[r][1] for r in range(n_rnn)], [W[r][0] for r in range(n_rnn)])
+            packs = be.gru_chain_pack_x_multi([W[r][1] for r in range(n_rnn)], [W[r][0] for r in range(n_rnn)],
+                                              dx=bool(bwd) and any(ctx.needs_input_grad))
             be.gru_chain_fwd_x(tabs, x_all, prog.x_index(dev), lam, variant, packs, [W[r][3] for r in range(n_rnn)], [W[r][2] for r in range(n_rnn)],
                                H, saved)
         elif tabs is not None:
@@ -360,6 +361,8 @@
             kw = dict(row_keys=[keys[0][b] for b in hsl], col_keys=[keys[1][g["rnn"]] for g in groups]) if keyed else {}
             if keyed and ctx.x_keys is not None:
                 kw["x_col_keys"] = [ctx.x_keys[1]] * len(groups)
+            if keyed and getattr(ctx.packs[0], "chain_pack_layout", None) == _lib.CHAIN_PACK_HX_X_DX:
+                kw["dx_packs"] = [ctx.packs[g["rnn"]] for g in groups]
             multi = be.gru_grads_g4([x_all[a] for a in xsl], [saved[4, b] for b in hsl], [g4[b] for b in hsl], [W[g["rnn"]][0] for g in groups],
                                     [d_x_all[a] for a in xsl], **kw)
             grads = [None] * (4 * ctx.n_rnn)
@@ -370,7 +373,7 @@
                     grads[4 * g["rnn"] + k] = gw[k]
             if not covered.all():
                 d_x_all[torch.from_numpy(~covered).to(dev)] = 0
-            return (d_x_all, None, None, None, None, None, None) + tuple(grads)
+            return (d_x_all, None, None, None, None, None, None, None) + tuple(grads)
         dgi = torch.empty(N, G, dtype=torch.float32, device=dev)
         dgh = torch.empty(N, 3 * d, dtype=torch.float32, device=dev)
         if ctx.tabs is not None:
@@ -421,7 +424,7 @@
                 grads[j] = gw[k] if grads[j] is None else grads[j] + gw[k]
         if not written.all():
             d_x_all[torch.from_numpy(~written).to(dev)] = 0
-        return (d_x_all, None, None, None, None, None, None) + tuple(grads)
+        return (d_x_all, None, None, None, None, None, None, None) + tuple(grads)
 
 
 def chain_kernels_usable(d, n_rnn=1):
@@ -450,4 +453,4 @@
         else:
             ws += [r.weight_ih_l0, r.weight_hh_l0, r.bias_ih_l0, r.bias_hh_l0]
     return _GruChainFn.apply(x_all, prog, float(lam), _lib.GRU_TYPE1 if type1 else _lib.GRU_TORCH, len(rnns),
-                             tuple(want) if want is not None else None, x_keys, *ws)
+                             tuple(want) if want is not None else None, x_keys, torch.is_grad_enabled(), *ws)
```

New measurement: 939.0 million, median of 6. 1.02x the previous value.
